# marl/l3embedding

Measured on AMD Instinct MI355X. Metric: AVC training pairs/sec (1s audio + 224x224 frame), higher is better.
Workload: dtype f32; 1 GPU; full cnn_L3_melspec2 AVC training step (audio+vision+fusion, fwd+bwd+Adam), batch 64 per GPU, global batch 64, fp32, inputs resident in HBM; global_batch=64, parallelism=dp1, fp32_conv=f4x4

## Files before the change

### include/l3hip.h

```cpp
#ifndef L3HIP_H
#define L3HIP_H

#include <stdint.h>

#ifdef __cplusplus
extern "C" {
#endif

#define L3_OK 0
#define L3_EINVAL (-1)
#define L3_EHIP (-2)
#define L3_ENOMEM (-3)
#define L3_ESTATE (-4)
#define L3_ECOMM (-5)

#define L3_MODEL_CNN_L3_ORIG 0
#define L3_MODEL_TINY_L3 1
#define L3_MODEL_CNN_L3_KAPREDBINPUTBN 2
#define L3_MODEL_CNN_L3_MELSPEC1 3
#define L3_MODEL_CNN_L3_MELSPEC2 4

typedef struct l3_engine l3_engine;

#define L3_DTYPE_F32 0
#define L3_DTYPE_BF16 1

#define L3_FP32_CONV_F4X4 0
#define L3_FP32_CONV_F2X2 1
#define L3_FP32_CONV_F2X2_BF16X6 2

#define L3_DP_MOVING_REPLICAS 0
#define L3_DP_MOVING_RANK_LOCAL 1

typedef struct l3_config {
    int32_t struct_size;
    int32_t model_type;
    int32_t batch;
    int32_t global_batch;
    int32_t device;
    int32_t db_max_scope;
    int32_t bn_zero_debias;
    int32_t dtype;
    void *stream;
    int32_t fp32_conv;
    int32_t dp_moving;
} l3_config;

int l3_create(const l3_config *cfg, uint64_t seed, l3_engine **out);
void l3_destroy(l3_engine *e);
const char *l3_last_error(const l3_engine *e);
int l3_model_type_from_name(const char *name);
int l3_build_experiments(void);
int l3_device_count(void);

int l3_param_count(const l3_engine *e);
int l3_param_info(const l3_engine *e, int index, char *name, int name_cap,
                  int32_t *ndim, int64_t shape[4], int32_t *trainable, int64_t *numel);
int l3_set_param(l3_engine *e, const char *name, const float *src, int64_t numel);
int l3_get_param(l3_engine *e, const char *name, float *dst, int64_t numel);
int l3_get_grad(l3_engine *e, const char *name, float *dst, int64_t numel);
int l3_reset_optimizer(l3_engine *e);
int l3_copy_state(l3_engine *dst, l3_engine *src);
int l3_optimizer_steps(const l3_engine *e, int64_t *adam_t, int64_t *bn_steps);

int l3_forward(l3_engine *e, const float *video, const float *audio, int training,
               float *probs, float *logits);

int l3_train_step(l3_engine *e, const float *video, const float *audio,
                  const float *labels, float lr, float *loss, float *acc);
int l3_eval_step(l3_engine *e, const float *video, const float *audio,
                 const float *labels, float *loss, float *acc);

int l3_upload_batch(l3_engine *e, const float *video, const float *audio, const float *labels);
int l3_upload_batch_raw(l3_engine *e, const uint8_t *video_u8, const int16_t *audio_i16,
                        const int32_t *labels_i32);
int l3_stage_batch_raw(l3_engine *e, const uint8_t *video_u8, const int16_t *audio_i16, const int32_t *labels_i32);
typedef struct l3_augment_params {
    int32_t start_x, start_y;
    int32_t flip;
    int32_t sat_first;
    float saturation;
    float brightness;
} l3_augment_params;
int l3_upload_batch_raw_aug(l3_engine *e, const uint8_t *video_u8, const int16_t *audio_i16, const int32_t *labels_i32,
                            const l3_augment_params *params, const double *u);
int l3_stage_batch_raw_aug(l3_engine *e, const uint8_t *video_u8, const int16_t *audio_i16, const int32_t *labels_i32,
                           const l3_augment_params *params, const double *u);
int l3_batch_gains(l3_engine *e, double *gains);
int l3_step_forward(l3_engine *e, int training);
int l3_tower_step(l3_engine *e, int tower, int backward);
int l3_step_bucket_count(const l3_engine *e);
int l3_step_backward_bucket(l3_engine *e, int bucket);
int l3_step_update(l3_engine *e, float lr, float grad_scale);
int l3_step_resident(l3_engine *e, float lr);
int l3_step_results(l3_engine *e, float *loss, float *acc, float *probs, float *logits);
int l3_step_results_enqueue(l3_engine *e, int slot, int reduce);
int l3_step_results_wait(l3_engine *e, int slot, float *loss, float *acc);

int l3_replicas_upload(l3_engine *e, const float *video, const float *audio, const float *labels, int replicas);
int l3_replicas_upload_raw(l3_engine *e, const uint8_t *video_u8, const int16_t *audio_i16, const int32_t *labels_i32, int replicas);
int l3_replicas_upload_raw_aug(l3_engine *e, const uint8_t *video_u8, const int16_t *audio_i16, const int32_t *labels_i32,
                               const l3_augment_params *params, const double *u, int replicas);
int l3_replicas_stage_raw(l3_engine *e, const uint8_t *video_u8, const int16_t *audio_i16, const int32_t *labels_i32, int replicas);
int l3_replicas_stage_raw_aug(l3_engine *e, const uint8_t *video_u8, const int16_t *audio_i16, const int32_t *labels_i32,
                              const l3_augment_params *params, const double *u, int replicas);
int l3_step_replicas(l3_engine *e, float lr);
int l3_eval_replicas(l3_engine *e, float *loss, float *acc);

#define L3_COMM_ID_BYTES 128
int l3_comm_unique_id(void *id128);
int l3_comm_init(l3_engine *e, const void *id128, int world, int rank);
int l3_comm_destroy(l3_engine *e);
int l3_comm_info(const l3_engine *e, int *world, int *rank, char *library_path, int path_cap);
int l3_comm_version(void);
int l3_comm_allreduce_host(l3_engine *e, double *vals, int n, int op);
int l3_step_dp(l3_engine *e, float lr);
int l3_comm_timing(l3_engine *e, int on);
int l3_comm_timing_read(l3_engine *e, double *exposed_ms, double *span_ms, double *bucket_ms, int cap, int *steps);

int l3_grad_arena_dev(l3_engine *e, void **dev_ptr, int64_t *numel);
int l3_bucket_range(const l3_engine *e, int bucket, int64_t *offset, int64_t *numel);
int l3_bn_stats_pack_dev(l3_engine *e, void **send_dev, int64_t *numel);
int l3_bn_stats_replicas_dev(l3_engine *e, int world, void **gathered_dev);

int l3_embed_audio(l3_engine *e, const float *audio, int64_t n, int pool_h, int pool_w, float *out);
int l3_embed_vision(l3_engine *e, const float *video, int64_t n, int pool_h, int pool_w, float *out);
int64_t l3_embed_dim(const l3_engine *e, int vision, int pool_h, int pool_w);
int l3_embed_audio_frames(l3_engine *e, const float *samples, int64_t n_samples, const int64_t *table,
                          int64_t n_frames, int pool_h, int pool_w, float *out);
int l3_embed_audio_clips_resampled(l3_engine *e, const float *native, int64_t n_native, const int64_t *clips,
                                   int64_t n_clips, const double *half_window, int64_t n_window, int num_table,
                                   int64_t n_samples, const int64_t *table, int64_t n_frames, int pool_h, int pool_w,
                                   float *out);

int l3_get_activation(l3_engine *e, const char *name, float *dst, int64_t numel);
int l3_activation_numel(l3_engine *e, const char *name, int64_t *numel);
int l3_sync(l3_engine *e);
int l3_profile_enable(l3_engine *e, int on);
int l3_set_tower_overlap(l3_engine *e, int on);
int l3_profile_read(l3_engine *e, int family, double *ms, int64_t *launches, double *flops);
int l3_profile_read_executed(l3_engine *e, int family, double *flops);
int l3_profile_read_bytes(l3_engine *e, int family, double *bytes);

#define L3_OP_BF16_STORED 2
#define L3_OP_BF16_STORED_OUT 3
int l3_op_conv2d_fwd_dt(int device, int dtype, const float *x, const float *w, const float *b, float *y,
                        int n, int h, int wd, int cin, int cout, int kh, int kw, int same);
int l3_op_conv2d_bwd_dt(int device, int dtype, const float *x, const float *w, const float *dy, float *dx,
                        float *dw, float *db, int n, int h, int wd, int cin, int cout, int kh, int kw, int same);
int l3_op_conv2d_fwd(int device, const float *x, const float *w, const float *b, float *y,
                     int n, int h, int wd, int cin, int cout, int kh, int kw, int same);
int l3_op_conv2d_bwd(int device, const float *x, const float *w, const float *dy,
                     float *dx, float *dw, float *db,
                     int n, int h, int wd, int cin, int cout, int kh, int kw, int same);
int l3_op_bn_relu_fwd(int device, const float *x, const float *gamma, const float *beta,
                      float *y, float *mean, float *var, int64_t rows, int c, int relu, int x_bf16);
int l3_op_bn_relu_bwd(int device, const float *x, const float *y, const float *dy,
                      const float *gamma, const float *beta, const float *mean, const float *var,
                      float *dx, float *dgamma, float *dbeta, int64_t rows, int c, int relu, int x_bf16);
int l3_op_bn_relu_pool2_fwd(int device, const float *x, const float *gamma, const float *beta, float *p,
                            float *mean, float *var, int n, int h, int wd, int c, int same, int relu_mode, int x_bf16);
int l3_op_bn_relu_pool2_bwd(int device, const float *x, const float *gamma, const float *beta, const float *dp,
                            float *dx, float *dgamma, float *dbeta, float *dbias, int n, int h, int wd, int c,
                            int same, int relu_mode, int x_bf16);
int l3_op_maxpool_fwd(int device, const float *x, float *y, int n, int h, int wd, int c,
                      int ph, int pw, int sh, int sw, int same);
int l3_op_maxpool_bwd(int device, const float *x, const float *dy, float *dx, int n, int h,
                      int wd, int c, int ph, int pw, int sh, int sw, int same);
int l3_op_frontend(int device, int model_type, const float *audio, int n, int db_max_scope, float *out);
int l3_op_gather_frames(int device, const float *samples, int64_t n_samples, const int64_t *table,
                        int64_t n_frames, float *frames);
int l3_op_resample(int device, const float *x, int64_t n_in, int64_t sr_orig, int64_t sr_new, const double *half_window,
                   int64_t n_window, int num_table, int64_t t0, int64_t n_out, float *y);
int l3_op_resample_clips(int device, const float *x, int64_t n_in, const int64_t *clips, int64_t n_clips, int64_t sr_new,
                         const double *half_window, int64_t n_window, int num_table, int64_t n_samples, int copy_equal,
                         float *y);
int l3_op_bn_stats_from_partials(int device, const float *part, int nblk, int c, const float *pivot, int64_t rows,
                                 float eps, float *mean, float *var);
int l3_op_preprocess(int device, const uint8_t *video_u8, int64_t nv, float *video,
                     const int16_t *audio_i16, int64_t na, float *audio);
int l3_op_augment_video(int device, const uint8_t *u8, int n, int h, int w, const l3_augment_params *params,
                        uint8_t *out_u8, float *out_f32);
int l3_op_augment_audio(int device, const int16_t *i16, int n, int t, const double *u, int16_t *out_i16, float *out_f32,
                        double *gains);

typedef struct l3_mlp l3_mlp;
int l3_mlp_create(int device, int D, int C, int batch, float weight_decay, uint64_t seed, l3_mlp **m);
void l3_mlp_destroy(l3_mlp *m);
int64_t l3_mlp_param_count(const l3_mlp *m);
int l3_mlp_set_data(l3_mlp *m, const float *X_train, const int32_t *y_train, int64_t n_train,
                    const float *X_valid, const int32_t *y_valid, int64_t n_valid);
int l3_mlp_epoch(l3_mlp *m, const int32_t *perm, float lr, int64_t t0, double *stats_out);
int l3_mlp_predict(l3_mlp *m, const float *X, int64_t n, float *probs_out);
int l3_mlp_get_weights(l3_mlp *m, float *dst, int64_t n);
int l3_mlp_set_weights(l3_mlp *m, const float *src, int64_t n);

int l3_op_mlp_dense_fwd(int device, const float *x, int64_t n_x, const int32_t *idx, int rows, int K, int N, const float *w,
                        const float *b, int relu, float *y);
int l3_op_mlp_dense_bwd_x(int device, const float *dy, const float *w, const float *h, int rows, int K, int N, float *dx);
int l3_op_mlp_wgrad(int device, const float *x, int64_t n_x, const int32_t *idx, int rows, int K, int N, const float *dy, float *dw,
                    float *db);
int l3_op_mlp_wgrad_adam(int device, const float *x, int64_t n_x, const int32_t *idx, int rows, int K, int N, const float *dy,
                         float *w, float *b, float *mw, float *vw, float *mb, float *vb, float weight_decay, float lr_t,
                         float *w2_out);
int l3_op_mlp_softmax_ce(int device, const float *z, const int32_t *labels, int rows, int C, float gscale, float *probs, float *dz,
                         float *ce, float *correct);
int l3_op_adam(int device, float *p, const float *g, float *m, float *v, int64_t n, int64_t n_l2, float l2x2, float lr_t);
int l3_op_adam_scaled(int device, float *p, const float *g, float *m, float *v, int64_t n, int64_t n_l2, float l2x2, float lr_t,
                      float b1, float b2, float eps, float gscale);
int l3_op_arena_fold(int device, float *acc, float *g, int64_t total, int64_t off, int64_t n, int mode);

int l3_op_head_dense_fwd(int device, const float *x, const float *w, const float *b, float *y, int B, int K, int N, int relu);
int l3_op_head_dense_bwd(int device, const float *x, const float *w, const float *dy, float *dw, float *db, float *dx, int B,
                         int K, int N);
int l3_op_softmax_ce2(int device, const float *logits, const float *labels, int B, float gscale, float *probs, float *dlogits,
                      float *stats);
int l3_op_sumsq(int device, const float *base, int64_t n_base, const int64_t *off, const int64_t *n, int count, int multi,
                float *out);
int l3_op_bn_moving_update(int device, int entries, const int32_t *c, const int64_t *slot_off, int64_t n_slots, float *moving,
                           float *biased, const float *batch, const float *gathered, int64_t n_gathered, int replicas,
                           int64_t stride, float momentum, int zero_debias, int64_t step, float *packed, int64_t n_packed);

#define L3_SVM_LINEAR 0
#define L3_SVM_POLY 1
#define L3_SVM_RBF 2
#define L3_SVM_SIGMOID 3
#define L3_SVM_DEFAULT_WS 64
#define L3_SVM_LOCAL_REL 0.1
typedef struct l3_svm_kernel {
    int32_t kind, degree;
    double gamma, coef0;
} l3_svm_kernel;
typedef struct l3_svm l3_svm;
int l3_svm_create(int device, l3_svm **m);
// ... 141 lines not shown
```

### l3embedding_amd/_build.py

```python
import os
import subprocess
from concurrent.futures import ThreadPoolExecutor

HERE = os.path.dirname(os.path.abspath(__file__))
CSRC = os.path.join(HERE, 'csrc')
LIBDIR = os.path.join(HERE, 'lib')
OBJDIR = os.path.join(LIBDIR, 'obj')
LIBPATH = os.path.join(LIBDIR, 'libl3hip.so')
SOURCES = ['conv.hip', 'conv_wino.hip', 'conv_wino4.hip', 'conv_bf16.hip', 'conv_bf16_halo.hip', 'conv_wgrad_bf16.hip', 'conv_wgrad_wino.hip',
           'conv_first.hip', 'conv_path.hip', 'elementwise.hip', 'bn_fused.hip', 'frontend.hip', 'clips.hip', 'resample.hip', 'batch_feed.hip', 'engine.hip', 'ops.hip',
           'comm.hip', 'mlp.hip', 'svm.hip', 'vggish.hip', 'augment.hip', 'featprep.hip', 'svm_eval.hip', 'forest.hip']
EXPERIMENT_SOURCES = ['conv_wino_bx6.hip', 'conv_wgrad_bx6.hip']
EXPERIMENTS = os.environ.get('L3_BUILD_EXPERIMENTS') == '1'
if EXPERIMENTS:
    SOURCES = SOURCES + EXPERIMENT_SOURCES
FLAGS = ['--offload-arch=gfx950', '-O3', '-std=c++17', '-fPIC'] + (['-DL3_EXPERIMENTS'] if EXPERIMENTS else [])
FILE_FLAGS = {'conv_wino4.hip': ['-fno-slp-vectorize'], 'conv_wino_bx6.hip': ['-fno-slp-vectorize'], 'conv_wgrad_bx6.hip': ['-fno-slp-vectorize'],
              'conv_first.hip': ['-mllvm', '-amdgpu-mfma-vgpr-form'], 'featprep.hip': ['-ffp-contract=off'], 'svm_eval.hip': ['-ffp-contract=off'],
              'forest.hip': ['-ffp-contract=off']}


def _headers():
    hs = [os.path.join(CSRC, f) for f in os.listdir(CSRC) if f.endswith('.h')]
    hs.append(os.path.join(HERE, '..', 'include', 'l3hip.h'))
    return [h for h in hs if os.path.exists(h)]


def source_hash(files=None):
    import hashlib
    h = hashlib.sha256()
    names = sorted(files) if files else sorted(f for f in os.listdir(CSRC) if f.endswith(('.hip', '.h')))
    for f in names:
        h.update(f.encode())
        with open(os.path.join(CSRC, f), 'rb') as fh:
            h.update(fh.read())
    return h.hexdigest()[:16]


def _stale(target, deps):
    if not os.path.exists(target):
        return True
    t = os.path.getmtime(target)
    return any(os.path.getmtime(d) > t for d in deps)


def needs_build():
    deps = [os.path.join(CSRC, s) for s in SOURCES] + _headers() + [os.path.abspath(__file__)]
    return _stale(LIBPATH, deps)


def _hipcc():
    hipcc = os.environ.get('HIPCC', '/opt/rocm/bin/hipcc')
    return hipcc if os.path.exists(hipcc) else 'hipcc'


def build(force=False, verbose=False, extra_flags=()):
    if not force and not needs_build():
        return LIBPATH
    os.makedirs(OBJDIR, exist_ok=True)
    hipcc, headers = _hipcc(), _headers()
    flags = FLAGS + list(extra_flags)
    stamp = os.path.join(OBJDIR, 'flags.txt')
    stamp_text = ' '.join(flags) + ' | ' + repr(sorted(FILE_FLAGS.items()))
    if not os.path.exists(stamp) or open(stamp).read() != stamp_text:
        force = True

    def compile_one(src):
        path, obj = os.path.join(CSRC, src), os.path.join(OBJDIR, src.replace('.hip', '.o'))
        if force or _stale(obj, [path] + headers):
            cmd = [hipcc] + flags + FILE_FLAGS.get(src, []) + ['-c', path, '-o', obj]
            if verbose:
                print(' '.join(cmd), flush=True)
            r = subprocess.run(cmd, stdout=subprocess.PIPE, stderr=subprocess.STDOUT)
            if r.returncode != 0:
                raise RuntimeError('hipcc failed for %s:\n%s' % (src, r.stdout.decode(errors='replace')))
        return obj

    with ThreadPoolExecutor(max_workers=min(len(SOURCES), os.cpu_count() or 1)) as pool:
        objs = list(pool.map(compile_one, SOURCES))
    cmd = [hipcc, '--offload-arch=gfx950', '-shared', '-fPIC', '-o', LIBPATH] + objs + ['-ldl']
    if verbose:
        print(' '.join(cmd), flush=True)
    subprocess.check_call(cmd)
    with open(stamp, 'w') as fh:
        fh.write(stamp_text)
    return LIBPATH


if __name__ == '__main__':
    print(build(force=True, verbose=True))
```

### l3embedding_amd/_lib.py

```python
import ctypes as C
import os

import numpy as np

from . import _build

MODEL_IDS = {
    'cnn_L3_orig': 0,
    'tiny_L3': 1,
    'cnn_L3_kapredbinputbn': 2,
    'cnn_L3_melspec1': 3,
    'cnn_L3_melspec2': 4,
}

FAMILIES = ('conv_fwd', 'conv_dgrad', 'conv_wgrad', 'elementwise', 'frontend', 'head', 'adam')


DTYPES = {'f32': 0, 'fp32': 0, 'float32': 0, 'bf16': 1}
FP32_CONV = {'f4x4': 0, 'f2x2': 1, 'f2x2_bf16x6': 2}
DP_MOVING = {'replicas': 0, 'rank_local': 1}
OP_DTYPES = dict(DTYPES, bf16_stored=2, bf16_stored_out=3)


class L3Config(C.Structure):
    _fields_ = [
        ('struct_size', C.c_int32),
        ('model_type', C.c_int32),
        ('batch', C.c_int32),
        ('global_batch', C.c_int32),
        ('device', C.c_int32),
        ('db_max_scope', C.c_int32),
        ('bn_zero_debias', C.c_int32),
        ('dtype', C.c_int32),
        ('stream', C.c_void_p),
        ('fp32_conv', C.c_int32),
        ('dp_moving', C.c_int32),
    ]


class L3Error(RuntimeError):
    pass


_f32p = C.POINTER(C.c_float)
_lib = None
TORCH_LOADED_FIRST = None

SIGNATURES = {
    'l3_create': (C.c_int, [C.POINTER(L3Config), C.c_uint64, C.POINTER(C.c_void_p)]),
    'l3_destroy': (None, [C.c_void_p]),
    'l3_last_error': (C.c_char_p, [C.c_void_p]),
    'l3_build_experiments': (C.c_int, []),
    'l3_comm_version': (C.c_int, []),
    'l3_bn_stats_pack_dev': (C.c_int, [C.c_void_p, C.POINTER(C.c_void_p), C.POINTER(C.c_int64)]),
    'l3_bn_stats_replicas_dev': (C.c_int, [C.c_void_p, C.c_int, C.POINTER(C.c_void_p)]),
    'l3_model_type_from_name': (C.c_int, [C.c_char_p]),
    'l3_device_count': (C.c_int, []),
    'l3_param_count': (C.c_int, [C.c_void_p]),
    'l3_param_info': (C.c_int, [C.c_void_p, C.c_int, C.c_char_p, C.c_int, C.POINTER(C.c_int32),
                                C.POINTER(C.c_int64), C.POINTER(C.c_int32), C.POINTER(C.c_int64)]),
    'l3_set_param': (C.c_int, [C.c_void_p, C.c_char_p, C.c_void_p, C.c_int64]),
    'l3_get_param': (C.c_int, [C.c_void_p, C.c_char_p, C.c_void_p, C.c_int64]),
    'l3_get_grad': (C.c_int, [C.c_void_p, C.c_char_p, C.c_void_p, C.c_int64]),
    'l3_reset_optimizer': (C.c_int, [C.c_void_p]),
    'l3_copy_state': (C.c_int, [C.c_void_p, C.c_void_p]),
    'l3_optimizer_steps': (C.c_int, [C.c_void_p, C.POINTER(C.c_int64), C.POINTER(C.c_int64)]),
    'l3_forward': (C.c_int, [C.c_void_p, C.c_void_p, C.c_void_p, C.c_int, C.c_void_p, C.c_void_p]),
    'l3_train_step': (C.c_int, [C.c_void_p, C.c_void_p, C.c_void_p, C.c_void_p, C.c_float,
                                C.POINTER(C.c_float), C.POINTER(C.c_float)]),
    'l3_eval_step': (C.c_int, [C.c_void_p, C.c_void_p, C.c_void_p, C.c_void_p,
                               C.POINTER(C.c_float), C.POINTER(C.c_float)]),
    'l3_upload_batch': (C.c_int, [C.c_void_p, C.c_void_p, C.c_void_p, C.c_void_p]),
    'l3_upload_batch_raw': (C.c_int, [C.c_void_p, C.c_void_p, C.c_void_p, C.c_void_p]),
    'l3_tower_step': (C.c_int, [C.c_void_p, C.c_int, C.c_int]),
    'l3_stage_batch_raw': (C.c_int, [C.c_void_p, C.c_void_p, C.c_void_p, C.c_void_p]),
    'l3_upload_batch_raw_aug': (C.c_int, [C.c_void_p, C.c_void_p, C.c_void_p, C.c_void_p, C.c_void_p, C.c_void_p]),
    'l3_stage_batch_raw_aug': (C.c_int, [C.c_void_p, C.c_void_p, C.c_void_p, C.c_void_p, C.c_void_p, C.c_void_p]),
    'l3_batch_gains': (C.c_int, [C.c_void_p, C.c_void_p]),
    'l3_step_forward': (C.c_int, [C.c_void_p, C.c_int]),
    'l3_step_bucket_count': (C.c_int, [C.c_void_p]),
    'l3_step_backward_bucket': (C.c_int, [C.c_void_p, C.c_int]),
    'l3_step_update': (C.c_int, [C.c_void_p, C.c_float, C.c_float]),
    'l3_step_resident': (C.c_int, [C.c_void_p, C.c_float]),
    'l3_replicas_upload': (C.c_int, [C.c_void_p, C.c_void_p, C.c_void_p, C.c_void_p, C.c_int]),
    'l3_replicas_upload_raw': (C.c_int, [C.c_void_p, C.c_void_p, C.c_void_p, C.c_void_p, C.c_int]),
    'l3_replicas_stage_raw': (C.c_int, [C.c_void_p, C.c_void_p, C.c_void_p, C.c_void_p, C.c_int]),
    'l3_replicas_upload_raw_aug': (C.c_int, [C.c_void_p] * 6 + [C.c_int]),
    'l3_replicas_stage_raw_aug': (C.c_int, [C.c_void_p] * 6 + [C.c_int]),
    'l3_step_replicas': (C.c_int, [C.c_void_p, C.c_float]),
    'l3_eval_replicas': (C.c_int, [C.c_void_p, C.POINTER(C.c_float), C.POINTER(C.c_float)]),
    'l3_step_results': (C.c_int, [C.c_void_p, C.POINTER(C.c_float), C.POINTER(C.c_float), C.c_void_p, C.c_void_p]),
    'l3_step_results_enqueue': (C.c_int, [C.c_void_p, C.c_int, C.c_int]),
    'l3_step_results_wait': (C.c_int, [C.c_void_p, C.c_int, C.POINTER(C.c_float), C.POINTER(C.c_float)]),
    'l3_comm_unique_id': (C.c_int, [C.c_void_p]),
    'l3_comm_init': (C.c_int, [C.c_void_p, C.c_void_p, C.c_int, C.c_int]),
    'l3_comm_destroy': (C.c_int, [C.c_void_p]),
    'l3_comm_info': (C.c_int, [C.c_void_p, C.POINTER(C.c_int), C.POINTER(C.c_int), C.c_char_p, C.c_int]),
    'l3_comm_allreduce_host': (C.c_int, [C.c_void_p, C.POINTER(C.c_double), C.c_int, C.c_int]),
    'l3_step_dp': (C.c_int, [C.c_void_p, C.c_float]),
    'l3_comm_timing': (C.c_int, [C.c_void_p, C.c_int]),
    'l3_comm_timing_read': (C.c_int, [C.c_void_p, C.POINTER(C.c_double), C.POINTER(C.c_double), C.POINTER(C.c_double), C.c_int, C.POINTER(C.c_int)]),
    'l3_grad_arena_dev': (C.c_int, [C.c_void_p, C.POINTER(C.c_void_p), C.POINTER(C.c_int64)]),
    'l3_bucket_range': (C.c_int, [C.c_void_p, C.c_int, C.POINTER(C.c_int64), C.POINTER(C.c_int64)]),
    'l3_embed_audio': (C.c_int, [C.c_void_p, C.c_void_p, C.c_int64, C.c_int, C.c_int, C.c_void_p]),
    'l3_embed_vision': (C.c_int, [C.c_void_p, C.c_void_p, C.c_int64, C.c_int, C.c_int, C.c_void_p]),
    'l3_embed_dim': (C.c_int64, [C.c_void_p, C.c_int, C.c_int, C.c_int]),
    'l3_embed_audio_frames': (C.c_int, [C.c_void_p, C.c_void_p, C.c_int64, C.c_void_p, C.c_int64, C.c_int, C.c_int,
                                        C.c_void_p]),
    'l3_embed_audio_clips_resampled': (C.c_int, [C.c_void_p, C.c_void_p, C.c_int64, C.c_void_p, C.c_int64, C.c_void_p,
                                                 C.c_int64, C.c_int, C.c_int64, C.c_void_p, C.c_int64, C.c_int, C.c_int,
                                                 C.c_void_p]),
    'l3_get_activation': (C.c_int, [C.c_void_p, C.c_char_p, C.c_void_p, C.c_int64]),
    'l3_activation_numel': (C.c_int, [C.c_void_p, C.c_char_p, C.POINTER(C.c_int64)]),
    'l3_sync': (C.c_int, [C.c_void_p]),
    'l3_profile_enable': (C.c_int, [C.c_void_p, C.c_int]),
    'l3_set_tower_overlap': (C.c_int, [C.c_void_p, C.c_int]),
    'l3_profile_read_executed': (C.c_int, [C.c_void_p, C.c_int, C.POINTER(C.c_double)]),
    'l3_profile_read_bytes': (C.c_int, [C.c_void_p, C.c_int, C.POINTER(C.c_double)]),
    'l3_profile_read': (C.c_int, [C.c_void_p, C.c_int, C.POINTER(C.c_double), C.POINTER(C.c_int64),
                                  C.POINTER(C.c_double)]),
    'l3_op_conv2d_fwd': (C.c_int, [C.c_int, C.c_void_p, C.c_void_p, C.c_void_p, C.c_void_p] + [C.c_int] * 8),
    'l3_op_conv2d_fwd_dt': (C.c_int, [C.c_int, C.c_int, C.c_void_p, C.c_void_p, C.c_void_p, C.c_void_p] + [C.c_int] * 8),
    'l3_op_conv2d_bwd_dt': (C.c_int, [C.c_int, C.c_int] + [C.c_void_p] * 6 + [C.c_int] * 8),
    'l3_op_conv2d_bwd': (C.c_int, [C.c_int] + [C.c_void_p] * 6 + [C.c_int] * 8),
    'l3_op_bn_relu_fwd': (C.c_int, [C.c_int] + [C.c_void_p] * 6 + [C.c_int64, C.c_int, C.c_int, C.c_int]),
    'l3_op_bn_relu_bwd': (C.c_int, [C.c_int] + [C.c_void_p] * 10 + [C.c_int64, C.c_int, C.c_int, C.c_int]),
    'l3_op_bn_relu_pool2_fwd': (C.c_int, [C.c_int] + [C.c_void_p] * 6 + [C.c_int] * 7),
    'l3_op_bn_relu_pool2_bwd': (C.c_int, [C.c_int] + [C.c_void_p] * 8 + [C.c_int] * 7),
    'l3_op_maxpool_fwd': (C.c_int, [C.c_int, C.c_void_p, C.c_void_p] + [C.c_int] * 9),
    'l3_op_maxpool_bwd': (C.c_int, [C.c_int, C.c_void_p, C.c_void_p, C.c_void_p] + [C.c_int] * 9),
    'l3_op_frontend': (C.c_int, [C.c_int, C.c_int, C.c_void_p, C.c_int, C.c_int, C.c_void_p]),
    'l3_op_gather_frames': (C.c_int, [C.c_int, C.c_void_p, C.c_int64, C.c_void_p, C.c_int64, C.c_void_p]),
    'l3_op_resample': (C.c_int, [C.c_int, C.c_void_p, C.c_int64, C.c_int64, C.c_int64, C.c_void_p, C.c_int64, C.c_int,
                                 C.c_int64, C.c_int64, C.c_void_p]),
    'l3_op_resample_clips': (C.c_int, [C.c_int, C.c_void_p, C.c_int64, C.c_void_p, C.c_int64, C.c_int64, C.c_void_p, C.c_int64,
                                       C.c_int, C.c_int64, C.c_int, C.c_void_p]),
    'l3_op_bn_stats_from_partials': (C.c_int, [C.c_int, C.c_void_p, C.c_int, C.c_int, C.c_void_p, C.c_int64, C.c_float,
                                               C.c_void_p, C.c_void_p]),
    'l3_op_preprocess': (C.c_int, [C.c_int, C.c_void_p, C.c_int64, C.c_void_p, C.c_void_p, C.c_int64, C.c_void_p]),
    'l3_op_augment_video': (C.c_int, [C.c_int, C.c_void_p, C.c_int, C.c_int, C.c_int, C.c_void_p, C.c_void_p, C.c_void_p]),
    'l3_op_augment_audio': (C.c_int, [C.c_int, C.c_void_p, C.c_int, C.c_int, C.c_void_p, C.c_void_p, C.c_void_p, C.c_void_p]),
    'l3_mlp_create': (C.c_int, [C.c_int, C.c_int, C.c_int, C.c_int, C.c_float, C.c_uint64, C.POINTER(C.c_void_p)]),
    'l3_mlp_destroy': (None, [C.c_void_p]),
    'l3_mlp_param_count': (C.c_int64, [C.c_void_p]),
    'l3_mlp_set_data': (C.c_int, [C.c_void_p, C.c_void_p, C.c_void_p, C.c_int64, C.c_void_p, C.c_void_p, C.c_int64]),
    'l3_mlp_epoch': (C.c_int, [C.c_void_p, C.c_void_p, C.c_float, C.c_int64, C.POINTER(C.c_double)]),
    'l3_mlp_predict': (C.c_int, [C.c_void_p, C.c_void_p, C.c_int64, C.c_void_p]),
    'l3_mlp_get_weights': (C.c_int, [C.c_void_p, C.c_void_p, C.c_int64]),
    'l3_mlp_set_weights': (C.c_int, [C.c_void_p, C.c_void_p, C.c_int64]),
    'l3_op_mlp_dense_fwd': (C.c_int, [C.c_int, C.c_void_p, C.c_int64, C.c_void_p, C.c_int, C.c_int, C.c_int, C.c_void_p,
                                      C.c_void_p, C.c_int, C.c_void_p]),
    'l3_op_mlp_dense_bwd_x': (C.c_int, [C.c_int, C.c_void_p, C.c_void_p, C.c_void_p, C.c_int, C.c_int, C.c_int, C.c_void_p]),
    'l3_op_mlp_wgrad': (C.c_int, [C.c_int, C.c_void_p, C.c_int64, C.c_void_p, C.c_int, C.c_int, C.c_int, C.c_void_p,
                                  C.c_void_p, C.c_void_p]),
    'l3_op_mlp_wgrad_adam': (C.c_int, [C.c_int, C.c_void_p, C.c_int64, C.c_void_p, C.c_int, C.c_int, C.c_int, C.c_void_p]
                             + [C.c_void_p] * 6 + [C.c_float, C.c_float, C.c_void_p]),
    'l3_op_mlp_softmax_ce': (C.c_int, [C.c_int, C.c_void_p, C.c_void_p, C.c_int, C.c_int, C.c_float] + [C.c_void_p] * 4),
    'l3_op_adam': (C.c_int, [C.c_int] + [C.c_void_p] * 4 + [C.c_int64, C.c_int64, C.c_float, C.c_float]),
    'l3_op_adam_scaled': (C.c_int, [C.c_int] + [C.c_void_p] * 4 + [C.c_int64, C.c_int64] + [C.c_float] * 6),
    'l3_op_arena_fold': (C.c_int, [C.c_int, C.c_void_p, C.c_void_p, C.c_int64, C.c_int64, C.c_int64, C.c_int]),
    'l3_op_head_dense_fwd': (C.c_int, [C.c_int] + [C.c_void_p] * 4 + [C.c_int] * 4),
    'l3_op_head_dense_bwd': (C.c_int, [C.c_int] + [C.c_void_p] * 6 + [C.c_int] * 3),
    'l3_op_softmax_ce2': (C.c_int, [C.c_int, C.c_void_p, C.c_void_p, C.c_int, C.c_float] + [C.c_void_p] * 3),
    'l3_op_sumsq': (C.c_int, [C.c_int, C.c_void_p, C.c_int64, C.c_void_p, C.c_void_p, C.c_int, C.c_int, C.c_void_p]),
    'l3_op_bn_moving_update': (C.c_int, [C.c_int, C.c_int, C.c_void_p, C.c_void_p, C.c_int64] + [C.c_void_p] * 4
                               + [C.c_int64, C.c_int, C.c_int64, C.c_float, C.c_int, C.c_int64, C.c_void_p, C.c_int64]),
    'l3_svm_create': (C.c_int, [C.c_int, C.POINTER(C.c_void_p)]),
    'l3_svm_destroy': (None, [C.c_void_p]),
    'l3_svm_set_data': (C.c_int, [C.c_void_p, C.c_void_p, C.c_int64, C.c_int]),
    'l3_svm_fit': (C.c_int, [C.c_void_p, C.c_void_p, C.c_double, C.c_double, C.c_int64, C.c_int] + [C.c_void_p] * 3
                   + [C.c_int] + [C.c_void_p] * 5),
    'l3_svm_fit_costs': (C.c_int, [C.c_void_p, C.c_void_p, C.c_void_p, C.c_double, C.c_int64, C.c_int] + [C.c_void_p] * 3
                         + [C.c_int] + [C.c_void_p] * 5),
    'l3_svm_cv_decision': (C.c_int, [C.c_void_p, C.c_void_p, C.c_int] + [C.c_void_p] * 8),
    'l3_op_svm_sigmoid_train': (C.c_int, [C.c_int, C.c_int] + [C.c_void_p] * 6),
    'l3_svm_decision': (C.c_int, [C.c_void_p, C.c_void_p, C.c_void_p, C.c_void_p, C.c_int64, C.c_int, C.c_void_p, C.c_void_p,
                                  C.c_int64, C.c_int] + [C.c_void_p] * 4),
    'l3_op_svm_kernel_rows': (C.c_int, [C.c_int, C.c_void_p, C.c_void_p, C.c_int64, C.c_int, C.c_void_p, C.c_int, C.c_void_p,
                                        C.c_int, C.c_void_p]),
    'l3_op_svm_smo': (C.c_int, [C.c_int, C.c_void_p, C.c_void_p, C.c_int, C.c_double, C.c_double, C.c_double, C.c_int64,
                                C.c_void_p, C.c_void_p, C.c_void_p]),
    'l3_svm_set_data_dev': (C.c_int, [C.c_void_p, C.c_void_p, C.c_int64, C.c_int64]),
    'l3_svm_get_rows': (C.c_int, [C.c_void_p, C.c_void_p, C.c_int64, C.c_void_p]),
    'l3_svm_set_model': (C.c_int, [C.c_void_p, C.c_void_p, C.c_void_p, C.c_void_p, C.c_int64, C.c_int, C.c_int] + [C.c_void_p] * 5),
    'l3_svm_score': (C.c_int, [C.c_void_p, C.c_void_p, C.c_void_p, C.c_void_p, C.c_int64, C.c_int64, C.c_int64, C.c_int, C.c_void_p,
                               C.c_void_p, C.c_int64] + [C.c_void_p] * 6),
    'l3_op_svm_tail': (C.c_int, [C.c_int, C.c_void_p, C.c_int64, C.c_int, C.c_void_p, C.c_void_p, C.c_void_p, C.c_void_p, C.c_int64]
                       + [C.c_void_p] * 8),
    'l3_vggish_create': (C.c_int, [C.c_int, C.c_int, C.POINTER(C.c_void_p)]),
    'l3_vggish_destroy': (None, [C.c_void_p]),
    'l3_vggish_batch': (C.c_int, [C.c_void_p]),
    'l3_vggish_set_conv': (C.c_int, [C.c_void_p, C.c_int]),
    'l3_vggish_set_weight': (C.c_int, [C.c_void_p, C.c_char_p, C.c_void_p, C.c_int64]),
    'l3_vggish_set_pca': (C.c_int, [C.c_void_p, C.c_void_p, C.c_void_p]),
    'l3_vggish_embed_clips_resampled': (C.c_int, [C.c_void_p, C.c_void_p, C.c_int64, C.c_void_p, C.c_int64, C.c_void_p, C.c_int64,
                                                  C.c_int, C.c_int64, C.c_void_p, C.c_int64, C.c_void_p, C.c_int64, C.c_int,
                                                  C.c_void_p]),
    'l3_op_vggish_logmel': (C.c_int, [C.c_int, C.c_void_p, C.c_int64, C.c_void_p, C.c_int64, C.c_void_p]),
    'l3_op_vggish_conv1': (C.c_int, [C.c_int, C.c_void_p, C.c_int64, C.c_void_p, C.c_int64, C.c_void_p, C.c_void_p, C.c_void_p]),
    'l3_op_vggish_bias_relu': (C.c_int, [C.c_int, C.c_void_p, C.c_void_p, C.c_void_p] + [C.c_int] * 5),
    'l3_op_vggish_postprocess': (C.c_int, [C.c_int, C.c_void_p, C.c_int64, C.c_void_p, C.c_void_p, C.c_int, C.c_void_p]),
    'l3_op_vggish_conv': (C.c_int, [C.c_int, C.c_int, C.c_void_p, C.c_void_p, C.c_void_p, C.c_void_p] + [C.c_int] * 6),
    'l3_feat_create': (C.c_int, [C.c_int, C.c_void_p, C.c_int64, C.c_int64, C.POINTER(C.c_void_p)]),
    'l3_feat_destroy': (None, [C.c_void_p]),
    'l3_feat_shape': (C.c_int, [C.c_void_p, C.POINTER(C.c_int64), C.POINTER(C.c_int64)]),
    'l3_feat_download': (C.c_int, [C.c_void_p, C.c_int64, C.c_int64, C.c_void_p]),
# ... 119 lines not shown
        cfg.db_max_scope = 0 if db_max_scope == 'sample' else 1
        cfg.bn_zero_debias = 1 if bn_zero_debias else 0
        cfg.stream = stream
        if dtype not in DTYPES:
            raise ValueError('dtype must be one of %s' % sorted(DTYPES))
        cfg.dtype = DTYPES[dtype]
        self.dtype = dtype
        if fp32_conv not in FP32_CONV:
            raise ValueError('fp32_conv must be one of %s' % sorted(FP32_CONV))
        cfg.fp32_conv = FP32_CONV[fp32_conv]
        self.fp32_conv = fp32_conv
        if dp_moving not in DP_MOVING:
            raise ValueError('dp_moving must be one of %s' % sorted(DP_MOVING))
        cfg.dp_moving = DP_MOVING[dp_moving]
        self.dp_moving = dp_moving
        h = C.c_void_p()
        rc = self.lib.l3_create(C.byref(cfg), int(seed), C.byref(h))
        check(rc, None)
        self.h = h
        self._params = None

    def close(self):
        if getattr(self, 'h', None):
            self.lib.l3_destroy(self.h)
            self.h = None

    def __del__(self):
        try:
            self.close()
        except Exception:
            pass

    def param_table(self):
        if self._params is None:
            out = []
            n = self.lib.l3_param_count(self.h)
            buf = C.create_string_buffer(256)
            for i in range(n):
                nd, tr, ne = C.c_int32(), C.c_int32(), C.c_int64()
                shp = (C.c_int64 * 4)()
                check(self.lib.l3_param_info(self.h, i, buf, 256, C.byref(nd), shp, C.byref(tr), C.byref(ne)), self.h)
                out.append((buf.value.decode(), tuple(int(shp[k]) for k in range(nd.value)), bool(tr.value)))
            self._params = out
        return self._params

    def set_param(self, name, value):
        v = _f32(value)
        check(self.lib.l3_set_param(self.h, name.encode(), _ptr(v), v.size), self.h)

    def get_param(self, name, shape):
        out = np.empty(shape, dtype=np.float32)
        check(self.lib.l3_get_param(self.h, name.encode(), _ptr(out), out.size), self.h)
        return out

    def get_grad(self, name, shape):
        out = np.empty(shape, dtype=np.float32)
        check(self.lib.l3_get_grad(self.h, name.encode(), _ptr(out), out.size), self.h)
        return out

    def set_params(self, P):
        for name, shape, _ in self.param_table():
            if name in P:
                self.set_param(name, np.asarray(P[name]).reshape(shape))

    def get_params(self):
        from collections import OrderedDict
        return OrderedDict((n, self.get_param(n, s)) for n, s, _ in self.param_table())

    def get_grads(self):
        from collections import OrderedDict
        return OrderedDict((n, self.get_grad(n, s)) for n, s, t in self.param_table() if t)

    def reset_optimizer(self):
        check(self.lib.l3_reset_optimizer(self.h), self.h)

    def copy_state_from(self, other):
        check(self.lib.l3_copy_state(self.h, other.h), self.h)

    def optimizer_steps(self):
        t, b = C.c_int64(), C.c_int64()
        check(self.lib.l3_optimizer_steps(self.h, C.byref(t), C.byref(b)), self.h)
        return t.value, b.value

    def forward(self, video, audio, training=False):
        v, a = _f32(video), _f32(audio)
        assert v.shape[0] == self.batch and a.shape[0] == self.batch
        probs = np.empty((self.batch, 2), np.float32)
        logits = np.empty((self.batch, 2), np.float32)
        check(self.lib.l3_forward(self.h, _ptr(v), _ptr(a), int(training), _ptr(probs), _ptr(logits)), self.h)
        return probs, logits

    def train_step(self, video, audio, labels, lr):
        v, a, l = _f32(video), _f32(audio), _f32(labels)
        loss, acc = C.c_float(), C.c_float()
        check(self.lib.l3_train_step(self.h, _ptr(v), _ptr(a), _ptr(l), lr, C.byref(loss), C.byref(acc)), self.h)
        return loss.value, acc.value

    def eval_step(self, video, audio, labels):
        v, a, l = _f32(video), _f32(audio), _f32(labels)
        loss, acc = C.c_float(), C.c_float()
        check(self.lib.l3_eval_step(self.h, _ptr(v), _ptr(a), _ptr(l), C.byref(loss), C.byref(acc)), self.h)
        return loss.value, acc.value

    def upload_batch(self, video=None, audio=None, labels=None):
        v, a, l = _f32(video), _f32(audio), _f32(labels)
        check(self.lib.l3_upload_batch(self.h, _ptr(v), _ptr(a), _ptr(l)), self.h)

    def _aug_args(self, params, u, replicas=None):
        p, g = augment_records(params), np.ascontiguousarray(u, dtype=np.float64)
        if replicas is not None:
            self._replica_rows(replicas, p, g)
        elif len(p) != self.batch or len(g) != self.batch:
            raise ValueError('%d augmentation records and %d gain draws for a batch of %d' % (len(p), len(g), self.batch))
        return p, g

    def _send_raw(self, fn, video_u8, audio_i16, labels_i32, records=None, replicas=None):
        args = [None if x is None else np.ascontiguousarray(x, dtype=t)
                for x, t in ((video_u8, np.uint8), (audio_i16, np.int16), (labels_i32, np.int32))]
        if replicas is not None:
            self._replica_rows(replicas, *args)
        if records is not None:
            args += self._aug_args(records[0], records[1], replicas)
        tail = [] if replicas is None else [int(replicas)]
        check(fn(self.h, *([_ptr(x) for x in args] + tail)), self.h)

    def upload_batch_raw(self, video_u8=None, audio_i16=None, labels_i32=None):
        self._send_raw(self.lib.l3_upload_batch_raw, video_u8, audio_i16, labels_i32)

    def stage_batch_raw(self, video_u8, audio_i16, labels_i32):
        self._send_raw(self.lib.l3_stage_batch_raw, video_u8, audio_i16, labels_i32)

    def upload_batch_raw_aug(self, video_u8, audio_i16, labels_i32, params, u):
        self._send_raw(self.lib.l3_upload_batch_raw_aug, video_u8, audio_i16, labels_i32, (params, u))

    def stage_batch_raw_aug(self, video_u8, audio_i16, labels_i32, params, u):
        self._send_raw(self.lib.l3_stage_batch_raw_aug, video_u8, audio_i16, labels_i32, (params, u))

    def batch_gains(self):
        out = np.empty(self.batch, np.float64)
        check(self.lib.l3_batch_gains(self.h, _ptr(out)), self.h)
        return out

    def tower_step(self, tower, backward=True):
        check(self.lib.l3_tower_step(self.h, {'vision': 0, 'audio': 1}[tower], int(backward)), self.h)

    def step_forward(self, training=True):
        check(self.lib.l3_step_forward(self.h, int(training)), self.h)

    def bucket_count(self):
        return self.lib.l3_step_bucket_count(self.h)

    def step_backward_bucket(self, b):
        check(self.lib.l3_step_backward_bucket(self.h, b), self.h)

    def step_update(self, lr, grad_scale=1.0):
        check(self.lib.l3_step_update(self.h, lr, grad_scale), self.h)

    def step_resident(self, lr):
        check(self.lib.l3_step_resident(self.h, lr), self.h)

    def _replica_rows(self, replicas, *arrays):
        rows = int(replicas) * self.batch
        for a in arrays:
            if len(a) != rows:
                raise ValueError('%d rows for %d replicas of batch %d (%d rows)' % (len(a), replicas, self.batch, rows))

# ... 98 lines not shown
        return out

    def embed_audio_frames(self, samples, table, pool, out=None):
        s = np.ascontiguousarray(samples, dtype=np.float32).reshape(-1)
        t = np.ascontiguousarray(table, dtype=np.int64).reshape(-1, 3)
        d = self.lib.l3_embed_dim(self.h, 0, pool[0], pool[1])
        if out is None:
            out = np.empty((t.shape[0], max(d, 0)), np.float32)
        elif out.dtype != np.float32 or not out.flags['C_CONTIGUOUS'] or out.shape != (t.shape[0], d):
            raise ValueError('out must be a C-contiguous float32 array of shape %s' % ((t.shape[0], d),))
        if s.size == 0:
            s = np.zeros(1, np.float32)[:0]
        check(self.lib.l3_embed_audio_frames(self.h, _ptr(s), s.size, _ptr(t), t.shape[0], pool[0], pool[1], _ptr(out)),
              self.h)
        return out

    def embed_audio_clips_resampled(self, native, clips, half_window, num_table, n_samples, table, pool, out=None):
        x = np.ascontiguousarray(native, dtype=np.float32).reshape(-1)
        c = np.ascontiguousarray(clips, dtype=np.int64).reshape(-1, 6)
        w = np.ascontiguousarray(half_window, dtype=np.float64).reshape(-1)
        t = np.ascontiguousarray(table, dtype=np.int64).reshape(-1, 3)
        d = self.lib.l3_embed_dim(self.h, 0, pool[0], pool[1])
        if out is None:
            out = np.empty((t.shape[0], max(d, 0)), np.float32)
        elif out.dtype != np.float32 or not out.flags['C_CONTIGUOUS'] or out.shape != (t.shape[0], d):
            raise ValueError('out must be a C-contiguous float32 array of shape %s' % ((t.shape[0], d),))
        if x.size == 0:
            x = np.zeros(1, np.float32)[:0]
        check(self.lib.l3_embed_audio_clips_resampled(self.h, _ptr(x), x.size, _ptr(c), c.shape[0], _ptr(w), w.size,
                                                      int(num_table), int(n_samples), _ptr(t), t.shape[0], pool[0], pool[1],
                                                      _ptr(out)), self.h)
        return out

    def embed_vision(self, video, pool=(7, 7)):
        v = _f32(video)
        d = self.lib.l3_embed_dim(self.h, 1, pool[0], pool[1])
        out = np.empty((v.shape[0], d), np.float32)
        check(self.lib.l3_embed_vision(self.h, _ptr(v), v.shape[0], pool[0], pool[1], _ptr(out)), self.h)
        return out

    def activation(self, name):
        n = C.c_int64()
        check(self.lib.l3_activation_numel(self.h, name.encode(), C.byref(n)), self.h)
        out = np.empty((n.value,), np.float32)
        check(self.lib.l3_get_activation(self.h, name.encode(), _ptr(out), n.value), self.h)
        return out

    def sync(self):
        check(self.lib.l3_sync(self.h), self.h)

    def set_tower_overlap(self, on=True):
        check(self.lib.l3_set_tower_overlap(self.h, int(on)), self.h)

    def profile_enable(self, on=True):
        check(self.lib.l3_profile_enable(self.h, int(on)), self.h)

    def profile_read(self):
        out = {}
        for i, fam in enumerate(FAMILIES):
            ms, n, fl = C.c_double(), C.c_int64(), C.c_double()
            check(self.lib.l3_profile_read(self.h, i, C.byref(ms), C.byref(n), C.byref(fl)), self.h)
            ex = C.c_double()
            check(self.lib.l3_profile_read_executed(self.h, i, C.byref(ex)), self.h)
            by = C.c_double()
            check(self.lib.l3_profile_read_bytes(self.h, i, C.byref(by)), self.h)
            out[fam] = dict(ms=ms.value, launches=n.value, flops=fl.value, executed_flops=ex.value, alg_bytes=by.value)
        return out


def op_conv2d_fwd(x, w, b, same, device=0, dtype='f32'):
    lib = load()
    x, w = _f32(x), _f32(w)
    b = _f32(b)
    n, h, wd, cin = x.shape
    kh, kw, _, cout = w.shape
    ho, wo = (h, wd) if same else (h - kh + 1, wd - kw + 1)
    y = np.empty((n, ho, wo, cout), np.float32)
    if OP_DTYPES[dtype]:
        check(lib.l3_op_conv2d_fwd_dt(device, OP_DTYPES[dtype], _ptr(x), _ptr(w), _ptr(b), _ptr(y), n, h, wd, cin, cout,
                                      kh, kw, int(same)))
    else:
        check(lib.l3_op_conv2d_fwd(device, _ptr(x), _ptr(w), _ptr(b), _ptr(y), n, h, wd, cin, cout, kh, kw, int(same)))
    return y


def op_conv2d_bwd(x, w, dy, same, device=0, dtype='f32'):
    lib = load()
    x, w, dy = _f32(x), _f32(w), _f32(dy)
    n, h, wd, cin = x.shape
    kh, kw, _, cout = w.shape
    dx, dw, db = np.empty_like(x), np.empty_like(w), np.empty((cout,), np.float32)
    if OP_DTYPES[dtype]:
        check(lib.l3_op_conv2d_bwd_dt(device, OP_DTYPES[dtype], _ptr(x), _ptr(w), _ptr(dy), _ptr(dx), _ptr(dw), _ptr(db),
                                      n, h, wd, cin, cout, kh, kw, int(same)))
    else:
        check(lib.l3_op_conv2d_bwd(device, _ptr(x), _ptr(w), _ptr(dy), _ptr(dx), _ptr(dw), _ptr(db),
                                   n, h, wd, cin, cout, kh, kw, int(same)))
    return dx, dw, db


def op_bn_relu_fwd(x, gamma, beta, relu, device=0, x_bf16=False):
    lib = load()
    x = _f32(x)
    c = x.shape[-1]
    rows = x.size // c
    y = np.empty_like(x)
    mean, var = np.empty((c,), np.float32), np.empty((c,), np.float32)
    check(lib.l3_op_bn_relu_fwd(device, _ptr(x), _ptr(_f32(gamma)), _ptr(_f32(beta)), _ptr(y), _ptr(mean),
                                _ptr(var), rows, c, int(relu), int(x_bf16)))
    return y, mean, var


def op_bn_relu_bwd(x, y, dy, gamma, mean, var, relu, device=0, beta=None, x_bf16=False):
    lib = load()
    x, y, dy = _f32(x), _f32(y), _f32(dy)
    c = x.shape[-1]
    rows = x.size // c
    dx = np.empty_like(x)
    dg, db = np.empty((c,), np.float32), np.empty((c,), np.float32)
    check(lib.l3_op_bn_relu_bwd(device, _ptr(x), _ptr(y), _ptr(dy), _ptr(_f32(gamma)), _ptr(_f32(beta)), _ptr(_f32(mean)),
                                _ptr(_f32(var)), _ptr(dx), _ptr(dg), _ptr(db), rows, c, int(relu), int(x_bf16)))
    return dx, dg, db


def op_bn_relu_pool2_fwd(x, gamma, beta, same, device=0, relu_mode=1, x_bf16=False):
    lib = load()
    x = _f32(x)
    n, h, wd, c = x.shape
    p = np.empty((n, _pool_out(h, 2, 2, same), _pool_out(wd, 2, 2, same), c), np.float32)
    mean, var = np.empty((c,), np.float32), np.empty((c,), np.float32)
    check(lib.l3_op_bn_relu_pool2_fwd(device, _ptr(x), _ptr(_f32(gamma)), _ptr(_f32(beta)), _ptr(p), _ptr(mean),
                                      _ptr(var), n, h, wd, c, int(same), int(relu_mode), int(x_bf16)))
    return p, mean, var


def op_bn_relu_pool2_bwd(x, gamma, beta, dp, same, device=0, relu_mode=1, x_bf16=False):
    lib = load()
    x, dp = _f32(x), _f32(dp)
    n, h, wd, c = x.shape
    dx = np.empty_like(x)
    dg, db, dbias = (np.empty((c,), np.float32) for _ in range(3))
    check(lib.l3_op_bn_relu_pool2_bwd(device, _ptr(x), _ptr(_f32(gamma)), _ptr(_f32(beta)), _ptr(dp), _ptr(dx),
                                      _ptr(dg), _ptr(db), _ptr(dbias), n, h, wd, c, int(same), int(relu_mode), int(x_bf16)))
    return dx, dg, db, dbias


def _pool_out(h, p, s, same):
    return -(-h // s) if same else (h - p) // s + 1


def op_maxpool_fwd(x, ph, pw, sh, sw, same, device=0):
    lib = load()
    x = _f32(x)
    n, h, wd, c = x.shape
    y = np.empty((n, _pool_out(h, ph, sh, same), _pool_out(wd, pw, sw, same), c), np.float32)
    check(lib.l3_op_maxpool_fwd(device, _ptr(x), _ptr(y), n, h, wd, c, ph, pw, sh, sw, int(same)))
    return y


def op_maxpool_bwd(x, dy, ph, pw, sh, sw, same, device=0):
    lib = load()
    x, dy = _f32(x), _f32(dy)
    n, h, wd, c = x.shape
    dx = np.empty_like(x)
    check(lib.l3_op_maxpool_bwd(device, _ptr(x), _ptr(dy), _ptr(dx), n, h, wd, c, ph, pw, sh, sw, int(same)))
    return dx
# ... 1039 lines not shown
```

### l3embedding_amd/csrc/conv_path.h

```cpp
#pragma once
#include "kernels.h"

namespace l3 {

ConvGeom conv_geom(int n, int h, int w, int cin, int cout, int kh, int kw, bool same, int f2x2);
ConvGeom conv_dgrad_geom(const ConvGeom& g);

struct ConvStorage {
    bool mixed = false;
    bool x_bf16 = false, y_bf16 = false, dy_bf16 = false, dx_bf16 = false;
};

enum ConvFwd { CF_BF16_STORED, CF_BF16_CAST, CF_FIRST, CF_FP32 };
enum ConvWgrad { WG_BF16_STORED, WG_BF16_CAST, WG_FP32 };
enum ConvDgrad { DG_NONE, DG_SMALL, DG_BF16_STORED, DG_BF16_CAST, DG_WINO, DG_FLIPPED };
struct ConvFwdPath {
    ConvFwd path = CF_FP32;
    bool wino_filter = false;
    double executed = -1.0;
};
struct ConvWgradPath {
    ConvWgrad path = WG_FP32;
    double executed = -1.0;
};
struct ConvDgradPath {
    ConvDgrad path = DG_NONE;
    double executed = -1.0;
};
ConvFwdPath conv_resolve_fwd(const ConvGeom& g, const ConvStorage& st, bool have_u);
ConvWgradPath conv_resolve_wgrad(const ConvGeom& g, const ConvStorage& st);
ConvDgradPath conv_resolve_dgrad(const ConvGeom& g, const ConvGeom& dg, const ConvStorage& st, bool have_u);

struct ConvBufs {
    const float* x = nullptr;
    const float* w = nullptr;
    const float* bias = nullptr;
    float* y = nullptr;
    float* dx = nullptr;
    float* dw = nullptr;
    float* wprep = nullptr;
    float* wino_u = nullptr;
    bool u_ready = false;
    float* wg_part = nullptr;
    float* stat_part = nullptr;
    int stat_mode = 0;
    const BnBwdFuse* bn_bwd = nullptr;
};
void conv_run_fwd(const ConvFwdPath& p, const ConvGeom& g, const ConvStorage& st, const ConvBufs& b, hipStream_t s);
void conv_run_wgrad(const ConvWgradPath& p, const ConvGeom& g, const ConvBufs& b, hipStream_t s);
void conv_run_dgrad(const ConvDgradPath& p, const ConvGeom& g, const ConvGeom& dg, const ConvStorage& st, const ConvBufs& b, hipStream_t s);

}
```

### l3embedding_amd/csrc/conv_path.hip

```cpp
#include "conv_path.h"

namespace l3 {

ConvGeom conv_geom(int n, int h, int w, int cin, int cout, int kh, int kw, bool same, int f2x2) {
    ConvGeom g{n, h, w, cin, 0, 0, cout, kh, kw, 0, 0};
    if (same) {
        tf_same(h, kh, 1, &g.Ho, &g.padT);
        tf_same(w, kw, 1, &g.Wo, &g.padL);
    } else {
        g.Ho = h - kh + 1;
        g.Wo = w - kw + 1;
    }
    g.f2x2 = f2x2;
    return g;
}

ConvGeom conv_dgrad_geom(const ConvGeom& g) {
    ConvGeom dg{g.N, g.Ho, g.Wo, g.Cout, g.H, g.W, g.Cin, g.KH, g.KW, g.KH - 1 - g.padT, g.KW - 1 - g.padL};
    dg.f2x2 = g.f2x2;
    dg.solo = g.solo;
    return dg;
}

ConvFwdPath conv_resolve_fwd(const ConvGeom& g, const ConvStorage& st, bool have_u) {
    ConvFwdPath p;
    const bool mp = st.mixed && conv_bf16_ok(g);
    p.path = mp ? (st.x_bf16 ? CF_BF16_STORED : CF_BF16_CAST) : conv_first_ok(g) ? CF_FIRST : CF_FP32;
    p.wino_filter = have_u && !mp && conv_wino_ok(g);
    p.executed = p.wino_filter ? conv_wino_executed_flops(g) : -1.0;
    return p;
}

ConvWgradPath conv_resolve_wgrad(const ConvGeom& g, const ConvStorage& st) {
    ConvWgradPath p;
    const bool wbf = st.mixed && conv_wgrad_bf16_ok(g);
    p.path = !wbf ? WG_FP32 : st.x_bf16 && st.dy_bf16 ? WG_BF16_STORED : WG_BF16_CAST;
    p.executed = conv_wgrad_executed_flops(g, wbf);
    return p;
}

ConvDgradPath conv_resolve_dgrad(const ConvGeom& g, const ConvGeom& dg, const ConvStorage& st, bool have_u) {
    ConvDgradPath p;
    const bool dbf = st.mixed && conv_bf16_ok(dg), wino = have_u && conv_wino_ok(dg);
    p.path = conv_dgrad_small_ok(g) ? DG_SMALL : dbf ? (st.dy_bf16 ? DG_BF16_STORED : DG_BF16_CAST) : wino ? DG_WINO : DG_FLIPPED;
    p.executed = wino && !dbf ? conv_wino_executed_flops(dg) : -1.0;
    return p;
}

void conv_run_fwd(const ConvFwdPath& p, const ConvGeom& g, const ConvStorage& st, const ConvBufs& b, hipStream_t s) {
    if (p.wino_filter && !b.u_ready) conv_wino_transform_weights(b.w, b.wino_u, g, false, s);
    switch (p.path) {
        case CF_BF16_STORED:
            conv_weights_bf16(b.w, b.wprep, g.KH, g.KW, g.Cin, g.Cout, true, s);
            conv_bf16_fwd(b.x, b.wprep, b.bias, b.y, g, s, true, b.stat_part, b.stat_mode, st.y_bf16);
            break;
        case CF_BF16_CAST:
            conv_flip_weights(b.w, b.wprep, g.KH, g.KW, g.Cin, g.Cout, s);
            conv_bf16_fwd(b.x, b.wprep, b.bias, b.y, g, s);
            break;
        case CF_FIRST:
            conv_first_fwd(b.x, b.w, b.bias, b.y, g, s, b.stat_part, b.stat_mode, st.y_bf16);
            break;
        case CF_FP32:
            conv_fwd(b.x, b.w, b.bias, b.y, g, s, p.wino_filter ? b.wino_u : nullptr, b.stat_part, b.stat_mode);
            break;
    }
}

void conv_run_wgrad(const ConvWgradPath& p, const ConvGeom& g, const ConvBufs& b, hipStream_t s) {
    conv_wgrad(b.x, b.y, b.dw, b.wg_part, g, s, p.path != WG_FP32, p.path == WG_BF16_STORED);
}

void conv_run_dgrad(const ConvDgradPath& p, const ConvGeom& g, const ConvGeom& dg, const ConvStorage& st, const ConvBufs& b, hipStream_t s) {
    switch (p.path) {
        case DG_SMALL:
            (void)conv_dgrad_small(b.y, b.w, b.dx, g, s);
            break;
        case DG_BF16_STORED:
            conv_weights_bf16(b.w, b.wprep, g.KH, g.KW, g.Cin, g.Cout, false, s);
            conv_bf16_fwd(b.y, b.wprep, nullptr, b.dx, dg, s, true, b.stat_part, 0, st.dx_bf16, b.bn_bwd);
            break;
        case DG_BF16_CAST:
            conv_bf16_fwd(b.y, b.w, nullptr, b.dx, dg, s);
            break;
        case DG_WINO:
            conv_wino_transform_weights(b.w, b.wino_u, dg, true, s);
            conv_fwd(b.y, nullptr, nullptr, b.dx, dg, s, b.wino_u, b.stat_part, 0, b.bn_bwd);
            break;
        case DG_FLIPPED:
            conv_flip_weights(b.w, b.wprep, g.KH, g.KW, g.Cin, g.Cout, s);
            conv_fwd(b.y, b.wprep, nullptr, b.dx, dg, s);
            break;
        case DG_NONE: break;
    }
}

}
```

### l3embedding_amd/csrc/conv_wino.hip

```cpp
#include "kernels.h"
#include "device_common.h"
#include "wino_common.h"

#include <stdlib.h>

#include <atomic>
#include <mutex>

namespace l3 {

bool conv_wino4_selected(const ConvGeom& g);
double conv_wino4_executed_flops(const ConvGeom& g);
int conv_wino4_blocks(const ConvGeom& g, int n);
void conv_wino4_transform_weights(const float* w, float* u, const ConvGeom& g, bool from_fwd_for_dgrad, hipStream_t s);
void conv_wino4_launch(const float* x, const float* u, const float* bias, float* y, const ConvGeom& g, int n, hipStream_t s,
                       float* stat_part, int stat_mode, const BnBwdFuse* bn_bwd);

#ifdef L3_EXPERIMENTS
bool conv_wino_bx6_ok(const ConvGeom& g);
int conv_wino_bx6_blocks(const ConvGeom& g, int n);
double conv_wino_bx6_executed_flops(const ConvGeom& g);
void conv_wino_bx6_transform_weights(const float* w, float* u, const ConvGeom& g, bool from_fwd_for_dgrad, hipStream_t s);
void conv_wino_bx6_launch(const float* x, const float* u, const float* bias, float* y, const ConvGeom& g, int n, hipStream_t s,
                          float* stat_part, int stat_mode, const BnBwdFuse* bn_bwd);
// ... 222 lines not shown
    }
}

template <int BTX, int SM>
void launch_wino2(const WinoArgs& a, hipStream_t s) {
    using G = WinoGeom<BTX>;
    static std::once_flag once[L3_MAX_DEVICES];
    int dev = 0;
    (void)hipGetDevice(&dev);
    std::call_once(once[dev & (L3_MAX_DEVICES - 1)], [] {
        (void)hipFuncSetAttribute((const void*)conv_wino_kernel<BTX, SM>, hipFuncAttributeMaxDynamicSharedMemorySize, (int)G::LDS_BYTES + 16);
    });
    static const int persist_env = l3_knob("L3_WINO_PERSIST") ? atoi(l3_knob("L3_WINO_PERSIST")) : -1;
    const int persist = persist_env >= 0 ? persist_env : 1;
    static int cus[L3_MAX_DEVICES] = {0};
    int& ncu = cus[dev & (L3_MAX_DEVICES - 1)];
    if (ncu == 0) {
        hipDeviceProp_t prop;
        ncu = hipGetDeviceProperties(&prop, dev) == hipSuccess && prop.multiProcessorCount >= 8 ? prop.multiProcessorCount / 8 * 8 : 256;
    }
    const int total = a.mblocks * a.nblocks;
    const int ncu_k = l3_knob("L3_W4_NCU") ? atoi(l3_knob("L3_W4_NCU")) / 8 * 8 : 0;
    const int ncu_eff = ncu_k > 0 && ncu_k < ncu ? ncu_k : ncu;
    const int dyn_on = l3_knob("L3_W4_DYNAMIC") ? atoi(l3_knob("L3_W4_DYNAMIC")) : a.dynamic;
    WinoArgs m = a;
    m.work = persist && total > ncu_eff && dyn_on ? persistent_work_counters(s) : nullptr;
    hipLaunchKernelGGL((conv_wino_kernel<BTX, SM>), dim3(persist && total > ncu_eff ? ncu_eff : total), dim3(1024), G::LDS_BYTES + 16, s, m);
}
template <int BTX>
void launch_wino(const WinoArgs& a, hipStream_t s) {
    if (a.stat_part != nullptr && a.bb.x != nullptr)
        launch_wino2<BTX, 2>(a, s);
    else if (a.stat_part != nullptr)
        launch_wino2<BTX, 1>(a, s);
    else
        launch_wino2<BTX, 0>(a, s);
}

struct WinoPlan {
    int btx, txb, mblocks;
};
WinoPlan wino_plan(const ConvGeom& g) {
    const int TY = (g.H + 1) / 2, TX = (g.W + 1) / 2;
    int best = 16, waste = ((TX + 15) / 16) * 16;
    for (int btx : {8, 4}) {
        const int wst = ((TX + btx - 1) / btx) * btx;
        if (wst < waste) {
            waste = wst;
            best = btx;
        }
    }
    static const int force = l3_knob("L3_WINO_BTX") ? atoi(l3_knob("L3_WINO_BTX")) : 0;
    if (force == 4 || force == 8 || force == 16) best = force;
    WinoPlan p;
    p.btx = best;
    p.txb = (TX + best - 1) / best;
    const int bty = 64 / best;
    p.mblocks = ((g.N * TY + bty - 1) / bty) * p.txb;
    return p;
}

}

bool conv_wino_ok(const ConvGeom& g) {
    static const int enabled = l3_knob("L3_WINOGRAD") ? atoi(l3_knob("L3_WINOGRAD")) : 1;
    return enabled && g.KH == 3 && g.KW == 3 && g.padT == 1 && g.padL == 1 && g.Ho == g.H && g.Wo == g.W &&
           g.Cin % 8 == 0 && g.Cout % 64 == 0 && (size_t)16 * g.Cin * g.Cout * 4 < (1ull << 31) &&
           (size_t)g.H * g.W * (g.Cin > g.Cout ? g.Cin : g.Cout) * 4 < (1ull << 31);
}

static int wino_chunk_samples(const ConvGeom& g) {
    const size_t per_sample = (size_t)g.H * g.W * (g.Cin > g.Cout ? g.Cin : g.Cout) * 4;
    size_t nc = ((1ull << 31) - 1) / per_sample;
    const size_t row_cap = ((1u << 22) - 1) / (size_t)((g.H + 1) / 2);
    if (nc > row_cap) nc = row_cap;
    if (nc > (size_t)g.N) nc = (size_t)g.N;
    return nc < 1 ? 1 : (int)nc;
}

static bool use_bx6(const ConvGeom& g) { return g.f2x2 == 2 && conv_wino_ok(g) && conv_wino_bx6_ok(g); }
static bool use_wino4(const ConvGeom& g) { return !use_bx6(g) && conv_wino_ok(g) && conv_wino4_selected(g); }

bool conv_wino_is_bx6(const ConvGeom& g) { return use_bx6(g); }

double conv_wino_executed_flops(const ConvGeom& g) {
    if (use_bx6(g)) return conv_wino_bx6_executed_flops(g);
    if (use_wino4(g)) return conv_wino4_executed_flops(g);
    return 2.0 * 16.0 * (double)g.N * ((g.H + 1) / 2) * ((g.W + 1) / 2) * (double)g.Cin * (double)g.Cout;
}

size_t conv_wino_floats(const ConvGeom& g) { return conv_wino_ok(g) ? (size_t)36 * g.Cin * g.Cout : 0; }

void conv_wino_transform_weights(const float* w, float* u, const ConvGeom& g, bool from_fwd_for_dgrad, hipStream_t s) {
    if (use_bx6(g)) return conv_wino_bx6_transform_weights(w, u, g, from_fwd_for_dgrad, s);
    if (use_wino4(g)) return conv_wino4_transform_weights(w, u, g, from_fwd_for_dgrad, s);
    const int total = g.Cin * g.Cout;
    hipLaunchKernelGGL(wino_weights_kernel, dim3((total + 255) / 256), dim3(256), 0, s, w, u, g.Cin, g.Cout,
                       from_fwd_for_dgrad ? 1 : 0);
}

static int stat_blocks_of(const ConvGeom& g, int algo) {
    const int nc = wino_chunk_samples(g);
    int blocks = 0;
    for (int n0 = 0; n0 < g.N; n0 += nc) {
        ConvGeom gc = g;
        gc.N = g.N - n0 < nc ? g.N - n0 : nc;
        blocks += algo == 1 ? conv_wino4_blocks(g, gc.N) : algo == 2 ? conv_wino_bx6_blocks(g, gc.N) : wino_plan(gc).mblocks;
    }
    return blocks;
}

int conv_wino_stat_blocks(const ConvGeom& g) { return conv_wino_ok(g) ? stat_blocks_of(g, use_bx6(g) ? 2 : use_wino4(g) ? 1 : 0) : 0; }

int conv_wino_stat_blocks_max(const ConvGeom& g) {
    if (!conv_wino_ok(g)) return 0;
    int m = stat_blocks_of(g, 0);
    const int b = stat_blocks_of(g, 1);
    if (b > m) m = b;
    if (g.Cin % 16 == 0 && conv_wino_bx6_ok(g)) {
        const int c = stat_blocks_of(g, 2);
        if (c > m) m = c;
    }
    return m;
}

void conv_wino_fwd(const float* x, const float* u, const float* bias, float* y, const ConvGeom& g, hipStream_t s,
                   float* stat_part, int stat_mode, const BnBwdFuse* bn_bwd) {
    const int nc = wino_chunk_samples(g);
    if (use_bx6(g)) {
        for (int n0 = 0; n0 < g.N; n0 += nc) {
            const int n = g.N - n0 < nc ? g.N - n0 : nc;
            BnBwdFuse bb;
            if (bn_bwd != nullptr) {
                bb = *bn_bwd;
                bb.x = bn_bwd->x + (size_t)n0 * g.H * g.W * g.Cout;
            }
            conv_wino_bx6_launch(x + (size_t)n0 * g.H * g.W * g.Cin, u, bias, y + (size_t)n0 * g.H * g.W * g.Cout, g, n, s, stat_part,
                                 stat_mode, bn_bwd != nullptr ? &bb : nullptr);
            if (stat_part != nullptr) stat_part += (size_t)conv_wino_bx6_blocks(g, n) * 2 * g.Cout;
        }
        return;
    }
    if (use_wino4(g)) {
        for (int n0 = 0; n0 < g.N; n0 += nc) {
            const int n = g.N - n0 < nc ? g.N - n0 : nc;
            BnBwdFuse bb;
            if (bn_bwd != nullptr) {
                bb = *bn_bwd;
                bb.x = bn_bwd->x + (size_t)n0 * g.H * g.W * g.Cout;
            }
            conv_wino4_launch(x + (size_t)n0 * g.H * g.W * g.Cin, u, bias, y + (size_t)n0 * g.H * g.W * g.Cout, g, n, s,
                              stat_part, stat_mode, bn_bwd != nullptr ? &bb : nullptr);
            if (stat_part != nullptr) stat_part += (size_t)conv_wino4_blocks(g, n) * 2 * g.Cout;
        }
        return;
    }
    for (int n0 = 0; n0 < g.N; n0 += nc) {
        ConvGeom gc = g;
        gc.N = g.N - n0 < nc ? g.N - n0 : nc;
        WinoArgs a;
        a.dynamic = g.dynamic;
        a.x = x + (size_t)n0 * g.H * g.W * g.Cin;
        a.u = u; a.bias = bias;
        a.y = y + (size_t)n0 * g.H * g.W * g.Cout;
        a.N = gc.N; a.H = g.H; a.W = g.W; a.Cin = g.Cin; a.Cout = g.Cout;
        a.TY = (g.H + 1) / 2;
// ... 27 lines not shown
```

### l3embedding_amd/csrc/engine.hip

```cpp
#include <hip/hip_runtime.h>
#include "knobs.h"

#include <cmath>
#include <cstdio>
#include <cstdlib>
#include <cstring>
#include <map>
#include <string>
#include <vector>

#include "../../include/l3hip.h"
#include "comm.h"
#include "conv_path.h"
#include "kernels.h"

namespace {

using namespace l3;

static thread_local std::string g_create_error;

constexpr float BN_EPS = 1e-3f;
constexpr float BN_MOMENTUM = 0.99f;
constexpr float L2_WEIGHT = 1e-5f;
constexpr float ADAM_B1 = 0.9f, ADAM_B2 = 0.999f, ADAM_EPS = 1e-8f;
constexpr int AUDIO_T = 48000;

enum ParamKind { PK_KERNEL, PK_BIAS, PK_GAMMA, PK_BETA, PK_MMEAN, PK_MVAR, PK_CONST };
enum OpKind { OP_CONV, OP_BN, OP_RELU, OP_POOL, OP_FLATTEN };
enum Family { F_CONV_FWD, F_CONV_DGRAD, F_CONV_WGRAD, F_ELEMWISE, F_FRONTEND, F_HEAD, F_ADAM, F_COUNT };

struct Tensor {
    float* d = nullptr;
    float* g = nullptr;
    int N = 0, H = 0, W = 0, C = 0;
    int64_t batch_stride = 0;
    bool alias = false;
    bool d_bf16 = false, g_bf16 = false;
    int64_t numel() const { return (int64_t)N * H * W * C; }
    int64_t rows() const { return (int64_t)N * H * W; }
};

struct Param {
    std::string name;
    int ndim = 0;
    int64_t shape[4] = {1, 1, 1, 1};
    bool trainable = false;
    int kind = 0;
    int64_t numel = 0;
    int bucket = 0;
    float* d = nullptr;
    float* g = nullptr;
};

enum FirstWgrad { FW_NONE, FW_AUG, FW_AUG_DEFERRED };
struct ConvPlan {
    ConvStorage st;
    ConvFwdPath fwd;
    int stat_mode = 0;
    FirstWgrad aug = FW_NONE;
    ConvWgradPath wgrad;
    bool colsum = false;
    ConvDgradPath dgrad;
    int bwd_bn = -1;
    double fwd_bytes = 0.0, wg_bytes = 0.0, dg_bytes = 0.0;
};
enum BnStats { BS_PARTIALS, BS_FAST, BS_PLAIN, BS_MOVING };
enum BnBwd { BB_BY_FIRST_CONV, BB_FAST_POOLED, BB_FAST, BB_FAST_DEFERRED, BB_PLAIN };
struct BnPlan {
    BnStats stats = BS_MOVING;
    int stat_blocks = 0;
    BnBwd bwd = BB_PLAIN;
    int bwd_blocks = 0;
    double fwd_bytes = 0.0, bwd_bytes = 0.0;
};

struct Op {
    OpKind kind;
    std::string name;
    int in = 0, out = 0;
    int block = 0, bucket = 0;
    int kh = 0, kw = 0, cout = 0;
    bool same = false;
    ConvGeom geom{};
    ConvGeom dgeom{};
    int p_kernel = -1, p_bias = -1;
    float* wflip = nullptr;
    float *wino_uf = nullptr, *wino_ud = nullptr;
    int in_bn = -1;
    bool fused_first = false;
    bool defer_apply = false;
    int bn_defer = -1;
    float *xaug = nullptr, *gaug = nullptr;
    ConvGeom ageom{};
    int bn_follow = -1;
    bool need_dx = true;
    int dy_to_bn = -1;
    float* xwin = nullptr;
    int p_gamma = -1, p_beta = -1, p_mmean = -1, p_mvar = -1;
    bool fused_relu = false;
    bool prerelu = false;
    int fuse_pool = -1;
    int bias_param = -1;
    bool fused_into_bn = false;
    bool bias_by_bn = false;
    float *mean = nullptr, *var = nullptr, *scale = nullptr, *shift = nullptr;
    float *biased_mean = nullptr, *biased_var = nullptr;
    PoolGeom pg{};
    ConvPlan cp{};
    BnPlan bp{};
};

struct Tower {
    std::string prefix;
    std::vector<Tensor> t;
    std::vector<Op> ops;
    int nblocks = 0;
    int emb_conv_op = -1;
    bool training = false;
};

struct FrontendDef {
    int n_dft, n_hop, same, n_mels, sqrt_out, db, loglambda;
    const char* layer_name;
};

struct ProfRec {
    int family;
    hipEvent_t a, b;
    double flops;
    double executed;
    double bytes;
    const char* tag;
};

}

struct l3_engine {
    l3_config cfg{};
    int B = 0;
    hipStream_t stream = nullptr;
    bool own_stream = false;
    hipStream_t side = nullptr;
    hipEvent_t ev_fork = nullptr, ev_join = nullptr;
    float *red_scratch2 = nullptr, *wg_scratch2 = nullptr;
    float *stat_scratch = nullptr, *stat_scratch2 = nullptr;
    size_t stat_max = 0;
    float* w4_tail = nullptr;
    bool overlap = true;
    BnMovingEntry* bn_table = nullptr;
    int bn_table_n = 0, bn_table_max_c = 0;
    std::string err;
    l3::DeviceBufs bufs;

    std::vector<Param> params;
    std::map<std::string, int> pindex;
    float *arena_p = nullptr, *arena_g = nullptr, *arena_m = nullptr, *arena_v = nullptr;
    int64_t n_train = 0;
    struct Segment { int64_t off, n; bool l2; };
    std::vector<Segment> segments;
    struct Bucket { int64_t off, n; };
    std::vector<Bucket> buckets;
    int64_t adam_t = 0;
    int64_t bn_step = 0;

    Tower vis, aud;
    FrontendDef fe{};
    FrontendCfg fcfg{};
    int p_real = -1, p_imag = -1, p_mel = -1;
    bool consts_dirty = true;
    float *wdft = nullptr, *melw = nullptr, *frames = nullptr, *spec = nullptr, *smax = nullptr;
    bool dft_consts_done = false;
    float *dft_win = nullptr, *dft_b1 = nullptr, *dft_b2 = nullptr, *dft_tw = nullptr, *dft_y = nullptr, *dft_a2 = nullptr, *dft_nyq = nullptr;
    int *mel_start = nullptr, *mel_len = nullptr, *mel_off = nullptr;
    int64_t melw_cap = 0;

    float *video = nullptr, *audio = nullptr, *labels = nullptr;
    l3::BatchFeed feed;
    float* res_host = nullptr;
    float* res_sum = nullptr;
    bool res_reduced[2] = {false, false};
    bool res_pending[2] = {false, false};
    hipEvent_t ev_res[2] = {nullptr, nullptr};
    hipEvent_t ev_res_a = nullptr, ev_res_b = nullptr;
    hipEvent_t ev_step[2] = {nullptr, nullptr};
    bool ev_step_set[2] = {false, false};
    int64_t steps_enqueued = 0;
    float *rep_acc = nullptr, *rep_stats = nullptr;
    bool results_global = false;
    bool res_global[2] = {false, false};
    int nv = 0, na = 0, head = 0;
    int p_w1 = -1, p_b1 = -1, p_w2 = -1, p_b2 = -1;
    float *h0 = nullptr, *dh0 = nullptr, *h1 = nullptr, *dh1 = nullptr, *logits = nullptr, *dlogits = nullptr,
          *probs = nullptr, *stats = nullptr, *l2part = nullptr;
    float *red_scratch = nullptr, *wg_scratch = nullptr, *sq_scratch = nullptr, *emb_out = nullptr;
    size_t emb_out_cap = 0;
    float* clip_samples = nullptr;
    int64_t* clip_table = nullptr;
    size_t clip_samples_cap = 0, clip_table_cap = 0;
    l3::ResampleStage resample;
    bool last_training = false;
    bool fwd_done = false;

    l3::Comm* comm = nullptr;
    std::vector<hipEvent_t> ev_bucket;
    int bucket_ready = -1;
    hipEvent_t ev_comm_done = nullptr;
    double* comm_scratch = nullptr;
    bool dp_order_alt = false;
    float *bn_send = nullptr, *bn_gathered = nullptr;
    int bn_pack_floats = 0, bn_gathered_world = 0, bn_replicas_armed = 0;
    bool bn_packed = false;
    bool comm_timing = false;
    std::vector<hipEvent_t> ev_ct0, ev_ct1;
    hipEvent_t ev_ct_ready = nullptr, ev_ct_done = nullptr;
    std::vector<double> ct_bucket_ms;
    double ct_exposed_ms = 0.0, ct_span_ms = 0.0;
    int64_t ct_steps = 0;

    bool prof_on = false;
    std::vector<ProfRec> prof_recs;
    std::vector<hipEvent_t> ev_pool;
    double prof_ms[F_COUNT] = {0};
    int64_t prof_n[F_COUNT] = {0};
    double prof_flops[F_COUNT] = {0};
    double prof_exec[F_COUNT] = {0};
    double prof_bytes[F_COUNT] = {0};
};

namespace {

#define HIPCHK(e, call)                                                                       \
    do {                                                                                      \
        hipError_t _st = (call);                                                              \
        if (_st != hipSuccess) {                                                              \
            (e)->err = std::string(#call) + ": " + hipGetErrorString(_st);                    \
            return L3_EHIP;                                                                   \
        }                                                                                     \
    } while (0)

template <class T>
int dev_alloc_t(l3_engine* e, T** p, size_t count) {
    if ((*p = e->bufs.alloc<T>(count)) != nullptr) return L3_OK;
    e->err = "hipMalloc(" + std::to_string(l3::DeviceBufs::bytes_of<T>(count)) + "): " + hipGetErrorString(hipGetLastError());
    return L3_ENOMEM;
}
template <class T>
// ... 567 lines not shown
            return L3_EINVAL;
        }
        HIPCHK(e, hipMemcpy(e->melw, packed.data(), packed.size() * 4, hipMemcpyHostToDevice));
        HIPCHK(e, hipMemcpy(e->mel_start, st.data(), st.size() * 4, hipMemcpyHostToDevice));
        HIPCHK(e, hipMemcpy(e->mel_len, ln.data(), ln.size() * 4, hipMemcpyHostToDevice));
        HIPCHK(e, hipMemcpy(e->mel_off, of.data(), of.size() * 4, hipMemcpyHostToDevice));
    }
    e->consts_dirty = false;
    return L3_OK;
}

int alloc_everything(l3_engine* e, uint64_t seed) {
    const int B = e->B;
    const int nbuckets = 1 + e->vis.nblocks + e->aud.nblocks;
    std::vector<int64_t> offs(e->params.size(), -1);
    int64_t off = 0;
    e->buckets.resize(nbuckets);
    for (int b = 0; b < nbuckets; ++b) {
        e->buckets[b].off = off;
        for (int pass = 0; pass < 2; ++pass) {
            const int64_t seg0 = off;
            for (size_t i = 0; i < e->params.size(); ++i) {
                Param& p = e->params[i];
                if (!p.trainable || p.bucket != b) continue;
                const bool is_l2 = p.kind == PK_KERNEL;
                if ((pass == 0) != is_l2) continue;
                offs[i] = off;
                off += (p.numel + 3) / 4 * 4;
            }
            if (off > seg0) e->segments.push_back({seg0, off - seg0, pass == 0});
        }
        e->buckets[b].n = off - e->buckets[b].off;
    }
    e->n_train = off;
    int rc;
    if ((rc = dev_alloc_t(e, &e->arena_p, off))) return rc;
    if ((rc = dev_alloc_t(e, &e->arena_g, off))) return rc;
    if ((rc = dev_alloc_t(e, &e->arena_m, off))) return rc;
    if ((rc = dev_alloc_t(e, &e->arena_v, off))) return rc;
    HIPCHK(e, hipMemset(e->arena_p, 0, off * 4));
    HIPCHK(e, hipMemset(e->arena_g, 0, off * 4));
    HIPCHK(e, hipMemset(e->arena_m, 0, off * 4));
    HIPCHK(e, hipMemset(e->arena_v, 0, off * 4));
    for (size_t i = 0; i < e->params.size(); ++i) {
        Param& p = e->params[i];
        if (p.trainable) {
            p.d = e->arena_p + offs[i];
            p.g = e->arena_g + offs[i];
        } else {
            if ((rc = dev_alloc_t(e, &p.d, p.numel))) return rc;
        }
    }
    Rng rng(seed);
    std::vector<float> real, imag, mel;
    host_dft_kernels(e->fcfg.n_dft, real, imag);
    if (e->fcfg.n_mels) host_mel_basis(48000, e->fcfg.n_dft, e->fcfg.n_mels, mel);
    for (size_t i = 0; i < e->params.size(); ++i) {
        Param& p = e->params[i];
        std::vector<float> h((size_t)p.numel, 0.f);
        switch (p.kind) {
            case PK_KERNEL: {
                const int64_t fan_in = p.numel / p.shape[p.ndim - 1];
                const double sd = std::sqrt(2.0 / (double)fan_in);
                for (auto& v : h) {
                    double z = rng.normal();
                    while (std::fabs(z) > 2.0) z = rng.normal();
                    v = (float)(z * sd);
                }
                break;
            }
            case PK_GAMMA:
            case PK_MVAR:
                for (auto& v : h) v = 1.f;
                break;
            case PK_CONST:
                if ((int)i == e->p_real) h = real;
                else if ((int)i == e->p_imag) h = imag;
                else h = mel;
                break;
            default: break;
        }
        HIPCHK(e, hipMemcpy(p.d, h.data(), (size_t)p.numel * 4, hipMemcpyHostToDevice));
    }
    const FrontendCfg& f = e->fcfg;
    if ((rc = dev_alloc_t(e, &e->wdft, (size_t)f.n_dft * f.ncols_pad))) return rc;
    {
        const size_t per_row = (size_t)(f.ke + f.ko) > (size_t)f.n_dft ? (size_t)(f.ke + f.ko) : (size_t)f.n_dft;
        if ((rc = dev_alloc_t(e, &e->frames, (size_t)B * f.n_frames * per_row))) return rc;
    }
    if ((rc = dev_alloc_t(e, &e->spec, (size_t)B * f.n_frames * f.ncols_pad))) return rc;
    if ((rc = dev_alloc_t(e, &e->smax, (size_t)B + 16))) return rc;
    if (f.n_dft == 2048) {
        const size_t M = (size_t)B * f.n_frames;
        if ((rc = dev_alloc_t(e, &e->dft_y, M * 2 * f.n_dft))) return rc;
        if ((rc = dev_alloc_t(e, &e->dft_a2, M * 2 * f.n_dft))) return rc;
        if ((rc = dev_alloc_t(e, &e->dft_nyq, M))) return rc;
        if ((rc = dev_alloc_t(e, &e->dft_win, (size_t)f.n_dft))) return rc;
        if ((rc = dev_alloc_t(e, &e->dft_b1, (size_t)f.N1 * 2 * f.N1))) return rc;
        if ((rc = dev_alloc_t(e, &e->dft_b2, (size_t)2 * f.N2 * f.N2))) return rc;
        if ((rc = dev_alloc_t(e, &e->dft_tw, (size_t)f.N2 * f.N1 * 2))) return rc;
    }
    if (f.n_mels) {
        e->melw_cap = (int64_t)f.n_freq * 64 + 1024;
        if ((rc = dev_alloc_t(e, &e->melw, (size_t)e->melw_cap))) return rc;
        if ((rc = dev_alloc_t(e, &e->mel_start, (size_t)f.n_mels))) return rc;
        if ((rc = dev_alloc_t(e, &e->mel_len, (size_t)f.n_mels))) return rc;
        if ((rc = dev_alloc_t(e, &e->mel_off, (size_t)f.n_mels))) return rc;
    }
    if ((rc = dev_alloc_t(e, &e->video, (size_t)B * 224 * 224 * 3))) return rc;
    if ((rc = dev_alloc_t(e, &e->audio, (size_t)B * AUDIO_T))) return rc;
    if ((rc = dev_alloc_t(e, &e->labels, (size_t)B * 2))) return rc;
    e->feed.bind(B, AUDIO_T, e->video, e->audio, e->labels);
    HIPCHK(e, hipMemset(e->labels, 0, (size_t)B * 2 * 4));
    const int D = e->nv + e->na;
    if ((rc = dev_alloc_t(e, &e->h0, (size_t)B * D))) return rc;
    if ((rc = dev_alloc_t(e, &e->dh0, (size_t)B * D))) return rc;
    if ((rc = dev_alloc_t(e, &e->h1, (size_t)B * e->head))) return rc;
    if ((rc = dev_alloc_t(e, &e->dh1, (size_t)B * e->head))) return rc;
    if ((rc = dev_alloc_t(e, &e->logits, (size_t)B * 2))) return rc;
    if ((rc = dev_alloc_t(e, &e->dlogits, (size_t)B * 2))) return rc;
    if ((rc = dev_alloc_t(e, &e->probs, (size_t)B * 2))) return rc;
    if ((rc = dev_alloc_t(e, &e->stats, 16))) return rc;
    if ((rc = dev_alloc_t(e, &e->l2part, 64))) return rc;
    HIPCHK(e, hipMemset(e->l2part, 0, 64 * 4));
    static const int bf16_storage = knob_int("L3_BF16_STORAGE", 1);
    static const int bf16_out = knob_int("L3_BF16_CONV_OUT", 1);
    static const int bf16_dgrad_out = knob_int("L3_BF16_DGRAD_OUT", 1);
    if (e->cfg.dtype == L3_DTYPE_BF16 && bf16_storage)
        for (Tower* tw : {&e->vis, &e->aud})
            for (size_t ci = 0; ci < tw->ops.size(); ++ci) {
                Op& cv = tw->ops[ci];
                if (cv.kind != OP_CONV || cv.in_bn >= 0 || !conv_bf16_ok(cv.geom) || !conv_wgrad_bf16_ok(cv.geom) ||
                    !cv.need_dx || !conv_bf16_ok(cv.dgeom) || cv.bn_follow < 0 || !cv.bias_by_bn)
                    continue;
                bool produced_ok = false;
                for (const Op& pr : tw->ops) {
                    if (pr.kind != OP_BN || !bn_fast_ok(tw->t[pr.in].C)) continue;
                    if (pr.fuse_pool >= 0 ? tw->ops[pr.fuse_pool].out == cv.in : pr.out == cv.in) produced_ok = true;
                }
                if (!produced_ok) continue;
                tw->t[cv.in].d_bf16 = true;
                tw->t[cv.out].g_bf16 = true;
                if (bf16_out && (int)ci != tw->emb_conv_op) tw->t[cv.out].d_bf16 = true;
                if (bf16_dgrad_out) tw->t[cv.in].g_bf16 = true;
            }
    if (e->cfg.dtype == L3_DTYPE_BF16 && bf16_storage && bf16_out)
        for (Tower* tw : {&e->vis, &e->aud})
            for (size_t ci = 0; ci < tw->ops.size(); ++ci) {
                Op& cv = tw->ops[ci];
                if (cv.kind == OP_CONV && conv_first_ok(cv.geom) && cv.bn_follow >= 0 && cv.bias_by_bn &&
                    (int)ci != tw->emb_conv_op)
                    tw->t[cv.out].d_bf16 = true;
            }
    auto t_floats = [](const Tensor& t, bool bf16) { return bf16 ? (size_t)(t.numel() + 1) / 2 : (size_t)t.numel(); };
    size_t red_max = 1024, wg_max = 16;
    size_t& stat_max = e->stat_max;
    for (int ti = 0; ti < 2; ++ti) {
        Tower& tw = ti == 0 ? e->vis : e->aud;
        tw.t[0].d = ti == 0 ? e->video : nullptr;
        if (ti == 1) {
            if ((rc = dev_alloc_t(e, &tw.t[0].d, (size_t)tw.t[0].numel()))) return rc;
        }
        const int64_t concat_off = ti == 0 ? 0 : e->nv;
        for (size_t oi = 0; oi < tw.ops.size(); ++oi) {
            Op& op = tw.ops[oi];
            Tensor& y = tw.t[op.out];
            const bool last = oi + 1 == tw.ops.size();
            if (last) {
                y.d = e->h0 + concat_off;
                y.g = e->dh0 + concat_off;
                y.batch_stride = D;
                y.alias = true;
                if (op.kind == OP_POOL) op.pg.out_batch_stride = D;
            } else if ((op.kind == OP_BN && op.fuse_pool >= 0) || (op.kind == OP_RELU && op.fused_into_bn)) {
                if (op.kind == OP_BN) {
                    bool wanted = false;
                    for (size_t ci = 0; ci < tw.ops.size(); ++ci)
                        if (tw.ops[ci].kind == OP_CONV && tw.ops[ci].dy_to_bn == (int)oi) wanted = true;
                    const Tensor& pl = tw.t[tw.ops[op.fuse_pool].out];
                    if (wanted && (rc = dev_alloc_t(e, &op.xwin, t_floats(pl, tw.t[op.in].d_bf16)))) return rc;
                }
            } else {
                if ((rc = dev_alloc_t(e, &y.d, t_floats(y, y.d_bf16)))) return rc;
                if ((rc = dev_alloc_t(e, &y.g, t_floats(y, y.g_bf16)))) return rc;
            }
            const Tensor& x = tw.t[op.in];
            if (op.kind == OP_CONV) {
                if ((rc = dev_alloc_t(e, &op.wflip, (size_t)e->params[op.p_kernel].numel))) return rc;
                if (conv_wino_floats(op.geom) && (rc = dev_alloc_t(e, &op.wino_uf, conv_wino_floats(op.geom)))) return rc;
                {
                    const size_t sf = (size_t)conv_wino_stat_blocks_max(op.geom) * 2 * op.geom.Cout;
                    if (sf > stat_max) stat_max = sf;
                    const size_t sb = (size_t)conv_bf16_stat_blocks(op.geom) * 2 * op.geom.Cout;
                    if (e->cfg.dtype == L3_DTYPE_BF16 && sb > stat_max) stat_max = sb;
                    const size_t s1 = (size_t)conv_first_stat_blocks(op.geom) * 2 * op.geom.Cout;
                    if (s1 > stat_max) stat_max = s1;
                    const size_t sd = op.dy_to_bn >= 0 ? (size_t)conv_wino_stat_blocks_max(op.dgeom) * 2 * op.dgeom.Cout : 0;
                    if (sd > stat_max) stat_max = sd;
                    const size_t sdb = op.dy_to_bn >= 0 && e->cfg.dtype == L3_DTYPE_BF16
                                           ? (size_t)conv_bf16_stat_blocks(op.dgeom) * 2 * op.dgeom.Cout : 0;
                    if (sdb > stat_max) stat_max = sdb;
                }
                if (op.need_dx && conv_wino_floats(op.dgeom) &&
                    (rc = dev_alloc_t(e, &op.wino_ud, conv_wino_floats(op.dgeom))))
                    return rc;
                const size_t w = conv_wgrad_scratch_floats(op.geom);
                if (w > wg_max) wg_max = w;
                if (op.in_bn >= 0) {
                    if ((rc = dev_alloc_t(e, &op.xaug, (size_t)x.rows() * op.ageom.Cin))) return rc;
                    if ((rc = dev_alloc_t(e, &op.gaug, (size_t)op.kh * op.kw * op.ageom.Cin * op.cout))) return rc;
                    const size_t wa = conv_wgrad_scratch_floats(op.ageom);
                    if (wa > wg_max) wg_max = wa;
                }
                const size_t r = colreduce_scratch_floats(y.rows(), y.C);
                if (r > red_max) red_max = r;
            } else if (op.kind == OP_BN) {
                const int C = x.C;
                for (float** p : {&op.mean, &op.var, &op.scale, &op.shift, &op.biased_mean, &op.biased_var}) {
                    if ((rc = dev_alloc_t(e, p, (size_t)(C + 3) / 4 * 4))) return rc;
                    HIPCHK(e, hipMemset(*p, 0, (size_t)(C + 3) / 4 * 4 * 4));
                }
                const size_t r = colreduce_scratch_floats(x.rows(), C);
                if (r > red_max) red_max = r;
            }
        }
    }
    if (e->vis.ops.back().kind != OP_POOL || e->aud.ops.back().kind != OP_POOL) {
        e->err = "tower must end in a pooling layer";
        return L3_EINVAL;
    }
    if ((rc = dev_alloc_t(e, &e->red_scratch, red_max))) return rc;
    if ((rc = dev_alloc_t(e, &e->wg_scratch, wg_max))) return rc;
    if ((rc = dev_alloc_t(e, &e->sq_scratch, 2048))) return rc;
    if (stat_max && (rc = dev_alloc_t(e, &e->stat_scratch, stat_max))) return rc;
    {
        bool any_w4 = false;
        for (Tower* tw : {&e->vis, &e->aud})
            for (auto& op : tw->ops)
                if (op.kind == OP_CONV && (op.wino_uf || op.wino_ud)) any_w4 = true;
        if (any_w4 && e->cfg.dtype != L3_DTYPE_BF16 && (rc = dev_alloc_t(e, &e->w4_tail, conv_wino4_tail_scratch_bytes() / sizeof(float)))) return rc;
    }
    if (e->side) {
        if ((rc = dev_alloc_t(e, &e->red_scratch2, red_max))) return rc;
        if ((rc = dev_alloc_t(e, &e->wg_scratch2, wg_max))) return rc;
        if (stat_max && (rc = dev_alloc_t(e, &e->stat_scratch2, stat_max))) return rc;
    }
    return L3_OK;
}

int run_frontend(l3_engine* e) {
    int rc = rebuild_consts(e);
    if (rc) return rc;
    const FrontendCfg& f = e->fcfg;
    const int B = e->B;
    const int M = B * f.n_frames;
    if (f.factored) {
        const int N1 = f.N1, N2 = f.N2;
        const int form = knob_int("L3_DFT_FACTORED", 1);
        if (form != 2 && f.n_mels > 0 && N1 == 32 && N2 == 64) {
            const double m1 = (double)M * N2, m2 = (double)M * N1;
            ProfScope ps(e, F_FRONTEND, 2.0 * M * (double)f.n_dft * 2.0 * f.n_freq + 2.0 * M * (double)f.n_freq * f.n_mels, nullptr,
                         2.0 * m1 * N1 * 2 * N1 + 2.0 * m2 * 2 * N2 * N2);
            dft_fused(e->audio, e->dft_win, e->dft_b1, e->dft_b2, e->dft_tw, e->melw, e->mel_start, e->mel_len, e->mel_off, e->aud.t[0].d, B,
                      AUDIO_T, f, e->stream);
            if (f.db) db_normalize(e->aud.t[0].d, e->smax, B, e->aud.t[0].batch_stride, e->cfg.db_max_scope, e->stream);
            return L3_OK;
        }
        {
            ProfScope ps(e, F_FRONTEND, 0.0);
            dft_pack_frames(e->audio, e->dft_win, e->frames, B, AUDIO_T, f, e->stream);
        }
        {
            const double m1 = (double)M * N2, m2 = (double)M * N1;
            ProfScope ps(e, F_FRONTEND, 2.0 * M * (double)f.n_dft * 2.0 * f.n_freq, nullptr, 2.0 * m1 * N1 * 2 * N1 + 2.0 * m2 * 2 * N2 * N2);
            const ConvGeom g1{1, 1, M * N2, N1, 1, M * N2, 2 * N1, 1, 1, 0, 0}, g2{1, 1, M * N1, 2 * N2, 1, M * N1, N2, 1, 1, 0, 0};
            conv_fwd(e->frames, e->dft_b1, nullptr, e->dft_y, g1, e->stream);
            dft_twiddle(e->dft_y, e->dft_tw, e->dft_a2, e->dft_nyq, M, f, e->stream);
            conv_fwd(e->dft_a2, e->dft_b2, nullptr, e->spec, g2, e->stream);
        }
    } else if (f.folded) {
        float* fe = e->frames;
        float* fo = e->frames + (size_t)M * f.ke;
        {
            ProfScope ps(e, F_FRONTEND, 0.0);
            frame_audio_folded(e->audio, fe, fo, B, AUDIO_T, f, e->stream);
        }
        ProfScope ps(e, F_FRONTEND, 2.0 * M * (double)f.n_dft * 2.0 * f.n_freq, nullptr,
                     2.0 * M * (double)(f.ke + f.ko) * f.nc);
        const ConvGeom ge{1, 1, M, f.ke, 1, M, f.nc, 1, 1, 0, 0}, go{1, 1, M, f.ko, 1, M, f.nc, 1, 1, 0, 0};
        conv_fwd(fe, e->wdft, nullptr, e->spec, ge, e->stream);
        conv_fwd(fo, e->wdft + (size_t)f.ke * f.nc, nullptr, e->spec + (size_t)M * f.nc, go, e->stream);
    } else {
        {
            ProfScope ps(e, F_FRONTEND, 0.0);
            frame_audio(e->audio, e->frames, B, AUDIO_T, f, e->stream);
        }
        ConvGeom g{1, 1, M, f.n_dft, 1, M, f.ncols_pad, 1, 1, 0, 0};
        ProfScope ps(e, F_FRONTEND, 2.0 * M * (double)f.n_dft * 2.0 * f.n_freq);
        conv_fwd(e->frames, e->wdft, nullptr, e->spec, g, e->stream);
    }
    {
        ProfScope ps(e, F_FRONTEND, f.n_mels ? 2.0 * B * f.n_frames * (double)f.n_freq * f.n_mels : 0.0);
        spec_to_features(e->spec, e->melw, e->mel_start, e->mel_len, e->mel_off, e->aud.t[0].d, B, f, e->stream, e->dft_nyq);
        if (f.db) db_normalize(e->aud.t[0].d, e->smax, B, e->aud.t[0].batch_stride, e->cfg.db_max_scope, e->stream);
    }
    return L3_OK;
}

static inline double act_bytes(const Tensor& t) { return (double)t.numel() * (t.d_bf16 ? 2.0 : 4.0); }
static inline double grad_bytes(const Tensor& t) { return (double)t.numel() * (t.g_bf16 ? 2.0 : 4.0); }

int plan_tower(l3_engine* e, Tower& tw, bool training, int solo) {
    static const int epi_stats = knob_int("L3_EPILOGUE_STATS", 1);
    const bool bf16 = e->cfg.dtype == L3_DTYPE_BF16;
    tw.training = training;
    auto fits = [&](const Op& cv, int blocks, int C) {
        if ((size_t)blocks * 2 * C <= e->stat_max) return true;
        e->err = cv.name + ": " + std::to_string(blocks) + " partial blocks of " + std::to_string(C) + " channels exceed the statistics scratch (" +
                 std::to_string(e->stat_max) + " floats)";
        return false;
    };
    auto defers = [&](const Op& bn) {
        return training && bn.defer_apply && bn.fuse_pool < 0 && bn_fast_ok(tw.t[bn.in].C) && tw.t[bn.in].d_bf16 == tw.t[bn.out].g_bf16;
    };
    for (auto& op : tw.ops) op.bp = BnPlan{};
    for (auto& op : tw.ops) {
        if (op.kind != OP_CONV) continue;
        op.geom.solo = op.dgeom.solo = solo;
        op.geom.dynamic = op.dgeom.dynamic = e->comm != nullptr ? 1 : 0;
        float* ts = solo ? e->w4_tail : nullptr;
        op.geom.tail_scratch = op.dgeom.tail_scratch = ts;
        op.geom.tail_scratch_bytes = op.dgeom.tail_scratch_bytes = ts ? conv_wino4_tail_scratch_bytes() : 0;

        const Tensor &x = tw.t[op.in], &y = tw.t[op.out];
        const double wbytes = (double)e->params[op.p_kernel].numel * 4.0;
        ConvPlan& p = op.cp = ConvPlan{};
        p.st = ConvStorage{bf16, x.d_bf16, y.d_bf16, y.g_bf16, x.g_bf16};
        p.fwd = conv_resolve_fwd(op.geom, p.st, op.wino_uf != nullptr);
        p.fwd_bytes = act_bytes(x) + act_bytes(y) + wbytes;
        const int nblk = p.fwd.path == CF_BF16_STORED ? conv_bf16_stat_blocks(op.geom)
                         : p.fwd.path == CF_FIRST     ? conv_first_stat_blocks(op.geom)
                         : p.fwd.path == CF_FP32 && p.fwd.wino_filter ? conv_wino_stat_blocks(op.geom) : 0;
        if (epi_stats && training && op.bn_follow >= 0 && e->stat_max > 0 && nblk > 0) {
            if (!fits(op, nblk, op.geom.Cout)) return L3_ESTATE;
            p.stat_mode = tw.ops[op.bn_follow].prerelu ? 2 : 1;
            tw.ops[op.bn_follow].bp.stat_blocks = nblk;
        }
        if (training && op.in_bn >= 0) {
            const Op* fb = op.bn_defer >= 0 && defers(tw.ops[op.bn_defer]) ? &tw.ops[op.bn_defer] : nullptr;
            p.aug = fb ? FW_AUG_DEFERRED : FW_AUG;
            p.wg_bytes = (double)x.rows() * op.ageom.Cin * 4.0 + (fb ? act_bytes(tw.t[fb->in]) + grad_bytes(tw.t[fb->out]) : grad_bytes(y));
            continue;
        }
        p.wgrad = conv_resolve_wgrad(op.geom, p.st);
        p.wg_bytes = act_bytes(x) + grad_bytes(y) + wbytes;
        p.colsum = !op.bias_by_bn;
        if (!op.need_dx) continue;
        p.dgrad = conv_resolve_dgrad(op.geom, op.dgeom, p.st, op.wino_ud != nullptr);
        p.dg_bytes = grad_bytes(y) + grad_bytes(x) + wbytes;
        Op* bn = training && op.dy_to_bn >= 0 && e->stat_max > 0 ? &tw.ops[op.dy_to_bn] : nullptr;
        if (bn != nullptr && bn->fuse_pool >= 0 && (bn->xwin == nullptr || x.batch_stride != (int64_t)x.H * x.W * x.C)) bn = nullptr;
        if (bn == nullptr) continue;
        const bool bx = tw.t[bn->in].d_bf16;
        int blocks = -1;
        if (p.dgrad.path == DG_BF16_STORED && x.g_bf16 && bx && conv_bf16_halo_ok(op.dgeom)) blocks = conv_bf16_stat_blocks(op.dgeom);
        if (p.dgrad.path == DG_WINO && !x.g_bf16 && !bx && conv_wino_ok(op.dgeom)) blocks = conv_wino_stat_blocks(op.dgeom);
        if (blocks < 0) continue;
        if (!fits(op, blocks, op.dgeom.Cout)) return L3_ESTATE;
        p.bwd_bn = op.dy_to_bn;
        bn->bp.bwd_blocks = blocks;
    }
    for (auto& op : tw.ops) {
        if (op.kind != OP_BN) continue;
        const Tensor &x = tw.t[op.in], &y = tw.t[op.out];
        const Tensor& out = op.fuse_pool >= 0 ? tw.t[tw.ops[op.fuse_pool].out] : y;
        BnPlan& p = op.bp;
        p.stats = !training ? BS_MOVING : p.stat_blocks > 0 ? BS_PARTIALS : op.prerelu || x.d_bf16 ? BS_FAST : BS_PLAIN;
        p.bwd = training && op.fused_first ? BB_BY_FIRST_CONV : !bn_fast_ok(x.C) ? BB_PLAIN : op.fuse_pool >= 0 ? BB_FAST_POOLED
                : defers(op) ? BB_FAST_DEFERRED : BB_FAST;
        p.fwd_bytes = (!training ? 0.0 : p.stat_blocks > 0 ? (double)p.stat_blocks * 2 * x.C * 4 : act_bytes(x)) + act_bytes(x) + act_bytes(out);
        if (p.bwd == BB_BY_FIRST_CONV) p.fwd_bytes += act_bytes(x) + (double)x.rows() * (&op + 1)->ageom.Cin * 4.0;
        if (op.fuse_pool >= 0 && training && op.xwin != nullptr) p.fwd_bytes += (double)out.numel() * (x.d_bf16 ? 2.0 : 4.0);
        p.bwd_bytes = p.bwd == BB_PLAIN ? 2.0 * (act_bytes(x) + grad_bytes(y)) + grad_bytes(x)
                                        : (p.bwd_blocks > 0 ? (double)p.bwd_blocks * 2 * x.C * 4 : act_bytes(x) + grad_bytes(out)) +
                                              (p.bwd == BB_FAST_DEFERRED ? 0.0 : act_bytes(x) + grad_bytes(out) + grad_bytes(x));
    }
    return L3_OK;
}

void tower_forward(l3_engine* e, Tower& tw) {
    const bool training = tw.training;
    for (auto& op : tw.ops) {
        Tensor& x = tw.t[op.in];
        Tensor& y = tw.t[op.out];
        switch (op.kind) {
            case OP_CONV: {
                const ConvPlan& p = op.cp;
                ConvBufs b;
                b.x = x.d, b.w = e->params[op.p_kernel].d, b.bias = e->params[op.p_bias].d, b.y = y.d;
                b.wprep = op.wflip, b.wino_u = op.wino_uf;
                b.stat_part = p.stat_mode ? e->stat_scratch : nullptr, b.stat_mode = p.stat_mode;
                ProfScope ps(e, F_CONV_FWD, conv_flops(op.geom), op.name.c_str(), p.fwd.executed);
                ps.bytes(p.fwd_bytes);
                conv_run_fwd(p.fwd, op.geom, p.st, b, e->stream);
                break;
            }
            case OP_BN: {
                const BnPlan& p = op.bp;
                ProfScope ps(e, F_ELEMWISE, 0.0);
                ps.bytes(p.fwd_bytes);
                const float* gamma = e->params[op.p_gamma].d;
                const float* beta = e->params[op.p_beta].d;
                switch (p.stats) {
                    case BS_PARTIALS:
                        bn_stats_from_partials(e->stat_scratch, p.stat_blocks, e->params[op.bias_param].d, gamma, beta, op.mean, op.var,
                                               op.scale, op.shift, x.rows(), x.C, BN_EPS, op.prerelu ? 1 : 0, e->stream);
                        break;
                    case BS_FAST:
                        bn_stats_fast(x.d, gamma, beta, op.mean, op.var, op.scale, op.shift, e->red_scratch, x.rows(), x.C, BN_EPS,
                                      op.prerelu ? 1 : 0, e->stream, x.d_bf16 ? 1 : 0);
                        break;
                    case BS_PLAIN:
                        bn_stats(x.d, gamma, beta, op.mean, op.var, op.scale, op.shift, e->red_scratch, x.rows(), x.C, BN_EPS, e->stream);
                        break;
                    case BS_MOVING:
                        bn_scale_shift(gamma, beta, e->params[op.p_mmean].d, e->params[op.p_mvar].d, op.scale, op.shift, x.C, BN_EPS,
                                       e->stream);
                        break;
                }
                if (p.bwd == BB_BY_FIRST_CONV) bn_xhat_ones(x.d, op.mean, op.var, BN_EPS, (&op + 1)->xaug, x.rows(), x.C, e->stream);
                if (op.fuse_pool >= 0) {
                    Tensor& pl = tw.t[tw.ops[op.fuse_pool].out];
                    bn_relu_pool2_fwd(x.d, op.scale, op.shift, pl.d, x.N, x.H, x.W, x.C, pl.H, pl.W, pl.batch_stride,
                                      op.prerelu ? 2 : (op.fused_relu ? 1 : 0), e->stream, pl.d_bf16 ? 1 : 0, x.d_bf16 ? 1 : 0,
                                      training ? (void*)op.xwin : nullptr);
                } else if (y.d_bf16 || x.d_bf16) {
                    bn_apply_fast(x.d, op.scale, op.shift, y.d, x.rows(), x.C, op.fused_relu ? 1 : 0, e->stream, y.d_bf16 ? 1 : 0,
                                  x.d_bf16 ? 1 : 0);
                } else {
                    bn_apply(x.d, op.scale, op.shift, y.d, x.rows(), x.C, op.fused_relu ? 1 : 0, e->stream);
                }
                break;
            }
            case OP_RELU: {
                if (op.fused_into_bn) break;
                ProfScope ps(e, F_ELEMWISE, 0.0);
                ps.bytes(act_bytes(x) + act_bytes(y));
                relu_fwd(x.d, y.d, x.numel(), e->stream);
                break;
            }
            case OP_POOL: {
                if (op.fused_into_bn) break;
                ProfScope ps(e, F_ELEMWISE, 0.0);
                ps.bytes(act_bytes(x) + act_bytes(y));
                maxpool_fwd(x.d, y.d, op.pg, e->stream);
                break;
            }
            default: break;
        }
    }
}

BnBwdFuse bn_bwd_fuse(const Tower& tw, const Op& bn) {
    return BnBwdFuse{bn.fuse_pool >= 0 ? bn.xwin : tw.t[bn.in].d, bn.scale, bn.shift, bn.mean, bn.var, BN_EPS, bn.fused_relu ? 1 : 0};
}

void tower_backward_block(l3_engine* e, Tower& tw, int block) {
    const bool training = tw.training;
    for (int oi = (int)tw.ops.size() - 1; oi >= 0; --oi) {
        Op& op = tw.ops[oi];
        if (op.block != block) continue;
        Tensor& x = tw.t[op.in];
        Tensor& y = tw.t[op.out];
        switch (op.kind) {
            case OP_POOL: {
                if (op.fused_into_bn) break;
                ProfScope ps(e, F_ELEMWISE, 0.0);
                ps.bytes(act_bytes(x) + grad_bytes(y) + grad_bytes(x));
                maxpool_bwd(x.d, y.g, x.g, op.pg, e->stream);
                break;
            }
            case OP_RELU: {
                if (op.fused_into_bn) break;
                ProfScope ps(e, F_ELEMWISE, 0.0);
                ps.bytes(act_bytes(y) + grad_bytes(y) + grad_bytes(x));
                relu_bwd(y.d, y.g, x.g, x.numel(), e->stream);
                break;
            }
            case OP_BN: {
                const BnPlan& p = op.bp;
                if (p.bwd == BB_BY_FIRST_CONV) break;
                ProfScope ps(e, F_ELEMWISE, 0.0);
                ps.bytes(p.bwd_bytes);
                const float* mean = training ? op.mean : e->params[op.p_mmean].d;
                const float* var = training ? op.var : e->params[op.p_mvar].d;
                const float* gamma = e->params[op.p_gamma].d;
                float *dgamma = e->params[op.p_gamma].g, *dbeta = e->params[op.p_beta].g;
                if (p.bwd == BB_PLAIN) {
                    bn_bwd(x.d, y.d, y.g, gamma, mean, var, x.g, dgamma, dbeta, e->red_scratch, x.rows(), x.C, BN_EPS, op.fused_relu ? 1 : 0,
                           training ? 1 : 0, e->stream);
                    break;
                }
                const bool pooled = p.bwd == BB_FAST_POOLED, defer = p.bwd == BB_FAST_DEFERRED;
                const Tensor& dy = pooled ? tw.t[tw.ops[op.fuse_pool].out] : y;
                bn_bwd_fast(x.d, op.scale, op.shift, mean, var, gamma, dy.g, pooled ? 1 : 0, x.N, x.H, x.W, x.C, dy.H, dy.W,
                            pooled ? dy.batch_stride : (int64_t)x.H * x.W * x.C, defer ? nullptr : x.g, dgamma, dbeta,
                            defer ? nullptr : op.bias_param >= 0 ? e->params[op.bias_param].g : nullptr, e->red_scratch, BN_EPS,
                            pooled ? (op.prerelu ? 2 : 1) : (op.fused_relu ? 1 : 0), training ? 1 : 0, e->stream, x.g_bf16 ? 1 : 0,
                            x.d_bf16 ? 1 : 0, dy.g_bf16 ? 1 : 0, p.bwd_blocks > 0 ? e->stat_scratch : nullptr, p.bwd_blocks);
                break;
            }
            case OP_CONV: {
                const ConvPlan& p = op.cp;
                const float* w = e->params[op.p_kernel].d;
                if (p.aug != FW_NONE) {
                    ProfScope ps(e, F_CONV_WGRAD, conv_flops(op.geom), op.name.c_str());
                    ps.bytes(p.wg_bytes);
                    const Op& bn = tw.ops[op.in_bn];
                    if (p.aug == FW_AUG_DEFERRED) {
                        const Op& fb = tw.ops[op.bn_defer];
                        const Tensor &bi = tw.t[fb.in], &bo = tw.t[fb.out];
                        const float* co = bn_bwd_fast_coeffs(e->red_scratch, op.cout);
                        const FirstWgFuse f{bi.d, bo.g, fb.scale, fb.shift, co, co + op.cout, co + 2 * op.cout, fb.fused_relu ? 1 : 0,
                                            bi.d_bf16 ? 1 : 0};
                        conv_wgrad(op.xaug, nullptr, op.gaug, e->wg_scratch, op.ageom, e->stream, false, false, &f);
                    } else {
                        conv_wgrad(op.xaug, y.g, op.gaug, e->wg_scratch, op.ageom, e->stream);
                    }
                    first_conv_grads(op.gaug, w, e->params[bn.p_gamma].d, e->params[bn.p_beta].d, e->params[op.p_kernel].g,
                                     e->params[bn.p_gamma].g, e->params[bn.p_beta].g,
                                     op.bias_by_bn && p.aug == FW_AUG ? nullptr : e->params[op.p_bias].g, op.kh * op.kw, x.C, op.cout,
                                     e->stream);
                    break;
                }
                ConvBufs b;
                b.x = x.d, b.w = w, b.y = y.g, b.dx = x.g, b.dw = e->params[op.p_kernel].g;
                b.wprep = op.wflip, b.wino_u = op.wino_ud, b.wg_part = e->wg_scratch;
                {
                    ProfScope ps(e, F_CONV_WGRAD, conv_flops(op.geom), op.name.c_str(), p.wgrad.executed);
                    ps.bytes(p.wg_bytes);
                    conv_run_wgrad(p.wgrad, op.geom, b, e->stream);
                }
                if (p.colsum) {
                    ProfScope ps(e, F_ELEMWISE, 0.0);
                    ps.bytes(grad_bytes(y));
                    colsum(y.g, e->params[op.p_bias].g, e->red_scratch, y.rows(), y.C, e->stream);
                }
                if (p.dgrad.path == DG_NONE) break;
                ProfScope ps(e, F_CONV_DGRAD, conv_flops(op.geom), op.name.c_str(), p.dgrad.executed);
                ps.bytes(p.dg_bytes);
                BnBwdFuse bb{};
                if (p.bwd_bn >= 0) {
                    bb = bn_bwd_fuse(tw, tw.ops[p.bwd_bn]);
                    b.bn_bwd = &bb, b.stat_part = e->stat_scratch;
                }
                conv_run_dgrad(p.dgrad, op.geom, op.dgeom, p.st, b, e->stream);
                break;
            }
            default: break;
        }
    }
}

void l2_sums(l3_engine* e) {
    SumsqSegs segs{};
    int nl2 = 0;
    for (auto& s : e->segments) nl2 += s.l2 ? 1 : 0;
    if (nl2 <= SUMSQ_MAX_SEGS) {
        for (auto& s : e->segments)
            if (s.l2) {
                segs.off[segs.count] = s.off;
                segs.n[segs.count++] = s.n;
            }
        sumsq_multi(e->arena_p, segs, e->l2part, e->sq_scratch, e->stream);
        return;
    }
    int si = 0;
    for (auto& s : e->segments)
        if (s.l2) sumsq(e->arena_p + s.off, s.n, e->l2part + si++, e->sq_scratch, e->stream);
}

int forward_all(l3_engine* e, bool training) {
    int rc;
    e->fwd_done = false;
    e->results_global = false;
    if ((rc = plan_tower(e, e->vis, training, 0)) || (rc = plan_tower(e, e->aud, training, 0))) return rc;
    if (e->side && e->overlap) {
        HIPCHK(e, hipEventRecord(e->ev_fork, e->stream));
        HIPCHK(e, hipStreamWaitEvent(e->side, e->ev_fork, 0));
        l2_sums(e);
        {
            SideScope sd(e);
            if ((rc = run_frontend(e))) return rc;
            tower_forward(e, e->aud);
            HIPCHK(e, hipEventRecord(e->ev_join, e->stream));
        }
        tower_forward(e, e->vis);
        HIPCHK(e, hipStreamWaitEvent(e->stream, e->ev_join, 0));
    } else {
        l2_sums(e);
        if ((rc = run_frontend(e))) return rc;
        tower_forward(e, e->vis);
        tower_forward(e, e->aud);
    }
    ProfScope ps(e, F_HEAD, 0.0);
    const int D = e->nv + e->na;
    dense_fwd(e->h0, e->params[e->p_w1].d, e->params[e->p_b1].d, e->h1, e->B, D, e->head, 1, e->stream);
    dense_fwd(e->h1, e->params[e->p_w2].d, e->params[e->p_b2].d, e->logits, e->B, e->head, 2, 0, e->stream);
    e->last_training = training;
    return L3_OK;
}

void loss_and_head_backward(l3_engine* e, bool backward) {
    ProfScope ps(e, F_HEAD, 0.0);
    const int gb = e->cfg.global_batch > 0 ? e->cfg.global_batch : e->B;
    softmax_ce(e->logits, e->labels, e->probs, e->dlogits, e->stats, e->B, 1.0f / (float)gb, e->stream);
    if (!backward) return;
    const int D = e->nv + e->na;
    dense_bwd_w(e->h1, e->dlogits, e->params[e->p_w2].g, e->params[e->p_b2].g, e->B, e->head, 2, e->stream);
    dense_bwd_x(e->dlogits, e->params[e->p_w2].d, e->dh1, e->B, e->head, 2, e->stream);
    relu_bwd(e->h1, e->dh1, e->dh1, (int64_t)e->B * e->head, e->stream);
    dense_bwd_w(e->h0, e->dh1, e->params[e->p_w1].g, e->params[e->p_b1].g, e->B, D, e->head, e->stream);
    dense_bwd_x(e->dh1, e->params[e->p_w1].d, e->dh0, e->B, D, e->head, e->stream);
    if (e->side && e->overlap) {
        (void)hipEventRecord(e->ev_fork, e->stream);
        (void)hipStreamWaitEvent(e->side, e->ev_fork, 0);
    }
}

int backward_bucket(l3_engine* e, int bucket, bool join = true) {
    const int nbv = e->vis.nblocks, nba = e->aud.nblocks;
    if (bucket < 1 || bucket > nbv + nba) {
        e->err = "bucket out of range";
        return L3_EINVAL;
    }
    if (bucket <= nbv) {
        tower_backward_block(e, e->vis, nbv - bucket);
    } else if (e->side && e->overlap) {
        {
            SideScope sd(e);
            tower_backward_block(e, e->aud, nba - (bucket - nbv));
            HIPCHK(e, hipEventRecord(e->ev_join, e->stream));
            if (e->comm && (size_t)bucket < e->ev_bucket.size()) {
                HIPCHK(e, hipEventRecord(e->ev_bucket[bucket], e->stream));
                e->bucket_ready = bucket;
            }
        }
        if (join) HIPCHK(e, hipStreamWaitEvent(e->stream, e->ev_join, 0));
    } else {
        tower_backward_block(e, e->aud, nba - (bucket - nbv));
    }
    return L3_OK;
}

int ensure_bn_table(l3_engine* e) {
    if (e->bn_table != nullptr) return L3_OK;
    std::vector<BnMovingEntry> tab;
    int off = 0;
    for (Tower* tw : {&e->vis, &e->aud})
        for (auto& op : tw->ops)
            if (op.kind == OP_BN) {
                const int C = tw->t[op.in].C;
                tab.push_back(BnMovingEntry{e->params[op.p_mmean].d, op.biased_mean, op.mean, C, off});
                tab.push_back(BnMovingEntry{e->params[op.p_mvar].d, op.biased_var, op.var, C, off + C});
                off += 2 * C;
                e->bn_table_max_c = std::max(e->bn_table_max_c, C);
            }
    e->bn_table_n = (int)tab.size();
    e->bn_pack_floats = off;
    BnMovingEntry* dev = nullptr;
    if (int rc = dev_alloc_t(e, &dev, tab.size() + 1)) return rc;
    HIPCHK(e, hipMemcpy(dev, tab.data(), tab.size() * sizeof(BnMovingEntry), hipMemcpyHostToDevice));
    e->bn_table = dev;
    return L3_OK;
}

int bn_stats_pack(l3_engine* e, int world, int slot = -1) {
    int rc = ensure_bn_table(e);
    if (rc) return rc;
    if (e->bn_pack_floats == 0) return L3_OK;
    if (slot < 0 && e->bn_send == nullptr && (rc = dev_alloc_t(e, &e->bn_send, (size_t)e->bn_pack_floats))) return rc;
    if (e->bn_gathered_world < world) {
        if ((rc = dev_alloc_t(e, &e->bn_gathered, (size_t)e->bn_pack_floats * world))) return rc;
        e->bn_gathered_world = world;
    }
    bn_moving_pack(e->bn_table, e->bn_table_n, e->bn_table_max_c,
                   slot < 0 ? e->bn_send : e->bn_gathered + (size_t)slot * e->bn_pack_floats, e->stream);
    return L3_OK;
}

int do_update(l3_engine* e, float lr, float grad_scale) {
    {
        ProfScope ps(e, F_ADAM, 0.0);
        e->adam_t += 1;
        const double t = (double)e->adam_t;
        const float lr_t = lr * (sqrtf(1.f - powf(ADAM_B2, (float)t)) / (1.f - powf(ADAM_B1, (float)t)));
        for (size_t i = 0; i < e->segments.size(); ++i) {
            const auto& s = e->segments[i];
            int64_t n = s.n;
            const int64_t n_l2 = s.l2 ? s.n : 0;
            if (s.l2 && i + 1 < e->segments.size() && !e->segments[i + 1].l2 && e->segments[i + 1].off == s.off + s.n)
                n += e->segments[++i].n;
            adam_step(e->arena_p + s.off, e->arena_g + s.off, e->arena_m + s.off, e->arena_v + s.off, n, n_l2, 2.f * L2_WEIGHT,
                      lr_t, ADAM_B1, ADAM_B2, ADAM_EPS, grad_scale, e->stream);
        }
    }
    ProfScope ps(e, F_ELEMWISE, 0.0);
    int rc = ensure_bn_table(e);
    if (rc) return rc;
    const int replicas = e->bn_replicas_armed;
    e->bn_replicas_armed = 0;
    e->bn_step += replicas > 0 ? replicas : 1;
    bn_moving_update_all(e->bn_table, e->bn_table_n, e->bn_table_max_c, BN_MOMENTUM, e->cfg.bn_zero_debias, e->bn_step, e->stream,
                         replicas > 0 ? e->bn_gathered : nullptr, replicas, e->bn_pack_floats);
    return L3_OK;
}

int read_results(l3_engine* e, float* loss, float* acc, float* probs, float* logits) {
    HIPCHK(e, l3::stream_wait(e->stream));
    prof_collect(e);
    float st[16], l2[64];
    HIPCHK(e, hipMemcpy(st, e->stats, sizeof(st), hipMemcpyDeviceToHost));
    HIPCHK(e, hipMemcpy(l2, e->l2part, sizeof(l2), hipMemcpyDeviceToHost));
    double reg = 0.0;
    int si = 0;
    for (auto& s : e->segments)
        if (s.l2) reg += (double)L2_WEIGHT * (double)l2[si++];
    if (e->results_global) {
        if (probs || logits) {
            e->err = "probs / logits after a replicas step: the engine holds those of the last slice of " + std::to_string(e->B) +
                     " rows, not of the global batch of " + std::to_string(e->cfg.global_batch > 0 ? e->cfg.global_batch : e->B);
            return L3_ESTATE;
        }
        const double gb = (double)(e->cfg.global_batch > 0 ? e->cfg.global_batch : e->B);
        if (loss) *loss = (float)((double)st[0] / gb + reg);
        if (acc) *acc = (float)((double)st[1] / gb);
        return L3_OK;
    }
    if (loss) *loss = (float)((double)st[0] / (double)e->B + reg);
    if (acc) *acc = st[1] / (float)e->B;
    if (probs) HIPCHK(e, hipMemcpy(probs, e->probs, (size_t)e->B * 2 * 4, hipMemcpyDeviceToHost));
    if (logits) HIPCHK(e, hipMemcpy(logits, e->logits, (size_t)e->B * 2 * 4, hipMemcpyDeviceToHost));
    return L3_OK;
}

int upload_inputs(l3_engine* e, const float* video, const float* audio, const float* labels) {
    const int B = e->B;
    e->feed.inputs_replaced(BATCH_SINGLE);
    if (video) HIPCHK(e, hipMemcpyAsync(e->video, video, (size_t)B * 224 * 224 * 3 * 4, hipMemcpyHostToDevice, e->stream));
    if (audio) HIPCHK(e, hipMemcpyAsync(e->audio, audio, (size_t)B * AUDIO_T * 4, hipMemcpyHostToDevice, e->stream));
    if (labels) HIPCHK(e, hipMemcpyAsync(e->labels, labels, (size_t)B * 2 * 4, hipMemcpyHostToDevice, e->stream));
    HIPCHK(e, l3::stream_wait(e->stream));
    return L3_OK;
}

Tower* find_tower_tensor(l3_engine* e, const std::string& name, Tensor** out) {
    for (Tower* tw : {&e->vis, &e->aud}) {
        if (name == tw->prefix + "/input" || (tw == &e->aud && name == "audio_model/frontend")) {
            *out = &tw->t[0];
            return tw;
        }
        for (auto& op : tw->ops)
            if ((op.kind == OP_CONV || op.kind == OP_BN) && name == tw->prefix + "/" + op.name) {
                *out = &tw->t[op.out];
                return tw;
            }
    }
    return nullptr;
}

}

void l3::set_op_error(const std::string& msg) { g_create_error = msg; }

static void comm_release_events(l3_engine* e) {
    for (auto* vec : {&e->ev_bucket, &e->ev_ct0, &e->ev_ct1}) {
        for (auto ev : *vec)
            if (ev) (void)hipEventDestroy(ev);
        vec->clear();
    }
    for (hipEvent_t* ev : {&e->ev_comm_done, &e->ev_ct_ready, &e->ev_ct_done})
        if (*ev) {
            (void)hipEventDestroy(*ev);
            *ev = nullptr;
        }
    e->comm_timing = false;
    e->bucket_ready = -1;
    e->bn_replicas_armed = 0;
}

extern "C" {

const char* l3_last_error(const l3_engine* e) { return e ? e->err.c_str() : g_create_error.c_str(); }

int l3_device_count(void) {
    int n = 0;
    return hipGetDeviceCount(&n) == hipSuccess ? n : 0;
}
// ... 85 lines not shown
    rc = alloc_everything(e, seed);
    if (rc) return fail(rc);
    rc = rebuild_consts(e);
    if (rc) return fail(rc);
    *out = e;
    return L3_OK;
}

void l3_destroy(l3_engine* e) {
    if (!e) return;
    (void)hipSetDevice(e->cfg.device);
    if (e->stream) (void)l3::stream_wait(e->stream);
    e->feed.destroy();
    if (e->side) {
        (void)l3::stream_wait(e->side);
        (void)hipStreamDestroy(e->side);
        (void)hipEventDestroy(e->ev_fork);
        (void)hipEventDestroy(e->ev_join);
    }
    if (e->comm) {
        l3::comm_destroy(e->comm);
        e->comm = nullptr;
    }
    comm_release_events(e);
    for (auto ev : e->ev_res)
        if (ev) (void)hipEventDestroy(ev);
    if (e->ev_res_a) (void)hipEventDestroy(e->ev_res_a);
    if (e->ev_res_b) (void)hipEventDestroy(e->ev_res_b);
    for (auto ev : e->ev_step)
        if (ev) (void)hipEventDestroy(ev);
    if (e->res_host) (void)hipHostFree(e->res_host);
    e->bufs.clear();
    for (auto ev : e->ev_pool) (void)hipEventDestroy(ev);
    for (auto& r : e->prof_recs) {
        (void)hipEventDestroy(r.a);
        (void)hipEventDestroy(r.b);
    }
    if (e->own_stream && e->stream) (void)hipStreamDestroy(e->stream);
    delete e;
}

int l3_param_count(const l3_engine* e) { return e ? (int)e->params.size() : L3_EINVAL; }

int l3_param_info(const l3_engine* e, int index, char* name, int name_cap, int32_t* ndim, int64_t shape[4],
                  int32_t* trainable, int64_t* numel) {
    if (!e || index < 0 || index >= (int)e->params.size()) return L3_EINVAL;
    const Param& p = e->params[index];
    if (name && name_cap > 0) {
        strncpy(name, p.name.c_str(), name_cap - 1);
        name[name_cap - 1] = 0;
    }
    if (ndim) *ndim = p.ndim;
    if (shape)
        for (int i = 0; i < 4; ++i) shape[i] = i < p.ndim ? p.shape[i] : 1;
    if (trainable) *trainable = p.trainable ? 1 : 0;
    if (numel) *numel = p.numel;
    return L3_OK;
}

static int find_param(l3_engine* e, const char* name, int64_t numel, Param** out) {
    if (!e || !name) return L3_EINVAL;
    auto it = e->pindex.find(name);
    if (it == e->pindex.end()) {
        e->err = std::string("unknown parameter: ") + name;
        return L3_EINVAL;
    }
    Param& p = e->params[it->second];
    if (p.numel != numel) {
        e->err = std::string("size mismatch for ") + name + ": expected " + std::to_string(p.numel) + " got " +
                 std::to_string(numel);
        return L3_EINVAL;
    }
    *out = &p;
    return L3_OK;
}

int l3_set_param(l3_engine* e, const char* name, const float* src, int64_t numel) {
    Param* p;
    int rc = find_param(e, name, numel, &p);
    if (rc) return rc;
    HIPCHK(e, hipSetDevice(e->cfg.device));
    HIPCHK(e, l3::stream_wait(e->stream));
    HIPCHK(e, hipMemcpy(p->d, src, (size_t)numel * 4, hipMemcpyHostToDevice));
    if (p->kind == PK_CONST) e->consts_dirty = true;
    return L3_OK;
}

int l3_get_param(l3_engine* e, const char* name, float* dst, int64_t numel) {
    Param* p;
    int rc = find_param(e, name, numel, &p);
    if (rc) return rc;
    HIPCHK(e, hipSetDevice(e->cfg.device));
    HIPCHK(e, l3::stream_wait(e->stream));
    HIPCHK(e, hipMemcpy(dst, p->d, (size_t)numel * 4, hipMemcpyDeviceToHost));
    return L3_OK;
}

int l3_get_grad(l3_engine* e, const char* name, float* dst, int64_t numel) {
    Param* p;
    int rc = find_param(e, name, numel, &p);
    if (rc) return rc;
    if (!p->trainable) {
        e->err = std::string("not trainable: ") + name;
        return L3_EINVAL;
    }
    HIPCHK(e, hipSetDevice(e->cfg.device));
    HIPCHK(e, l3::stream_wait(e->stream));
    HIPCHK(e, hipMemcpy(dst, p->g, (size_t)numel * 4, hipMemcpyDeviceToHost));
    return L3_OK;
}

int l3_reset_optimizer(l3_engine* e) {
    if (!e) return L3_EINVAL;
    HIPCHK(e, hipSetDevice(e->cfg.device));
    HIPCHK(e, hipMemsetAsync(e->arena_m, 0, (size_t)e->n_train * 4, e->stream));
    HIPCHK(e, hipMemsetAsync(e->arena_v, 0, (size_t)e->n_train * 4, e->stream));
    e->adam_t = 0;
    e->bn_step = 0;
    for (Tower* tw : {&e->vis, &e->aud})
        for (auto& op : tw->ops)
            if (op.kind == OP_BN) {
                const size_t n = (size_t)(tw->t[op.in].C + 3) / 4 * 4 * 4;
                HIPCHK(e, hipMemsetAsync(op.biased_mean, 0, n, e->stream));
                HIPCHK(e, hipMemsetAsync(op.biased_var, 0, n, e->stream));
            }
    HIPCHK(e, l3::stream_wait(e->stream));
    return L3_OK;
}

int l3_copy_state(l3_engine* dst, l3_engine* src) {
    if (!dst || !src) return L3_EINVAL;
    if (dst == src) return L3_OK;
    if (dst->cfg.model_type != src->cfg.model_type || dst->params.size() != src->params.size() ||
        dst->n_train != src->n_train || dst->cfg.device != src->cfg.device) {
        dst->err = "l3_copy_state: engines differ in model type or device";
        return L3_EINVAL;
    }
    HIPCHK(dst, hipSetDevice(dst->cfg.device));
    HIPCHK(dst, l3::stream_wait(src->stream));
    if (src->side) HIPCHK(dst, l3::stream_wait(src->side));
    const size_t nb = (size_t)src->n_train * 4;
    HIPCHK(dst, hipMemcpyAsync(dst->arena_p, src->arena_p, nb, hipMemcpyDeviceToDevice, dst->stream));
    HIPCHK(dst, hipMemcpyAsync(dst->arena_m, src->arena_m, nb, hipMemcpyDeviceToDevice, dst->stream));
    HIPCHK(dst, hipMemcpyAsync(dst->arena_v, src->arena_v, nb, hipMemcpyDeviceToDevice, dst->stream));
    for (size_t i = 0; i < src->params.size(); ++i) {
        const Param& ps = src->params[i];
        if (ps.trainable) continue;
        HIPCHK(dst, hipMemcpyAsync(dst->params[i].d, ps.d, (size_t)ps.numel * 4, hipMemcpyDeviceToDevice, dst->stream));
    }
    Tower* dt[2] = {&dst->vis, &dst->aud};
    Tower* st[2] = {&src->vis, &src->aud};
    for (int t = 0; t < 2; ++t)
        for (size_t i = 0; i < st[t]->ops.size(); ++i) {
            const Op& so = st[t]->ops[i];
            Op& dop = dt[t]->ops[i];
            if (so.kind != OP_BN) continue;
            const size_t n = (size_t)(st[t]->t[so.in].C + 3) / 4 * 4 * 4;
            HIPCHK(dst, hipMemcpyAsync(dop.biased_mean, so.biased_mean, n, hipMemcpyDeviceToDevice, dst->stream));
            HIPCHK(dst, hipMemcpyAsync(dop.biased_var, so.biased_var, n, hipMemcpyDeviceToDevice, dst->stream));
        }
    dst->adam_t = src->adam_t;
    dst->bn_step = src->bn_step;
    dst->consts_dirty = true;
    HIPCHK(dst, l3::stream_wait(dst->stream));
    return L3_OK;
}

int l3_optimizer_steps(const l3_engine* e, int64_t* adam_t, int64_t* bn_steps) {
    if (!e) return L3_EINVAL;
    if (adam_t) *adam_t = e->adam_t;
    if (bn_steps) *bn_steps = e->bn_step;
    return L3_OK;
}

int l3_upload_batch(l3_engine* e, const float* video, const float* audio, const float* labels) {
    if (!e) return L3_EINVAL;
    HIPCHK(e, hipSetDevice(e->cfg.device));
    return upload_inputs(e, video, audio, labels);
}

int l3_upload_batch_raw(l3_engine* e, const uint8_t* video_u8, const int16_t* audio_i16, const int32_t* labels_i32) {
    if (!e) return L3_EINVAL;
    HIPCHK(e, hipSetDevice(e->cfg.device));
    return e->feed.upload(BATCH_SINGLE, 1, video_u8, audio_i16, labels_i32, nullptr, nullptr, e->stream, &e->err);
}

static int aug_prepare(l3_engine* e, const l3_augment_params* params, const double* u, int rows) {
    if (!params || !u) {
        e->err = "augmented batch without its parameter records or gain draws";
        return L3_EINVAL;
    }
    for (int i = 0; i < rows; ++i)
        if (params[i].start_x != 0 || params[i].start_y != 0) {
            e->err = "augmentation record " + std::to_string(i) + ": the engine's frames are 224 x 224, the crop must start at (0, 0)";
            return L3_EINVAL;
        }
    return L3_OK;
}

static int single_raw_aug(l3_engine* e, const char* name, bool stage, const uint8_t* video_u8, const int16_t* audio_i16,
                          const int32_t* labels_i32, const l3_augment_params* params, const double* u) {
    if (!e) return L3_EINVAL;
    if (!video_u8 || !audio_i16 || !labels_i32) {
        e->err = std::string(name) + ": NULL batch pointer";
        return L3_EINVAL;
    }
    HIPCHK(e, hipSetDevice(e->cfg.device));
    if (int rc = aug_prepare(e, params, u, e->B)) return rc;
    const AugmentParams* p = reinterpret_cast<const AugmentParams*>(params);
    return stage ? e->feed.stage(BATCH_SINGLE, 1, video_u8, audio_i16, labels_i32, p, u, &e->err)
                 : e->feed.upload(BATCH_SINGLE, 1, video_u8, audio_i16, labels_i32, p, u, e->stream, &e->err);
}

int l3_upload_batch_raw_aug(l3_engine* e, const uint8_t* video_u8, const int16_t* audio_i16, const int32_t* labels_i32,
                            const l3_augment_params* params, const double* u) {
    return single_raw_aug(e, "l3_upload_batch_raw_aug", false, video_u8, audio_i16, labels_i32, params, u);
}

int l3_stage_batch_raw(l3_engine* e, const uint8_t* video_u8, const int16_t* audio_i16, const int32_t* labels_i32) {
    if (!e || !video_u8 || !audio_i16 || !labels_i32) return L3_EINVAL;
    HIPCHK(e, hipSetDevice(e->cfg.device));
    return e->feed.stage(BATCH_SINGLE, 1, video_u8, audio_i16, labels_i32, nullptr, nullptr, &e->err);
}

int l3_stage_batch_raw_aug(l3_engine* e, const uint8_t* video_u8, const int16_t* audio_i16, const int32_t* labels_i32,
                           const l3_augment_params* params, const double* u) {
    return single_raw_aug(e, "l3_stage_batch_raw_aug", true, video_u8, audio_i16, labels_i32, params, u);
}

int l3_batch_gains(l3_engine* e, double* gains) {
    if (!e || !gains) return L3_EINVAL;
    if (!e->feed.gains_valid) {
        e->err = "l3_batch_gains: the current batch was not augmented";
        return L3_ESTATE;
    }
    HIPCHK(e, hipSetDevice(e->cfg.device));
    HIPCHK(e, l3::stream_wait(e->stream));
    HIPCHK(e, hipMemcpy(gains, e->feed.gains, (size_t)e->B * sizeof(double), hipMemcpyDeviceToHost));
    return L3_OK;
}

int l3_step_forward(l3_engine* e, int training) {
    if (!e) return L3_EINVAL;
    HIPCHK(e, hipSetDevice(e->cfg.device));
    e->bucket_ready = -1;
    e->bn_replicas_armed = 0;
    e->bn_packed = false;
    if (training) {
        const int slot = (int)(e->steps_enqueued & 1);
        if (e->ev_step_set[slot]) HIPCHK(e, l3::event_wait(e->ev_step[slot]));
    }
    int rc = e->feed.adopt(BATCH_SINGLE, e->stream, &e->err);
    if (rc) return rc;
    rc = forward_all(e, training != 0);
    if (rc) return rc;
    loss_and_head_backward(e, training != 0);
    e->fwd_done = true;
    HIPCHK(e, hipGetLastError());
    return L3_OK;
}

int l3_tower_step(l3_engine* e, int tower, int backward) {
    if (!e || (tower != 0 && tower != 1)) return L3_EINVAL;
    HIPCHK(e, hipSetDevice(e->cfg.device));
    int rc = e->feed.adopt(BATCH_SINGLE, e->stream, &e->err);
    if (rc) return rc;
    Tower& tw = tower == 0 ? e->vis : e->aud;
    if (tower == 1 && (rc = run_frontend(e))) return rc;
    if ((rc = plan_tower(e, tw, true, 1))) return rc;
    tower_forward(e, tw);
    if (backward) {
        const int width = tower == 0 ? e->nv : e->na;
        fill(e->dh0, 1.0f / ((float)e->B * (float)width), (int64_t)e->B * (e->nv + e->na), e->stream);
        for (int b = tw.nblocks - 1; b >= 0; --b) tower_backward_block(e, tw, b);
    }
    e->fwd_done = false;
    HIPCHK(e, hipGetLastError());
    return L3_OK;
}

int l3_step_bucket_count(const l3_engine* e) { return e ? (int)e->buckets.size() : L3_EINVAL; }

int l3_step_backward_bucket(l3_engine* e, int bucket) {
    if (!e) return L3_EINVAL;
    if (!e->fwd_done) {
        e->err = "l3_step_backward_bucket before l3_step_forward";
        return L3_ESTATE;
    }
    if (!e->last_training && e->cfg.dtype == L3_DTYPE_BF16) {
        e->err = "inference-mode gradients are available in L3_DTYPE_F32 engines only";
        return L3_ESTATE;
    }
    HIPCHK(e, hipSetDevice(e->cfg.device));
    int rc = backward_bucket(e, bucket);
    if (rc) return rc;
    HIPCHK(e, hipGetLastError());
    return L3_OK;
}

int l3_step_update(l3_engine* e, float lr, float grad_scale) {
    if (!e) return L3_EINVAL;
    if (!e->fwd_done || !e->last_training) {
        e->err = "l3_step_update without a training-mode forward";
        return L3_ESTATE;
    }
    HIPCHK(e, hipSetDevice(e->cfg.device));
    int rc = do_update(e, lr, grad_scale);
    e->fwd_done = false;
    if (rc) return rc;
    {
        const int slot = (int)(e->steps_enqueued & 1);
        if (e->ev_step[slot] == nullptr) HIPCHK(e, hipEventCreateWithFlags(&e->ev_step[slot], hipEventDisableTiming));
        HIPCHK(e, hipEventRecord(e->ev_step[slot], e->stream));
        e->ev_step_set[slot] = true;
        ++e->steps_enqueued;
    }
    HIPCHK(e, hipGetLastError());
    return L3_OK;
}

int l3_step_resident(l3_engine* e, float lr) {
    int rc = l3_step_forward(e, 1);
    if (rc) return rc;
    const int nb = (int)e->buckets.size();
    for (int b = 1; b < nb; ++b)
        if ((rc = l3_step_backward_bucket(e, b))) return rc;
    return l3_step_update(e, lr, 1.0f);
}

static int rep_refuse(l3_engine* e, const char* name, int replicas) {
    const int gb = e->cfg.global_batch > 0 ? e->cfg.global_batch : e->B;
    if (replicas < 1) {
        e->err = std::string(name) + ": replicas = " + std::to_string(replicas) + ", must be >= 1";
        return L3_EINVAL;
    }
    if ((int64_t)replicas * e->B != gb) {
        e->err = std::string(name) + ": " + std::to_string(replicas) + " replicas of batch " + std::to_string(e->B) + " are " +
                 std::to_string((int64_t)replicas * e->B) + " rows, the engine's global_batch is " + std::to_string(gb);
        return L3_EINVAL;
    }
    if (e->cfg.dp_moving == L3_DP_MOVING_RANK_LOCAL) {
        e->err = std::string(name) + ": dp_moving = L3_DP_MOVING_RANK_LOCAL (1) applies one moving-average update per step, " +
                 std::to_string(replicas) + " replicas apply " + std::to_string(replicas) + ": create the engine with L3_DP_MOVING_REPLICAS (0)";
        return L3_ESTATE;
    }
    if (e->comm) {
        e->err = std::string(name) + ": the engine holds a communicator of " + std::to_string(l3::comm_world(e->comm)) +
                 " ranks; its step is l3_step_dp (l3_comm_destroy first)";
        return L3_ESTATE;
    }
    return L3_OK;
}
// ... 465 lines not shown
    loss_and_head_backward(e, false);
    e->fwd_done = false;
    return read_results(e, loss, acc, nullptr, nullptr);
}

int l3_grad_arena_dev(l3_engine* e, void** dev_ptr, int64_t* numel) {
    if (!e) return L3_EINVAL;
    if (dev_ptr) *dev_ptr = e->arena_g;
    if (numel) *numel = e->n_train;
    return L3_OK;
}

int l3_bucket_range(const l3_engine* e, int bucket, int64_t* offset, int64_t* numel) {
    if (!e || bucket < 0 || bucket >= (int)e->buckets.size()) return L3_EINVAL;
    if (offset) *offset = e->buckets[bucket].off;
    if (numel) *numel = e->buckets[bucket].n;
    return L3_OK;
}

int64_t l3_embed_dim(const l3_engine* e, int vision, int pool_h, int pool_w) {
    if (!e) return L3_EINVAL;
    const Tower& tw = vision ? e->vis : e->aud;
    if (tw.emb_conv_op < 0 || pool_h < 1 || pool_w < 1) return L3_EINVAL;
    const Tensor& t = tw.t[tw.ops[tw.emb_conv_op].out];
    int ho, wo, p;
    tf_same(t.H, pool_h, pool_h, &ho, &p);
    tf_same(t.W, pool_w, pool_w, &wo, &p);
    return (int64_t)ho * wo * t.C;
}

struct EmbedSource {
    const float* host = nullptr;
    const float* samples = nullptr;
    const int64_t* table = nullptr;
};

constexpr size_t EMBED_OUT_BYTES = (size_t)256 << 20;

static int embed_check(l3_engine* e, bool vision, int ph, int pw, int64_t* D) {
    Tower& tw = vision ? e->vis : e->aud;
    if (tw.emb_conv_op < 0) {
        e->err = "model type has no embedding layer";
        return L3_EINVAL;
    }
    *D = l3_embed_dim(e, vision ? 1 : 0, ph, pw);
    if (*D < 0) {
        e->err = "bad pooling size";
        return L3_EINVAL;
    }
    return L3_OK;
}

static int embed_rows(l3_engine* e, bool vision, const EmbedSource& src, int64_t n, int ph, int pw, int64_t D, float* out) {
    Tower& tw = vision ? e->vis : e->aud;
    const int B = e->B;
    int64_t cap_rows = (int64_t)(EMBED_OUT_BYTES / ((size_t)D * 4)) / B * B;
    if (cap_rows < B) cap_rows = B;
    const int64_t need_rows = (n + B - 1) / B * B;
    if (cap_rows > need_rows) cap_rows = need_rows;
    int rc = dev_grow_t(e, &e->emb_out, &e->emb_out_cap, (size_t)cap_rows * D);
    if (rc) return rc;
    const Tensor& t = tw.t[tw.ops[tw.emb_conv_op].out];
    PoolGeom pg{};
    pg.N = B; pg.H = t.H; pg.W = t.W; pg.C = t.C; pg.ph = ph; pg.pw = pw; pg.sh = ph; pg.sw = pw;
    tf_same(t.H, ph, ph, &pg.Ho, &pg.padT);
    tf_same(t.W, pw, pw, &pg.Wo, &pg.padL);
    pg.out_batch_stride = D;
    const size_t per = vision ? (size_t)224 * 224 * 3 : (size_t)AUDIO_T;
    float* dst_in = vision ? e->video : e->audio;
    int64_t f0 = 0;
    for (int64_t s0 = 0; s0 < n; s0 += B) {
        const int64_t cnt = n - s0 < B ? n - s0 : B;
        if (src.host) {
            HIPCHK(e, hipMemcpyAsync(dst_in, src.host + (size_t)s0 * per, (size_t)cnt * per * 4, hipMemcpyHostToDevice, e->stream));
            if (cnt < B) HIPCHK(e, hipMemsetAsync(dst_in + (size_t)cnt * per, 0, (size_t)(B - cnt) * per * 4, e->stream));
        } else {
            gather_frames(src.samples, src.table + 3 * s0, dst_in, B, (int)cnt, AUDIO_T, e->stream);
        }
        if (!vision) {
            rc = run_frontend(e);
            if (rc) return rc;
        }
        if ((rc = plan_tower(e, tw, false, 1))) return rc;
        tower_forward(e, tw);
        maxpool_fwd(t.d, e->emb_out + (size_t)(s0 - f0) * D, pg, e->stream);
        if (s0 + cnt == n || s0 + 2 * B - f0 > cap_rows) {
            HIPCHK(e, hipMemcpyAsync(out + (size_t)f0 * D, e->emb_out, (size_t)(s0 + cnt - f0) * D * 4, hipMemcpyDeviceToHost, e->stream));
            HIPCHK(e, l3::stream_wait(e->stream));
            f0 = s0 + B;
        }
    }
    prof_collect(e);
    return L3_OK;
}

static int embed_common(l3_engine* e, bool vision, const float* in, int64_t n, int ph, int pw, float* out) {
    if (!e || !in || !out || n < 0) return L3_EINVAL;
    HIPCHK(e, hipSetDevice(e->cfg.device));
    int64_t D = 0;
    int rc = embed_check(e, vision, ph, pw, &D);
    if (rc) return rc;
    EmbedSource src;
    src.host = in;
    return embed_rows(e, vision, src, n, ph, pw, D, out);
}

int l3_embed_audio(l3_engine* e, const float* audio, int64_t n, int pool_h, int pool_w, float* out) {
    return embed_common(e, false, audio, n, pool_h, pool_w, out);
}
int l3_embed_vision(l3_engine* e, const float* video, int64_t n, int pool_h, int pool_w, float* out) {
    return embed_common(e, true, video, n, pool_h, pool_w, out);
}

int l3_embed_audio_frames(l3_engine* e, const float* samples, int64_t n_samples, const int64_t* table, int64_t n_frames,
                          int pool_h, int pool_w, float* out) {
    if (!e) return L3_EINVAL;
    if (!samples || !table || !out) {
        e->err = "l3_embed_audio_frames: samples, table and out must not be NULL";
        return L3_EINVAL;
    }
    if (n_samples < 0 || n_frames < 0) {
        e->err = "l3_embed_audio_frames: n_samples and n_frames must be >= 0";
        return L3_EINVAL;
    }
    int64_t D = 0;
    int rc = embed_check(e, false, pool_h, pool_w, &D);
    if (rc) return rc;
    int64_t bad = 0;
    if (const char* why = frame_table_error(table, n_frames, n_samples, &bad)) {
        e->err = std::string("l3_embed_audio_frames: frame ") + std::to_string(bad) + ": " + why;
        return L3_EINVAL;
    }
    if (n_frames == 0) return L3_OK;
    HIPCHK(e, hipSetDevice(e->cfg.device));
    if ((rc = dev_grow_t(e, &e->clip_samples, &e->clip_samples_cap, (size_t)n_samples))) return rc;
    if ((rc = dev_grow_t(e, &e->clip_table, &e->clip_table_cap, (size_t)n_frames * 3))) return rc;
    if (n_samples > 0)
        HIPCHK(e, hipMemcpyAsync(e->clip_samples, samples, (size_t)n_samples * 4, hipMemcpyHostToDevice, e->stream));
    HIPCHK(e, hipMemcpyAsync(e->clip_table, table, (size_t)n_frames * 3 * 8, hipMemcpyHostToDevice, e->stream));
    EmbedSource src;
    src.samples = e->clip_samples;
    src.table = e->clip_table;
    return embed_rows(e, false, src, n_frames, pool_h, pool_w, D, out);
}

int l3_embed_audio_clips_resampled(l3_engine* e, const float* native, int64_t n_native, const int64_t* clips, int64_t n_clips,
                                   const double* half_window, int64_t n_window, int num_table, int64_t n_samples,
                                   const int64_t* table, int64_t n_frames, int pool_h, int pool_w, float* out) {
    if (!e) return L3_EINVAL;
    if (!native || !clips || !half_window || !table || !out) {
        e->err = "l3_embed_audio_clips_resampled: native, clips, half_window, table and out must not be NULL";
        return L3_EINVAL;
    }
    if (n_native < 0 || n_clips < 0 || n_samples < 0 || n_frames < 0) {
        e->err = "l3_embed_audio_clips_resampled: n_native, n_clips, n_samples and n_frames must be >= 0";
        return L3_EINVAL;
    }
    int64_t D = 0;
    int rc = embed_check(e, false, pool_h, pool_w, &D);
    if (rc) return rc;
    int64_t bad = 0;
    if (const char* why = resample_clips_error(clips, n_clips, n_native, AUDIO_T, n_window, num_table, n_samples, true, &bad)) {
        e->err = std::string("l3_embed_audio_clips_resampled: ") + (bad >= 0 ? "clip " + std::to_string(bad) + ": " : std::string()) + why;
        return L3_EINVAL;
    }
    if (const char* why = frame_table_error(table, n_frames, n_samples, &bad)) {
// ... 129 lines not shown
```

### l3embedding_amd/csrc/kernels.h

```cpp
#pragma once
#include <hip/hip_runtime.h>
#include <stdint.h>

#include <string>
#include <vector>

#include "host_common.h"

namespace l3 {

struct ConvGeom {
    int N, H, W, Cin;
    int Ho, Wo, Cout;
    int KH, KW, padT, padL;
    int f2x2 = 0;
    int solo = 0;
    int dynamic = 0;
    float* tail_scratch = nullptr;
    size_t tail_scratch_bytes = 0;
};
size_t conv_wino4_tail_scratch_bytes();

struct BnBwdFuse {
    const float* x;
    const float *scale, *shift;
    const float *mean, *var;
    float eps;
    int relu;
};
void conv_fwd(const float* x, const float* w, const float* bias, float* y, const ConvGeom& g,
              hipStream_t s, const float* wino_u = nullptr, float* bn_part = nullptr, int bn_mode = 0,
              const BnBwdFuse* bn_bwd = nullptr);
bool conv_wino_ok(const ConvGeom& g);
size_t conv_wino_floats(const ConvGeom& g);
double conv_wino_executed_flops(const ConvGeom& g);
void conv_wino_transform_weights(const float* w, float* u, const ConvGeom& g, bool from_fwd_for_dgrad, hipStream_t s);
void conv_wino_fwd(const float* x, const float* u, const float* bias, float* y, const ConvGeom& g, hipStream_t s,
                   float* stat_part = nullptr, int stat_mode = 0, const BnBwdFuse* bn_bwd = nullptr);
int conv_wino_stat_blocks(const ConvGeom& g);
int conv_wino_stat_blocks_max(const ConvGeom& g);
bool conv_dgrad_small_ok(const ConvGeom& g);
bool conv_dgrad_small(const float* dy, const float* w, float* dx, const ConvGeom& g, hipStream_t s);
void conv_flip_weights(const float* w, float* wt, int KH, int KW, int Cin, int Cout, hipStream_t s);
size_t conv_wgrad_scratch_floats(const ConvGeom& g);
bool conv_wgrad_bf16_ok(const ConvGeom& g);
struct FirstWgFuse;
void conv_wgrad(const float* x, const float* dy, float* dw, float* part, const ConvGeom& g,
                hipStream_t s, bool bf16 = false, bool in_bf16 = false, const FirstWgFuse* first_fuse = nullptr);

bool conv_first_ok(const ConvGeom& g);
bool conv_first_wgrad_ok(const ConvGeom& g);
size_t conv_first_wgrad_scratch_floats(const ConvGeom& g);
struct FirstWgFuse {
    const void *bnx, *dA;
    const float *scale, *shift;
    const float *cA, *cB, *cC;
    int relu;
    int bf16;
};
int conv_first_wgrad(const float* x, const float* dy, float* part, const ConvGeom& g, hipStream_t s, const FirstWgFuse* fuse = nullptr);
int conv_first_stat_blocks(const ConvGeom& g);
void conv_first_fwd(const float* x, const float* w, const float* bias, void* y, const ConvGeom& g, hipStream_t s,
                    float* stat_part = nullptr, int stat_mode = 0, bool out_bf16 = false);

bool conv_wgrad_wino_ok(const ConvGeom& g);
int conv_wgrad_wino_splits(const ConvGeom& g, int n);
int conv_wgrad_wino_max_splits(const ConvGeom& g, int n);
double conv_wgrad_wino_executed_flops(const ConvGeom& g);
void conv_wgrad_wino_launch(const float* x, const float* dy, float* part, const ConvGeom& g, int n, hipStream_t s);
void conv_wgrad_wino_finish(const float* part, float* dw, const ConvGeom& g, int splits, hipStream_t s);
double conv_wgrad_executed_flops(const ConvGeom& g, bool bf16);
bool conv_wgrad_bf16_tr_enabled();
void conv_wgrad_bf16_tr_launch(const void* x, const void* dy, float* part, const ConvGeom& g, int n, int splits, hipStream_t s);

bool conv_bf16_ok(const ConvGeom& g);
void conv_bf16_fwd(const float* x, const float* wn, const float* bias, float* y, const ConvGeom& g, hipStream_t s,
                   bool operands_bf16 = false, float* stat_part = nullptr, int stat_mode = 0, bool out_bf16 = false,
                   const BnBwdFuse* bn_bwd = nullptr);
int conv_bf16_stat_blocks(const ConvGeom& g);
bool conv_bf16_halo_ok(const ConvGeom& g);
int conv_bf16_halo_patches(const ConvGeom& g, int n);
void conv_bf16_halo_launch(const void* x, const void* wn, const float* bias, void* y, const ConvGeom& g, int n,
                           hipStream_t s, float* stat_part, int stat_mode, bool out_bf16, const BnBwdFuse* bn_bwd = nullptr);
void conv_weights_bf16(const float* w, void* out, int KH, int KW, int Cin, int Cout, bool flip, hipStream_t s);

void bn_xhat_ones(const float* x, const float* mean, const float* var, float eps, float* xa, int64_t rows, int C,
                  hipStream_t s);
void first_conv_grads(const float* gaug, const float* w, const float* gamma, const float* beta, float* dw, float* dgamma,
                      float* dbeta, float* dbias, int taps, int C, int Co, hipStream_t s);

size_t colreduce_scratch_floats(int64_t rows, int C);
void colsum(const float* x, float* out, float* scratch, int64_t rows, int C, hipStream_t s);
void bn_stats(const float* x, const float* gamma, const float* beta, float* mean, float* var,
              float* scale, float* shift, float* scratch, int64_t rows, int C, float eps,
              hipStream_t s);
void bn_scale_shift(const float* gamma, const float* beta, const float* mean, const float* var,
                    float* scale, float* shift, int C, float eps, hipStream_t s);
void bn_apply(const float* x, const float* scale, const float* shift, float* y, int64_t rows, int C,
              int relu, hipStream_t s);
void bn_bwd(const float* x, const float* y, const float* dy, const float* gamma, const float* mean,
            const float* var, float* dx, float* dgamma, float* dbeta, float* scratch, int64_t rows,
            int C, float eps, int relu, int training, hipStream_t s);
void bn_moving_update(float* moving, float* biased, const float* batch, int C, float momentum,
                      int zero_debias, int step, hipStream_t s);
int* persistent_work_counters(hipStream_t s);

struct BnMovingEntry {
    float* moving;
    float* biased;
    const float* batch;
    int C;
    int off;
};
void bn_moving_update_all(const BnMovingEntry* tab_dev, int entries, int max_c, float momentum, int zero_debias, int64_t step,
                          hipStream_t s, const float* gathered = nullptr, int replicas = 1, int64_t stride = 0);
void bn_moving_pack(const BnMovingEntry* tab_dev, int entries, int max_c, float* packed, hipStream_t s);

bool bn_fast_ok(int C);
size_t bn_fast_scratch_floats(int C);
// ... 171 lines not shown
```

### l3embedding_amd/csrc/ops.hip

```cpp
#include <hip/hip_runtime.h>

#include <cstring>
#include <string>
#include <vector>

#include "../../include/l3hip.h"
#include "conv_path.h"
#include "kernels.h"
#include "knobs.h"
#include "mlp.h"
#include "vggish.h"

namespace {
using namespace l3;

struct Scope {
    DeviceBufs bufs;
    hipStream_t s = nullptr;
    bool ok = true;
    explicit Scope(int device) : ok(device_ok(device)) {}
    ~Scope() { (void)hipDeviceSynchronize(); }
    template <class T>
    T* alloc(size_t count) {
        T* p = bufs.alloc<T>(count);
// ... 49 lines not shown

extern "C" {

int l3_op_conv2d_fwd_dt(int device, int dtype, const float* x, const float* w, const float* b, float* y, int n, int h,
                        int wd, int cin, int cout, int kh, int kw, int same) {
    Scope sc(device);
    if (!sc.ok) return L3_EHIP;
    const ConvGeom g = make_geom(n, h, wd, cin, cout, kh, kw, same);
    const size_t nx = (size_t)n * h * wd * cin, nw = (size_t)kh * kw * cin * cout, ny = (size_t)n * g.Ho * g.Wo * cout;
    const bool stored = dtype == L3_OP_BF16_STORED || dtype == L3_OP_BF16_STORED_OUT;
    ConvStorage st;
    st.mixed = dtype != L3_DTYPE_F32;
    st.x_bf16 = stored && conv_bf16_ok(g);
    const ConvFwdPath p = conv_resolve_fwd(g, st, conv_wino_floats(g) != 0);
    st.y_bf16 = dtype == L3_OP_BF16_STORED_OUT && (p.path == CF_BF16_STORED || p.path == CF_FIRST);
    ConvBufs cb;
    float* d_x = sc.put(x, nx);
    cb.x = d_x;
    cb.w = sc.put(w, nw);
    cb.bias = b ? sc.put(b, (size_t)cout) : nullptr;
    cb.y = sc.alloc<float>(ny);
    cb.wprep = sc.alloc<float>(nw);
    cb.wino_u = p.wino_filter ? sc.alloc<float>(conv_wino_floats(g)) : nullptr;
    uint16_t* xb = st.x_bf16 ? sc.alloc<uint16_t>(nx) : nullptr;
    if (!sc.ok) return L3_ENOMEM;
    if (st.x_bf16) {
        cast_bf16(d_x, xb, (int64_t)nx, sc.s);
        cb.x = reinterpret_cast<const float*>(xb);
    }
    conv_run_fwd(p, g, st, cb, sc.s);
    sc.get_stored(y, cb.y, ny, st.y_bf16);
    return sc.status();
}

int l3_op_conv2d_fwd(int device, const float* x, const float* w, const float* b, float* y, int n, int h, int wd,
                     int cin, int cout, int kh, int kw, int same) {
    return l3_op_conv2d_fwd_dt(device, L3_DTYPE_F32, x, w, b, y, n, h, wd, cin, cout, kh, kw, same);
}

int l3_op_conv2d_bwd_dt(int device, int dtype, const float* x, const float* w, const float* dy, float* dx, float* dw,
                        float* db, int n, int h, int wd, int cin, int cout, int kh, int kw, int same) {
    Scope sc(device);
    if (!sc.ok) return L3_EHIP;
    const ConvGeom g = make_geom(n, h, wd, cin, cout, kh, kw, same), dg = conv_dgrad_geom(g);
    const size_t nx = (size_t)n * h * wd * cin, ny = (size_t)n * g.Ho * g.Wo * cout, nw = (size_t)kh * kw * cin * cout;
    const bool stored = (dtype == L3_OP_BF16_STORED || dtype == L3_OP_BF16_STORED_OUT) && conv_wgrad_bf16_ok(g) && conv_bf16_ok(dg);
    ConvStorage st;
    st.mixed = dtype != L3_DTYPE_F32;
    st.x_bf16 = st.dy_bf16 = stored;
    st.dx_bf16 = stored && dtype == L3_OP_BF16_STORED_OUT;
    const ConvWgradPath pw = conv_resolve_wgrad(g, st);
    const ConvDgradPath pd = conv_resolve_dgrad(g, dg, st, conv_wino_floats(dg) != 0);
    ConvBufs cb;
    float* d_x = sc.put(x, nx);
    float* d_dy = sc.put(dy, ny);
    cb.x = d_x;
    cb.y = d_dy;
    cb.w = sc.put(w, nw);
    cb.dx = sc.alloc<float>(nx);
    cb.dw = sc.alloc<float>(nw);
    cb.wprep = sc.alloc<float>(nw);
    cb.wino_u = pd.path == DG_WINO ? sc.alloc<float>(conv_wino_floats(dg)) : nullptr;
    cb.wg_part = sc.alloc<float>(conv_wgrad_scratch_floats(g));
    float* d_db = sc.alloc<float>((size_t)cout);
    float* d_red = sc.alloc<float>(colreduce_scratch_floats((int64_t)n * g.Ho * g.Wo, cout));
    uint16_t* xb = stored ? sc.alloc<uint16_t>(nx) : nullptr;
    uint16_t* gb = stored ? sc.alloc<uint16_t>(ny) : nullptr;
    if (!sc.ok) return L3_ENOMEM;
    if (stored) {
        cast_bf16(d_x, xb, (int64_t)nx, sc.s);
        cast_bf16(d_dy, gb, (int64_t)ny, sc.s);
        cb.x = reinterpret_cast<const float*>(xb);
        cb.y = reinterpret_cast<float*>(gb);
    }
    conv_run_wgrad(pw, g, cb, sc.s);
    colsum(d_dy, d_db, d_red, (int64_t)n * g.Ho * g.Wo, cout, sc.s);
    conv_run_dgrad(pd, g, dg, st, cb, sc.s);
    sc.get_stored(dx, cb.dx, nx, st.dx_bf16);
    sc.get(dw, cb.dw, nw);
    sc.get(db, d_db, (size_t)cout);
    return sc.status();
}

int l3_op_conv2d_bwd(int device, const float* x, const float* w, const float* dy, float* dx, float* dw, float* db,
                     int n, int h, int wd, int cin, int cout, int kh, int kw, int same) {
    return l3_op_conv2d_bwd_dt(device, L3_DTYPE_F32, x, w, dy, dx, dw, db, n, h, wd, cin, cout, kh, kw, same);
}

int l3_op_bn_relu_fwd(int device, const float* x, const float* gamma, const float* beta, float* y, float* mean,
                      float* var, int64_t rows, int c, int relu, int x_bf16) {
    Scope sc(device);
    if (!sc.ok) return L3_EHIP;
    if ((x_bf16 & 1) && !bn_fast_ok(c)) return L3_EINVAL;
    const size_t n = (size_t)rows * c, cp = (size_t)(c + 3) / 4 * 4;
    float* d_x = sc.put(x, n);
    float* d_g = sc.alloc<float>(cp);
    float* d_b = sc.alloc<float>(cp);
    float *d_m = sc.alloc<float>(cp), *d_v = sc.alloc<float>(cp), *d_sc = sc.alloc<float>(cp), *d_sh = sc.alloc<float>(cp);
    float* d_y = sc.alloc<float>(n);
    float* d_red = sc.alloc<float>(colreduce_scratch_floats(rows, c));
    if (!sc.ok) return L3_ENOMEM;
    (void)hipMemcpy(d_g, gamma, c * 4, hipMemcpyHostToDevice);
    (void)hipMemcpy(d_b, beta, c * 4, hipMemcpyHostToDevice);
    if (x_bf16 & 1) {
        uint16_t* xb = sc.alloc<uint16_t>(n);
        if (!sc.ok) return L3_ENOMEM;
        cast_bf16(d_x, xb, (int64_t)n, sc.s);
        bn_stats_fast(reinterpret_cast<const float*>(xb), d_g, d_b, d_m, d_v, d_sc, d_sh, d_red, rows, c, 1e-3f, 0, sc.s, 1);
        bn_apply_fast(reinterpret_cast<const float*>(xb), d_sc, d_sh, d_y, rows, c, relu, sc.s, 0, 1);
    } else {
        bn_stats(d_x, d_g, d_b, d_m, d_v, d_sc, d_sh, d_red, rows, c, 1e-3f, sc.s);
        bn_apply(d_x, d_sc, d_sh, d_y, rows, c, relu, sc.s);
    }
    sc.get(y, d_y, n);
    sc.get(mean, d_m, (size_t)c);
    sc.get(var, d_v, (size_t)c);
    return sc.status();
}

int l3_op_bn_relu_bwd(int device, const float* x, const float* y, const float* dy, const float* gamma,
                      const float* beta, const float* mean, const float* var, float* dx, float* dgamma, float* dbeta,
                      int64_t rows, int c, int relu, int x_bf16) {
    Scope sc(device);
    if (!sc.ok) return L3_EHIP;
    const size_t n = (size_t)rows * c, cp = (size_t)(c + 3) / 4 * 4;
    float* d_x = sc.put(x, n);
    float* d_y = sc.put(y, n);
    float* d_dy = sc.put(dy, n);
    float *d_g = sc.alloc<float>(cp), *d_m = sc.alloc<float>(cp), *d_v = sc.alloc<float>(cp);
    float *d_dg = sc.alloc<float>(cp), *d_db = sc.alloc<float>(cp);
    float* d_dx = sc.alloc<float>(n);
    const bool fast = beta != nullptr && bn_fast_ok(c) && rows < (int64_t)1 << 30;
    if (x_bf16 && !fast) return L3_EINVAL;
    size_t red = colreduce_scratch_floats(rows, c);
    if (fast && bn_fast_scratch_floats(c) > red) red = bn_fast_scratch_floats(c);
    float* d_red = sc.alloc<float>(red);
    if (!sc.ok) return L3_ENOMEM;
    (void)hipMemcpy(d_g, gamma, c * 4, hipMemcpyHostToDevice);
    (void)hipMemcpy(d_m, mean, c * 4, hipMemcpyHostToDevice);
    (void)hipMemcpy(d_v, var, c * 4, hipMemcpyHostToDevice);
    if (fast) {
        float *d_b = sc.put(beta, (size_t)c), *d_sc = sc.alloc<float>(cp), *d_sh = sc.alloc<float>(cp);
        if (!sc.ok) return L3_ENOMEM;
        bn_scale_shift(d_g, d_b, d_m, d_v, d_sc, d_sh, c, 1e-3f, sc.s);
        const float* xin = d_x;
        const float* dyin = d_dy;
        if (x_bf16 & 1) {
            uint16_t* xb = sc.alloc<uint16_t>(n);
            if (!sc.ok) return L3_ENOMEM;
            cast_bf16(d_x, xb, (int64_t)n, sc.s);
            xin = reinterpret_cast<const float*>(xb);
        }
        if (x_bf16 & 2) {
            uint16_t* gb = sc.alloc<uint16_t>(n);
            if (!sc.ok) return L3_ENOMEM;
            cast_bf16(d_dy, gb, (int64_t)n, sc.s);
            dyin = reinterpret_cast<const float*>(gb);
        }
        bn_bwd_fast(xin, d_sc, d_sh, d_m, d_v, d_g, dyin, 0, 1, 1, (int)rows, c, 1, (int)rows, (int64_t)rows * c, d_dx, d_dg,
                    d_db, nullptr, d_red, 1e-3f, relu, 1, sc.s, 0, (x_bf16 & 1) ? 1 : 0, (x_bf16 & 2) ? 1 : 0);
    } else {
        bn_bwd(d_x, d_y, d_dy, d_g, d_m, d_v, d_dx, d_dg, d_db, d_red, rows, c, 1e-3f, relu, 1, sc.s);
    }
    sc.get(dx, d_dx, n);
    sc.get(dgamma, d_dg, (size_t)c);
    sc.get(dbeta, d_db, (size_t)c);
// ... 762 lines not shown
```

Measured before the change: 1997 pairs/s.

## Batch Winograd weight transforms into one launch after optimizer step with epoch caching

Adds a single batched kernel that computes the forward and dgrad Winograd weight operands for all eligible 3x3 conv layers. It runs right after the Adam step, so the tower passes can skip the per-layer transform launches. A weight epoch counter marks cached operands stale whenever weights change through set_param, copy_state or an optimizer step. The flip and bf16 weight preparation moves into shared prepare helpers, and the dgrad path gets its own flip buffer. This removes many small kernel launches and re-reads of each weight tensor per step, at the cost of extra memory for the operand buffers and some bookkeeping complexity.

```diff
diff --git a/include/l3hip.h b/include/l3hip.h
--- a/include/l3hip.h
+++ b/include/l3hip.h
@@ -62,6 +62,8 @@
 int l3_reset_optimizer(l3_engine *e);
 int l3_copy_state(l3_engine *dst, l3_engine *src);
 int l3_optimizer_steps(const l3_engine *e, int64_t *adam_t, int64_t *bn_steps);
+int l3_weight_operand_launches(const l3_engine *e, int64_t *batched, int64_t *per_layer);
+int l3_weight_operands_prepared(const l3_engine *e, int64_t *fwd, int64_t *dgrad);
 
 int l3_forward(l3_engine *e, const float *video, const float *audio, int training,
                float *probs, float *logits);
@@ -150,6 +152,8 @@
                         float *dw, float *db, int n, int h, int wd, int cin, int cout, int kh, int kw, int same);
 int l3_op_conv2d_fwd(int device, const float *x, const float *w, const float *b, float *y,
                      int n, int h, int wd, int cin, int cout, int kh, int kw, int same);
+int l3_op_weight_operands(int device, int layers, const int32_t *cin, const int32_t *cout, const float *w, float *uf, float *ud,
+                          float *uf_ref, float *ud_ref, int32_t *kind_fwd, int32_t *kind_dgrad);
 int l3_op_conv2d_bwd(int device, const float *x, const float *w, const float *dy,
                      float *dx, float *dw, float *db,
                      int n, int h, int wd, int cin, int cout, int kh, int kw, int same);
diff --git a/l3embedding_amd/_build.py b/l3embedding_amd/_build.py
--- a/l3embedding_amd/_build.py
+++ b/l3embedding_amd/_build.py
@@ -8,7 +8,7 @@
 OBJDIR = os.path.join(LIBDIR, 'obj')
 LIBPATH = os.path.join(LIBDIR, 'libl3hip.so')
 SOURCES = ['conv.hip', 'conv_wino.hip', 'conv_wino4.hip', 'conv_bf16.hip', 'conv_bf16_halo.hip', 'conv_wgrad_bf16.hip', 'conv_wgrad_wino.hip',
-           'conv_first.hip', 'conv_path.hip', 'elementwise.hip', 'bn_fused.hip', 'frontend.hip', 'clips.hip', 'resample.hip', 'batch_feed.hip', 'engine.hip', 'ops.hip',
+           'conv_first.hip', 'conv_path.hip', 'conv_weight_ops.hip', 'elementwise.hip', 'bn_fused.hip', 'frontend.hip', 'clips.hip', 'resample.hip', 'batch_feed.hip', 'engine.hip', 'ops.hip',
            'comm.hip', 'mlp.hip', 'svm.hip', 'vggish.hip', 'augment.hip', 'featprep.hip', 'svm_eval.hip', 'forest.hip']
 EXPERIMENT_SOURCES = ['conv_wino_bx6.hip', 'conv_wgrad_bx6.hip']
 EXPERIMENTS = os.environ.get('L3_BUILD_EXPERIMENTS') == '1'
diff --git a/l3embedding_amd/_lib.py b/l3embedding_amd/_lib.py
--- a/l3embedding_amd/_lib.py
+++ b/l3embedding_amd/_lib.py
@@ -65,6 +65,8 @@
     'l3_reset_optimizer': (C.c_int, [C.c_void_p]),
     'l3_copy_state': (C.c_int, [C.c_void_p, C.c_void_p]),
     'l3_optimizer_steps': (C.c_int, [C.c_void_p, C.POINTER(C.c_int64), C.POINTER(C.c_int64)]),
+    'l3_weight_operand_launches': (C.c_int, [C.c_void_p, C.POINTER(C.c_int64), C.POINTER(C.c_int64)]),
+    'l3_weight_operands_prepared': (C.c_int, [C.c_void_p, C.POINTER(C.c_int64), C.POINTER(C.c_int64)]),
     'l3_forward': (C.c_int, [C.c_void_p, C.c_void_p, C.c_void_p, C.c_int, C.c_void_p, C.c_void_p]),
     'l3_train_step': (C.c_int, [C.c_void_p, C.c_void_p, C.c_void_p, C.c_void_p, C.c_float,
                                 C.POINTER(C.c_float), C.POINTER(C.c_float)]),
@@ -122,6 +124,7 @@
     'l3_op_conv2d_fwd': (C.c_int, [C.c_int, C.c_void_p, C.c_void_p, C.c_void_p, C.c_void_p] + [C.c_int] * 8),
     'l3_op_conv2d_fwd_dt': (C.c_int, [C.c_int, C.c_int, C.c_void_p, C.c_void_p, C.c_void_p, C.c_void_p] + [C.c_int] * 8),
     'l3_op_conv2d_bwd_dt': (C.c_int, [C.c_int, C.c_int] + [C.c_void_p] * 6 + [C.c_int] * 8),
+    'l3_op_weight_operands': (C.c_int, [C.c_int, C.c_int] + [C.c_void_p] * 9),
     'l3_op_conv2d_bwd': (C.c_int, [C.c_int] + [C.c_void_p] * 6 + [C.c_int] * 8),
     'l3_op_bn_relu_fwd': (C.c_int, [C.c_int] + [C.c_void_p] * 6 + [C.c_int64, C.c_int, C.c_int, C.c_int]),
     'l3_op_bn_relu_bwd': (C.c_int, [C.c_int] + [C.c_void_p] * 10 + [C.c_int64, C.c_int, C.c_int, C.c_int]),
@@ -407,6 +410,16 @@
         check(self.lib.l3_optimizer_steps(self.h, C.byref(t), C.byref(b)), self.h)
         return t.value, b.value
 
+    def weight_operand_launches(self):
+        b, p = C.c_int64(), C.c_int64()
+        check(self.lib.l3_weight_operand_launches(self.h, C.byref(b), C.byref(p)), self.h)
+        return b.value, p.value
+
+    def weight_operands_prepared(self):
+        f, d = C.c_int64(), C.c_int64()
+        check(self.lib.l3_weight_operands_prepared(self.h, C.byref(f), C.byref(d)), self.h)
+        return f.value, d.value
+
     def forward(self, video, audio, training=False):
         v, a = _f32(video), _f32(audio)
         assert v.shape[0] == self.batch and a.shape[0] == self.batch
@@ -671,6 +684,29 @@
     else:
         check(lib.l3_op_conv2d_fwd(device, _ptr(x), _ptr(w), _ptr(b), _ptr(y), n, h, wd, cin, cout, kh, kw, int(same)))
     return y
+
+
+def op_weight_operands(weights, device=0):
+    lib = load()
+    ws = [_f32(w) for w in weights]
+    assert all(w.ndim == 4 and w.shape[:2] == (3, 3) for w in ws)
+    n = len(ws)
+    cin = np.array([w.shape[2] for w in ws], np.int32)
+    cout = np.array([w.shape[3] for w in ws], np.int32)
+    flat = np.concatenate([w.ravel() for w in ws])
+    sizes = [36 * int(a) * int(b) for a, b in zip(cin, cout)]
+    outs = [np.empty(sum(sizes), np.float32) for _ in range(4)]
+    kf, kd = np.zeros(n, np.int32), np.zeros(n, np.int32)
+    check(lib.l3_op_weight_operands(device, n, _ptr(cin), _ptr(cout), _ptr(flat), _ptr(outs[0]), _ptr(outs[1]), _ptr(outs[2]),
+                                    _ptr(outs[3]), _ptr(kf), _ptr(kd)))
+    res, off = [], 0
+    for i in range(n):
+        nf, nd = (36 if kf[i] == 1 else 16) * sizes[i] // 36, (36 if kd[i] == 1 else 16) * sizes[i] // 36
+        res.append({'kind_fwd': int(kf[i]), 'kind_dgrad': int(kd[i]),
+                    'fwd': outs[0][off:off + nf].copy(), 'dgrad': outs[1][off:off + nd].copy(),
+                    'fwd_ref': outs[2][off:off + nf].copy(), 'dgrad_ref': outs[3][off:off + nd].copy()})
+        off += sizes[i]
+    return res
 
 
 def op_conv2d_bwd(x, w, dy, same, device=0, dtype='f32'):
diff --git a/l3embedding_amd/csrc/conv_path.h b/l3embedding_amd/csrc/conv_path.h
--- a/l3embedding_amd/csrc/conv_path.h
+++ b/l3embedding_amd/csrc/conv_path.h
@@ -31,6 +31,19 @@
 ConvWgradPath conv_resolve_wgrad(const ConvGeom& g, const ConvStorage& st);
 ConvDgradPath conv_resolve_dgrad(const ConvGeom& g, const ConvGeom& dg, const ConvStorage& st, bool have_u);
 
+enum ConvWeightKind {
+    WK_NONE,
+    WK_WINO_F4,
+    WK_WINO_F2,
+    WK_WINO_BX6,
+    WK_FLIPPED,
+    WK_BF16_FWD,
+    WK_BF16_DGRAD
+};
+ConvWeightKind conv_weight_kind_fwd(const ConvFwdPath& p, const ConvGeom& g);
+ConvWeightKind conv_weight_kind_dgrad(const ConvDgradPath& p, const ConvGeom& g, const ConvGeom& dg);
+inline bool conv_weight_kind_is_wino(ConvWeightKind k) { return k == WK_WINO_F4 || k == WK_WINO_F2 || k == WK_WINO_BX6; }
+
 struct ConvBufs {
     const float* x = nullptr;
     const float* w = nullptr;
@@ -46,6 +59,10 @@
     int stat_mode = 0;
     const BnBwdFuse* bn_bwd = nullptr;
 };
+void conv_prepare_fwd(const ConvFwdPath& p, const ConvGeom& g, const ConvBufs& b, hipStream_t s);
+void conv_prepare_dgrad(const ConvDgradPath& p, const ConvGeom& g, const ConvGeom& dg, const ConvBufs& b, hipStream_t s);
+int conv_weight_op_kind(ConvWeightKind k);
+bool conv_prepare_batched(const WeightOpLayer* host_table, const WeightOpLayer* dev_table, int layers, hipStream_t s);
 void conv_run_fwd(const ConvFwdPath& p, const ConvGeom& g, const ConvStorage& st, const ConvBufs& b, hipStream_t s);
 void conv_run_wgrad(const ConvWgradPath& p, const ConvGeom& g, const ConvBufs& b, hipStream_t s);
 void conv_run_dgrad(const ConvDgradPath& p, const ConvGeom& g, const ConvGeom& dg, const ConvStorage& st, const ConvBufs& b, hipStream_t s);
diff --git a/l3embedding_amd/csrc/conv_path.hip b/l3embedding_amd/csrc/conv_path.hip
--- a/l3embedding_amd/csrc/conv_path.hip
+++ b/l3embedding_amd/csrc/conv_path.hip
@@ -47,15 +47,78 @@
     return p;
 }
 
+static ConvWeightKind wino_kind(const ConvGeom& g) {
+    const int algo = conv_wino_algo(g);
+    return algo == 2 ? WK_WINO_BX6 : algo == 1 ? WK_WINO_F4 : WK_WINO_F2;
+}
+
+ConvWeightKind conv_weight_kind_fwd(const ConvFwdPath& p, const ConvGeom& g) {
+    switch (p.path) {
+        case CF_BF16_STORED: return WK_BF16_FWD;
+        case CF_BF16_CAST: return WK_FLIPPED;
+        case CF_FIRST: return WK_NONE;
+        case CF_FP32: return p.wino_filter ? wino_kind(g) : WK_NONE;
+    }
+    return WK_NONE;
+}
+
+ConvWeightKind conv_weight_kind_dgrad(const ConvDgradPath& p, const ConvGeom& g, const ConvGeom& dg) {
+    (void)g;
+    switch (p.path) {
+        case DG_BF16_STORED: return WK_BF16_DGRAD;
+        case DG_WINO: return wino_kind(dg);
+        case DG_FLIPPED: return WK_FLIPPED;
+        case DG_NONE:
+        case DG_SMALL:
+        case DG_BF16_CAST: return WK_NONE;
+    }
+    return WK_NONE;
+}
+
+void conv_prepare_fwd(const ConvFwdPath& p, const ConvGeom& g, const ConvBufs& b, hipStream_t s) {
+    switch (conv_weight_kind_fwd(p, g)) {
+        case WK_WINO_F4:
+        case WK_WINO_F2:
+        case WK_WINO_BX6: conv_wino_transform_weights(b.w, b.wino_u, g, false, s); break;
+        case WK_BF16_FWD: conv_weights_bf16(b.w, b.wprep, g.KH, g.KW, g.Cin, g.Cout, true, s); break;
+        case WK_FLIPPED: conv_flip_weights(b.w, b.wprep, g.KH, g.KW, g.Cin, g.Cout, s); break;
+        default: break;
+    }
+}
+
+void conv_prepare_dgrad(const ConvDgradPath& p, const ConvGeom& g, const ConvGeom& dg, const ConvBufs& b, hipStream_t s) {
+    switch (conv_weight_kind_dgrad(p, g, dg)) {
+        case WK_WINO_F4:
+        case WK_WINO_F2:
+        case WK_WINO_BX6:
+            conv_wino_transform_weights(b.w, b.wino_u, dg, true, s);
+            break;
+        case WK_BF16_DGRAD: conv_weights_bf16(b.w, b.wprep, g.KH, g.KW, g.Cin, g.Cout, false, s); break;
+        case WK_FLIPPED: conv_flip_weights(b.w, b.wprep, g.KH, g.KW, g.Cin, g.Cout, s); break;
+        default: break;
+    }
+}
+
+int conv_weight_op_kind(ConvWeightKind k) { return k == WK_WINO_F4 ? WEIGHT_OP_F4 : k == WK_WINO_F2 ? WEIGHT_OP_F2 : WEIGHT_OP_NONE; }
+
+bool conv_prepare_batched(const WeightOpLayer* host_table, const WeightOpLayer* dev_table, int layers, hipStream_t s) {
+    int blocks = 0;
+    for (int i = 0; i < layers; ++i) {
+        const WeightOpLayer& l = host_table[i];
+        if (!weight_operands_layer_ok(l) || l.first_block != blocks) return false;
+        blocks += weight_operands_blocks(l.Cin, l.Cout);
+    }
+    weight_operands_launch(dev_table, layers, blocks, s);
+    return true;
+}
+
 void conv_run_fwd(const ConvFwdPath& p, const ConvGeom& g, const ConvStorage& st, const ConvBufs& b, hipStream_t s) {
-    if (p.wino_filter && !b.u_ready) conv_wino_transform_weights(b.w, b.wino_u, g, false, s);
+    if (!b.u_ready) conv_prepare_fwd(p, g, b, s);
     switch (p.path) {
         case CF_BF16_STORED:
-            conv_weights_bf16(b.w, b.wprep, g.KH, g.KW, g.Cin, g.Cout, true, s);
             conv_bf16_fwd(b.x, b.wprep, b.bias, b.y, g, s, true, b.stat_part, b.stat_mode, st.y_bf16);
             break;
         case CF_BF16_CAST:
-            conv_flip_weights(b.w, b.wprep, g.KH, g.KW, g.Cin, g.Cout, s);
             conv_bf16_fwd(b.x, b.wprep, b.bias, b.y, g, s);
             break;
         case CF_FIRST:
@@ -72,23 +135,21 @@
 }
 
 void conv_run_dgrad(const ConvDgradPath& p, const ConvGeom& g, const ConvGeom& dg, const ConvStorage& st, const ConvBufs& b, hipStream_t s) {
+    if (!b.u_ready) conv_prepare_dgrad(p, g, dg, b, s);
     switch (p.path) {
         case DG_SMALL:
             (void)conv_dgrad_small(b.y, b.w, b.dx, g, s);
             break;
         case DG_BF16_STORED:
-            conv_weights_bf16(b.w, b.wprep, g.KH, g.KW, g.Cin, g.Cout, false, s);
             conv_bf16_fwd(b.y, b.wprep, nullptr, b.dx, dg, s, true, b.stat_part, 0, st.dx_bf16, b.bn_bwd);
             break;
         case DG_BF16_CAST:
             conv_bf16_fwd(b.y, b.w, nullptr, b.dx, dg, s);
             break;
         case DG_WINO:
-            conv_wino_transform_weights(b.w, b.wino_u, dg, true, s);
             conv_fwd(b.y, nullptr, nullptr, b.dx, dg, s, b.wino_u, b.stat_part, 0, b.bn_bwd);
             break;
         case DG_FLIPPED:
-            conv_flip_weights(b.w, b.wprep, g.KH, g.KW, g.Cin, g.Cout, s);
             conv_fwd(b.y, b.wprep, nullptr, b.dx, dg, s);
             break;
         case DG_NONE: break;
diff --git a/l3embedding_amd/csrc/conv_weight_ops.hip b/l3embedding_amd/csrc/conv_weight_ops.hip
--- /dev/null
+++ b/l3embedding_amd/csrc/conv_weight_ops.hip
@@ -0,0 +1,150 @@
+#include <mutex>
+
+#include "device_common.h"
+#include "kernels.h"
+
+namespace l3 {
+namespace {
+
+constexpr int WO_TILE = 64;
+constexpr int WO_LD = WO_TILE + 1;
+constexpr int WO_LDS_BYTES = 9 * WO_TILE * WO_LD * (int)sizeof(float);
+
+__device__ __forceinline__ void gmul4(float a0, float a1, float a2, float* o) {
+    const float s02 = a0 + a2;
+    o[0] = a0;
+    o[1] = (-1.f / 3.f) * (s02 + a1);
+    o[2] = (1.f / 3.f) * (s02 - a1);
+    o[3] = (1.f / 15.f) * fmaf(2.f, a1, fmaf(4.f, a2, a0));
+    o[4] = (-4.f / 15.f) * fmaf(-2.f, a1, fmaf(4.f, a0, a2));
+    o[5] = a2;
+}
+
+__device__ __forceinline__ void xform4(const float* g, float* u) {
+    float gg[6][3];
+#pragma unroll
+    for (int kw = 0; kw < 3; ++kw) {
+        float o[6];
+        gmul4(g[kw], g[3 + kw], g[6 + kw], o);
+#pragma unroll
+        for (int xi = 0; xi < 6; ++xi) gg[xi][kw] = o[xi];
+    }
+#pragma unroll
+    for (int xi = 0; xi < 6; ++xi) {
+        float o[6];
+        gmul4(gg[xi][0], gg[xi][1], gg[xi][2], o);
+#pragma unroll
+        for (int nu = 0; nu < 6; ++nu) u[xi * 6 + nu] = o[nu];
+    }
+}
+
+__device__ __forceinline__ void xform2(const float* g, float* u) {
+    float gg[4][3];
+#pragma unroll
+    for (int kw = 0; kw < 3; ++kw) {
+        gg[0][kw] = g[kw];
+        gg[1][kw] = 0.5f * (g[kw] + g[3 + kw] + g[6 + kw]);
+        gg[2][kw] = 0.5f * (g[kw] - g[3 + kw] + g[6 + kw]);
+        gg[3][kw] = g[6 + kw];
+    }
+#pragma unroll
+    for (int xi = 0; xi < 4; ++xi) {
+        u[xi * 4 + 0] = gg[xi][0];
+        u[xi * 4 + 1] = 0.5f * (gg[xi][0] + gg[xi][1] + gg[xi][2]);
+        u[xi * 4 + 2] = 0.5f * (gg[xi][0] - gg[xi][1] + gg[xi][2]);
+        u[xi * 4 + 3] = gg[xi][2];
+    }
+}
+
+template <bool DGRAD>
+__device__ __forceinline__ void emit_operand(const float* taps, float* __restrict__ u, int kind, int cN, int kN, int c0, int k0) {
+    const int t = threadIdx.x;
+#pragma unroll 1
+    for (int j = 0; j < 4; ++j) {
+        const int item = t + 256 * j, kl = item & 63, cl = (item >> 6) * 4;
+        const int c = c0 + cl, k = k0 + kl;
+        if (c >= cN || k >= kN) continue;
+        auto load = [&](int ci, float* g) {
+#pragma unroll
+            for (int tap = 0; tap < 9; ++tap)
+                g[tap] = DGRAD ? taps[((8 - tap) * WO_TILE + kl) * WO_LD + cl + ci] : taps[(tap * WO_TILE + cl + ci) * WO_LD + kl];
+        };
+        if (kind == WEIGHT_OP_F4) {
+            const int c8 = c >> 3, hf = (c >> 2) & 1;
+#pragma unroll
+            for (int sub = 0; sub < 2; ++sub) {
+                float g[9], ua[36], ub[36];
+                load(2 * sub, g);
+                xform4(g, ua);
+                load(2 * sub + 1, g);
+                xform4(g, ub);
+#pragma unroll
+                for (int pos = 0; pos < 36; ++pos) {
+                    const size_t at = (((((size_t)pos * (cN >> 3) + c8) * 2 + sub) * 2 + hf) * kN + k) * 2;
+                    *reinterpret_cast<float2*>(u + at) = make_float2(ua[pos], ub[pos]);
+                }
+            }
+        } else {
+            float g[9], u0[16], u1[16], u2[16], u3[16];
+            load(0, g);
+            xform2(g, u0);
+            load(1, g);
+            xform2(g, u1);
+            load(2, g);
+            xform2(g, u2);
+            load(3, g);
+            xform2(g, u3);
+#pragma unroll
+            for (int pos = 0; pos < 16; ++pos) {
+                const size_t at = (((size_t)pos * (cN >> 2) + (c >> 2)) * kN + k) * 4;
+                *reinterpret_cast<float4*>(u + at) = make_float4(u0[pos], u1[pos], u2[pos], u3[pos]);
+            }
+        }
+    }
+}
+
+__global__ __launch_bounds__(256) void weight_operands_kernel(const WeightOpLayer* __restrict__ table, int layers) {
+    extern __shared__ __attribute__((aligned(16))) float taps[];
+    int li = 0;
+    while (li + 1 < layers && (int)blockIdx.x >= table[li + 1].first_block) ++li;
+    const WeightOpLayer L = table[li];
+    const int b = (int)blockIdx.x - L.first_block;
+    const int tiles_k = (L.Cout + WO_TILE - 1) / WO_TILE;
+    const int ci0 = (b / tiles_k) * WO_TILE, co0 = (b % tiles_k) * WO_TILE;
+    if (ci0 >= L.Cin) return;
+    const int t = threadIdx.x, col = t & 63, row0 = t >> 6;
+    const bool col_in = co0 + col < L.Cout;
+#pragma unroll 1
+    for (int tap = 0; tap < 9; ++tap)
+#pragma unroll 4
+        for (int i = 0; i < 16; ++i) {
+            const int row = row0 + 4 * i, ci = ci0 + row;
+            taps[(tap * WO_TILE + row) * WO_LD + col] = col_in && ci < L.Cin ? L.w[((size_t)tap * L.Cin + ci) * L.Cout + co0 + col] : 0.f;
+        }
+    __syncthreads();
+    if (L.kind_fwd != WEIGHT_OP_NONE) emit_operand<false>(taps, L.u_fwd, L.kind_fwd, L.Cin, L.Cout, ci0, co0);
+    if (L.kind_dgrad != WEIGHT_OP_NONE) emit_operand<true>(taps, L.u_dgrad, L.kind_dgrad, L.Cout, L.Cin, co0, ci0);
+}
+
+}
+
+int weight_operands_blocks(int Cin, int Cout) { return ((Cin + WO_TILE - 1) / WO_TILE) * ((Cout + WO_TILE - 1) / WO_TILE); }
+
+bool weight_operands_layer_ok(const WeightOpLayer& l) {
+    auto ok = [](int kind, int c) { return kind == WEIGHT_OP_NONE || (kind == WEIGHT_OP_F4 ? c % 8 == 0 : kind == WEIGHT_OP_F2 && c % 4 == 0); };
+    return l.Cin > 0 && l.Cout > 0 && ok(l.kind_fwd, l.Cin) && ok(l.kind_dgrad, l.Cout) && (l.kind_fwd == WEIGHT_OP_NONE || l.u_fwd != nullptr) &&
+           (l.kind_dgrad == WEIGHT_OP_NONE || l.u_dgrad != nullptr) && l.w != nullptr;
+}
+
+void weight_operands_launch(const WeightOpLayer* dev_table, int layers, int blocks, hipStream_t s) {
+    if (layers <= 0 || blocks <= 0) return;
+    static std::once_flag once[L3_MAX_DEVICES];
+    int dev = 0;
+    (void)hipGetDevice(&dev);
+    std::call_once(once[dev & (L3_MAX_DEVICES - 1)], [] {
+        (void)hipFuncSetAttribute((const void*)weight_operands_kernel, hipFuncAttributeMaxDynamicSharedMemorySize, WO_LDS_BYTES);
+    });
+    hipLaunchKernelGGL(weight_operands_kernel, dim3(blocks), dim3(256), WO_LDS_BYTES, s, dev_table, layers);
+}
+
+}
diff --git a/l3embedding_amd/csrc/conv_wino.hip b/l3embedding_amd/csrc/conv_wino.hip
--- a/l3embedding_amd/csrc/conv_wino.hip
+++ b/l3embedding_amd/csrc/conv_wino.hip
@@ -328,6 +328,7 @@
 static bool use_wino4(const ConvGeom& g) { return !use_bx6(g) && conv_wino_ok(g) && conv_wino4_selected(g); }
 
 bool conv_wino_is_bx6(const ConvGeom& g) { return use_bx6(g); }
+int conv_wino_algo(const ConvGeom& g) { return use_bx6(g) ? 2 : use_wino4(g) ? 1 : 0; }
 
 double conv_wino_executed_flops(const ConvGeom& g) {
     if (use_bx6(g)) return conv_wino_bx6_executed_flops(g);
diff --git a/l3embedding_amd/csrc/engine.hip b/l3embedding_amd/csrc/engine.hip
--- a/l3embedding_amd/csrc/engine.hip
+++ b/l3embedding_amd/csrc/engine.hip
@@ -1,10 +1,12 @@
 #include <hip/hip_runtime.h>
 #include "knobs.h"
 
+#include <algorithm>
 #include <cmath>
 #include <cstdio>
 #include <cstdlib>
 #include <cstring>
+#include <initializer_list>
 #include <map>
 #include <string>
 #include <vector>
@@ -62,6 +64,7 @@
     ConvWgradPath wgrad;
     bool colsum = false;
     ConvDgradPath dgrad;
+    ConvWeightKind wk_fwd = WK_NONE, wk_dgrad = WK_NONE;
     int bwd_bn = -1;
     double fwd_bytes = 0.0, wg_bytes = 0.0, dg_bytes = 0.0;
 };
@@ -87,6 +90,9 @@
     int p_kernel = -1, p_bias = -1;
     float* wflip = nullptr;
     float *wino_uf = nullptr, *wino_ud = nullptr;
+    float* wflip_d = nullptr;
+    int64_t uf_epoch = -1, ud_epoch = -1;
+    ConvWeightKind uf_kind = WK_NONE, ud_kind = WK_NONE;
     int in_bn = -1;
     bool fused_first = false;
     bool defer_apply = false;
@@ -163,6 +169,13 @@
     std::vector<Bucket> buckets;
     int64_t adam_t = 0;
     int64_t bn_step = 0;
+    int64_t w_epoch = 0;
+    std::vector<l3::WeightOpLayer> wop_host;
+    l3::WeightOpLayer* wop_dev = nullptr;
+    size_t wop_dev_cap = 0;
+    bool wop_cached = true;
+    int64_t wop_batched = 0, wop_per_layer = 0;
+    int64_t wop_fwd_ops = 0, wop_dgrad_ops = 0;
 
     Tower vis, aud;
     FrontendDef fe{};
@@ -896,6 +909,7 @@
         }
         HIPCHK(e, hipMemcpy(p.d, h.data(), (size_t)p.numel * 4, hipMemcpyHostToDevice));
     }
+    ++e->w_epoch;
     const FrontendCfg& f = e->fcfg;
     if ((rc = dev_alloc_t(e, &e->wdft, (size_t)f.n_dft * f.ncols_pad))) return rc;
     {
@@ -1018,6 +1032,8 @@
                 if (op.need_dx && conv_wino_floats(op.dgeom) &&
                     (rc = dev_alloc_t(e, &op.wino_ud, conv_wino_floats(op.dgeom))))
                     return rc;
+                op.wflip_d = op.wflip;
+                if (op.need_dx && e->cfg.dtype == L3_DTYPE_BF16 && (rc = dev_alloc_t(e, &op.wflip_d, (size_t)e->params[op.p_kernel].numel))) return rc;
                 const size_t w = conv_wgrad_scratch_floats(op.geom);
                 if (w > wg_max) wg_max = w;
                 if (op.in_bn >= 0) {
@@ -1151,6 +1167,7 @@
         ConvPlan& p = op.cp = ConvPlan{};
         p.st = ConvStorage{bf16, x.d_bf16, y.d_bf16, y.g_bf16, x.g_bf16};
         p.fwd = conv_resolve_fwd(op.geom, p.st, op.wino_uf != nullptr);
+        p.wk_fwd = conv_weight_kind_fwd(p.fwd, op.geom);
         p.fwd_bytes = act_bytes(x) + act_bytes(y) + wbytes;
         const int nblk = p.fwd.path == CF_BF16_STORED ? conv_bf16_stat_blocks(op.geom)
                          : p.fwd.path == CF_FIRST     ? conv_first_stat_blocks(op.geom)
@@ -1171,6 +1188,7 @@
         p.colsum = !op.bias_by_bn;
         if (!op.need_dx) continue;
         p.dgrad = conv_resolve_dgrad(op.geom, op.dgeom, p.st, op.wino_ud != nullptr);
+        p.wk_dgrad = conv_weight_kind_dgrad(p.dgrad, op.geom, op.dgeom);
         p.dg_bytes = grad_bytes(y) + grad_bytes(x) + wbytes;
         Op* bn = training && op.dy_to_bn >= 0 && e->stat_max > 0 ? &tw.ops[op.dy_to_bn] : nullptr;
         if (bn != nullptr && bn->fuse_pool >= 0 && (bn->xwin == nullptr || x.batch_stride != (int64_t)x.H * x.W * x.C)) bn = nullptr;
@@ -1202,6 +1220,68 @@
     return L3_OK;
 }
 
+static bool fwd_operand_current(const l3_engine* e, const Op& op) {
+    return e->wop_cached && op.cp.wk_fwd != WK_NONE && op.uf_epoch == e->w_epoch && op.uf_kind == op.cp.wk_fwd;
+}
+static bool dgrad_operand_current(const l3_engine* e, const Op& op) {
+    return e->wop_cached && op.cp.wk_dgrad != WK_NONE && op.ud_epoch == e->w_epoch && op.ud_kind == op.cp.wk_dgrad;
+}
+
+int ensure_weight_operands(l3_engine* e, std::initializer_list<Tower*> towers, bool dgrad) {
+    e->wop_cached = knob_int("L3_WEIGHT_OPS_CACHE", 1) != 0;
+    if (!e->wop_cached) return L3_OK;
+    std::vector<l3::WeightOpLayer> tab;
+    int blocks = 0;
+    for (Tower* tw : towers)
+        for (auto& op : tw->ops) {
+            if (op.kind != OP_CONV) continue;
+            const ConvPlan& p = op.cp;
+            const bool do_f = p.wk_fwd != WK_NONE && !fwd_operand_current(e, op);
+            const bool do_d = dgrad && p.wk_dgrad != WK_NONE && !dgrad_operand_current(e, op);
+            if (!do_f && !do_d) continue;
+            const float* w = e->params[op.p_kernel].d;
+            l3::WeightOpLayer l{w, op.wino_uf, op.wino_ud, op.geom.Cin, op.geom.Cout, do_f ? conv_weight_op_kind(p.wk_fwd) : WEIGHT_OP_NONE,
+                                do_d ? conv_weight_op_kind(p.wk_dgrad) : WEIGHT_OP_NONE, blocks};
+            if (l.kind_fwd != WEIGHT_OP_NONE || l.kind_dgrad != WEIGHT_OP_NONE) {
+                tab.push_back(l);
+                blocks += weight_operands_blocks(l.Cin, l.Cout);
+            }
+            ConvBufs b;
+            b.w = w;
+            if (do_f && l.kind_fwd == WEIGHT_OP_NONE) {
+                b.wprep = op.wflip, b.wino_u = op.wino_uf;
+                conv_prepare_fwd(p.fwd, op.geom, b, e->stream);
+                ++e->wop_per_layer;
+            }
+            if (do_d && l.kind_dgrad == WEIGHT_OP_NONE) {
+                b.wprep = op.wflip_d, b.wino_u = op.wino_ud;
+                conv_prepare_dgrad(p.dgrad, op.geom, op.dgeom, b, e->stream);
+                ++e->wop_per_layer;
+            }
+            if (do_f) op.uf_epoch = e->w_epoch, op.uf_kind = p.wk_fwd, ++e->wop_fwd_ops;
+            if (do_d) op.ud_epoch = e->w_epoch, op.ud_kind = p.wk_dgrad, ++e->wop_dgrad_ops;
+        }
+    if (tab.empty()) return L3_OK;
+    const size_t nb = tab.size() * sizeof(l3::WeightOpLayer);
+    auto same = [](const l3::WeightOpLayer& a, const l3::WeightOpLayer& b) {
+        return a.w == b.w && a.u_fwd == b.u_fwd && a.u_dgrad == b.u_dgrad && a.Cin == b.Cin && a.Cout == b.Cout && a.kind_fwd == b.kind_fwd &&
+               a.kind_dgrad == b.kind_dgrad && a.first_block == b.first_block;
+    };
+    if (tab.size() != e->wop_host.size() || !std::equal(tab.begin(), tab.end(), e->wop_host.begin(), same)) {
+        int rc = dev_grow_t(e, &e->wop_dev, &e->wop_dev_cap, tab.size());
+        if (rc) return rc;
+        HIPCHK(e, hipMemcpyAsync(e->wop_dev, tab.data(), nb, hipMemcpyHostToDevice, e->stream));
+        HIPCHK(e, l3::stream_wait(e->stream));
+        e->wop_host = tab;
+    }
+    if (!conv_prepare_batched(e->wop_host.data(), e->wop_dev, (int)e->wop_host.size(), e->stream)) {
+        e->err = "ensure_weight_operands: a layer's channel counts do not fit its Winograd operand layout";
+        return L3_ESTATE;
+    }
+    ++e->wop_batched;
+    return L3_OK;
+}
+
 void tower_forward(l3_engine* e, Tower& tw) {
     const bool training = tw.training;
     for (auto& op : tw.ops) {
@@ -1213,6 +1293,8 @@
                 ConvBufs b;
                 b.x = x.d, b.w = e->params[op.p_kernel].d, b.bias = e->params[op.p_bias].d, b.y = y.d;
                 b.wprep = op.wflip, b.wino_u = op.wino_uf;
+                b.u_ready = fwd_operand_current(e, op);
+                if (!b.u_ready && p.wk_fwd != WK_NONE) ++e->wop_per_layer, ++e->wop_fwd_ops, op.uf_epoch = -1;
                 b.stat_part = p.stat_mode ? e->stat_scratch : nullptr, b.stat_mode = p.stat_mode;
                 ProfScope ps(e, F_CONV_FWD, conv_flops(op.geom), op.name.c_str(), p.fwd.executed);
                 ps.bytes(p.fwd_bytes);
@@ -1349,7 +1431,9 @@
                 }
                 ConvBufs b;
                 b.x = x.d, b.w = w, b.y = y.g, b.dx = x.g, b.dw = e->params[op.p_kernel].g;
-                b.wprep = op.wflip, b.wino_u = op.wino_ud, b.wg_part = e->wg_scratch;
+                b.wprep = op.wflip_d, b.wino_u = op.wino_ud, b.wg_part = e->wg_scratch;
+                b.u_ready = dgrad_operand_current(e, op);
+                if (!b.u_ready && p.wk_dgrad != WK_NONE) ++e->wop_per_layer, ++e->wop_dgrad_ops, op.ud_epoch = -1;
                 {
                     ProfScope ps(e, F_CONV_WGRAD, conv_flops(op.geom), op.name.c_str(), p.wgrad.executed);
                     ps.bytes(p.wg_bytes);
@@ -1399,6 +1483,7 @@
     e->fwd_done = false;
     e->results_global = false;
     if ((rc = plan_tower(e, e->vis, training, 0)) || (rc = plan_tower(e, e->aud, training, 0))) return rc;
+    if ((rc = ensure_weight_operands(e, {&e->vis, &e->aud}, training))) return rc;
     if (e->side && e->overlap) {
         HIPCHK(e, hipEventRecord(e->ev_fork, e->stream));
         HIPCHK(e, hipStreamWaitEvent(e->side, e->ev_fork, 0));
@@ -1518,6 +1603,7 @@
             adam_step(e->arena_p + s.off, e->arena_g + s.off, e->arena_m + s.off, e->arena_v + s.off, n, n_l2, 2.f * L2_WEIGHT,
                       lr_t, ADAM_B1, ADAM_B2, ADAM_EPS, grad_scale, e->stream);
         }
+        ++e->w_epoch;
     }
     ProfScope ps(e, F_ELEMWISE, 0.0);
     int rc = ensure_bn_table(e);
@@ -1527,7 +1613,7 @@
     e->bn_step += replicas > 0 ? replicas : 1;
     bn_moving_update_all(e->bn_table, e->bn_table_n, e->bn_table_max_c, BN_MOMENTUM, e->cfg.bn_zero_debias, e->bn_step, e->stream,
                          replicas > 0 ? e->bn_gathered : nullptr, replicas, e->bn_pack_floats);
-    return L3_OK;
+    return ensure_weight_operands(e, {&e->vis, &e->aud}, true);
 }
 
 int read_results(l3_engine* e, float* loss, float* acc, float* probs, float* logits) {
@@ -1779,6 +1865,7 @@
     HIPCHK(e, hipSetDevice(e->cfg.device));
     HIPCHK(e, l3::stream_wait(e->stream));
     HIPCHK(e, hipMemcpy(p->d, src, (size_t)numel * 4, hipMemcpyHostToDevice));
+    ++e->w_epoch;
     if (p->kind == PK_CONST) e->consts_dirty = true;
     return L3_OK;
 }
@@ -1858,8 +1945,23 @@
         }
     dst->adam_t = src->adam_t;
     dst->bn_step = src->bn_step;
+    ++dst->w_epoch;
     dst->consts_dirty = true;
     HIPCHK(dst, l3::stream_wait(dst->stream));
+    return L3_OK;
+}
+
+int l3_weight_operand_launches(const l3_engine* e, int64_t* batched, int64_t* per_layer) {
+    if (!e) return L3_EINVAL;
+    if (batched) *batched = e->wop_batched;
+    if (per_layer) *per_layer = e->wop_per_layer;
+    return L3_OK;
+}
+
+int l3_weight_operands_prepared(const l3_engine* e, int64_t* fwd, int64_t* dgrad) {
+    if (!e) return L3_EINVAL;
+    if (fwd) *fwd = e->wop_fwd_ops;
+    if (dgrad) *dgrad = e->wop_dgrad_ops;
     return L3_OK;
 }
 
@@ -1965,6 +2067,7 @@
     Tower& tw = tower == 0 ? e->vis : e->aud;
     if (tower == 1 && (rc = run_frontend(e))) return rc;
     if ((rc = plan_tower(e, tw, true, 1))) return rc;
+    if ((rc = ensure_weight_operands(e, {&tw}, backward != 0))) return rc;
     tower_forward(e, tw);
     if (backward) {
         const int width = tower == 0 ? e->nv : e->na;
@@ -2596,6 +2699,7 @@
             if (rc) return rc;
         }
         if ((rc = plan_tower(e, tw, false, 1))) return rc;
+        if ((rc = ensure_weight_operands(e, {&tw}, false))) return rc;
         tower_forward(e, tw);
         maxpool_fwd(t.d, e->emb_out + (size_t)(s0 - f0) * D, pg, e->stream);
         if (s0 + cnt == n || s0 + 2 * B - f0 > cap_rows) {
diff --git a/l3embedding_amd/csrc/kernels.h b/l3embedding_amd/csrc/kernels.h
--- a/l3embedding_amd/csrc/kernels.h
+++ b/l3embedding_amd/csrc/kernels.h
@@ -35,6 +35,18 @@
 size_t conv_wino_floats(const ConvGeom& g);
 double conv_wino_executed_flops(const ConvGeom& g);
 void conv_wino_transform_weights(const float* w, float* u, const ConvGeom& g, bool from_fwd_for_dgrad, hipStream_t s);
+int conv_wino_algo(const ConvGeom& g);
+enum { WEIGHT_OP_NONE = 0, WEIGHT_OP_F4 = 1, WEIGHT_OP_F2 = 2 };
+struct WeightOpLayer {
+    const float* w;
+    float *u_fwd, *u_dgrad;
+    int Cin, Cout;
+    int kind_fwd, kind_dgrad;
+    int first_block;
+};
+int weight_operands_blocks(int Cin, int Cout);
+bool weight_operands_layer_ok(const WeightOpLayer& l);
+void weight_operands_launch(const WeightOpLayer* dev_table, int layers, int blocks, hipStream_t s);
 void conv_wino_fwd(const float* x, const float* u, const float* bias, float* y, const ConvGeom& g, hipStream_t s,
                    float* stat_part = nullptr, int stat_mode = 0, const BnBwdFuse* bn_bwd = nullptr);
 int conv_wino_stat_blocks(const ConvGeom& g);
diff --git a/l3embedding_amd/csrc/ops.hip b/l3embedding_amd/csrc/ops.hip
--- a/l3embedding_amd/csrc/ops.hip
+++ b/l3embedding_amd/csrc/ops.hip
@@ -155,6 +155,66 @@
     return sc.status();
 }
 
+int l3_op_weight_operands(int device, int layers, const int32_t* cin, const int32_t* cout, const float* w, float* uf, float* ud,
+                          float* uf_ref, float* ud_ref, int32_t* kind_fwd, int32_t* kind_dgrad) {
+    if (layers < 1 || !cin || !cout || !w || !kind_fwd || !kind_dgrad) return L3_EINVAL;
+    Scope sc(device);
+    if (!sc.ok) return L3_EHIP;
+    size_t nw = 0, nu = 0;
+    for (int i = 0; i < layers; ++i) {
+        if (cin[i] < 8 || cout[i] < 8 || cin[i] % 8 || cout[i] % 8) {
+            set_op_error("l3_op_weight_operands: channel counts must be positive multiples of 8");
+            return L3_EINVAL;
+        }
+        nw += (size_t)9 * cin[i] * cout[i];
+        nu += (size_t)36 * cin[i] * cout[i];
+    }
+    const float* d_w = sc.put(w, nw);
+    float* d_u[4];
+    for (auto& p : d_u) p = sc.alloc<float>(nu);
+    WeightOpLayer* d_tab = sc.alloc<WeightOpLayer>((size_t)layers);
+    if (!sc.ok) return L3_ENOMEM;
+    for (auto& p : d_u)
+        if (hipMemset(p, 0, nu * sizeof(float)) != hipSuccess) return L3_EHIP;
+    std::vector<WeightOpLayer> tab;
+    size_t ow = 0, ou = 0;
+    int blocks = 0;
+    for (int i = 0; i < layers; ++i) {
+        const ConvGeom g = make_geom(1, 8, 8, cin[i], cout[i], 3, 3, 1), dg = conv_dgrad_geom(g);
+        ConvFwdPath pf;
+        pf.path = CF_FP32, pf.wino_filter = true;
+        ConvDgradPath pd;
+        pd.path = DG_WINO;
+        const int af = conv_weight_op_kind(conv_weight_kind_fwd(pf, g)), ad = conv_weight_op_kind(conv_weight_kind_dgrad(pd, g, dg));
+        if (af == WEIGHT_OP_NONE || ad == WEIGHT_OP_NONE) {
+            set_op_error("l3_op_weight_operands: the split-bf16 operand is not one of the batched launch's layouts");
+            return L3_EINVAL;
+        }
+        kind_fwd[i] = af;
+        kind_dgrad[i] = ad;
+        tab.push_back(WeightOpLayer{d_w + ow, d_u[0] + ou, d_u[1] + ou, cin[i], cout[i], kind_fwd[i], kind_dgrad[i], blocks});
+        blocks += weight_operands_blocks(cin[i], cout[i]);
+        ConvBufs cb;
+        cb.w = d_w + ow;
+        cb.wino_u = d_u[2] + ou;
+        conv_prepare_fwd(pf, g, cb, sc.s);
+        cb.wino_u = d_u[3] + ou;
+        conv_prepare_dgrad(pd, g, dg, cb, sc.s);
+        ow += (size_t)9 * cin[i] * cout[i];
+        ou += (size_t)36 * cin[i] * cout[i];
+    }
+    if (hipMemcpy(d_tab, tab.data(), tab.size() * sizeof(WeightOpLayer), hipMemcpyHostToDevice) != hipSuccess) return L3_EHIP;
+    if (!conv_prepare_batched(tab.data(), d_tab, layers, sc.s)) {
+        set_op_error("l3_op_weight_operands: a layer does not fit its operand layout");
+        return L3_EINVAL;
+    }
+    sc.get(uf, d_u[0], nu);
+    sc.get(ud, d_u[1], nu);
+    sc.get(uf_ref, d_u[2], nu);
+    sc.get(ud_ref, d_u[3], nu);
+    return sc.status();
+}
+
 int l3_op_conv2d_bwd(int device, const float* x, const float* w, const float* dy, float* dx, float* dw, float* db,
                      int n, int h, int wd, int cin, int cout, int kh, int kw, int same) {
     return l3_op_conv2d_bwd_dt(device, L3_DTYPE_F32, x, w, dy, dx, dw, db, n, h, wd, cin, cout, kh, kw, same);
```

Measured after the change: 1998 pairs/s (median of 2 runs). No clear change (+0.1%).
